# LPD-EPFL/ByzantineMomentum

Measured on AMD Instinct MI355X. Metric: aggregations/sec (Byzantine-robust GAR over n workers x d dims; achieved HBM GB/s per GAR in roofline/per_gar), higher is better.
Workload: dtype f32

## Files before the change

### byzantinemomentum_amd/_lib.py

```python

import ctypes
import pathlib

import torch

import os

_PKG_DIR = pathlib.Path(__file__).resolve().parent
LIB_PATH = pathlib.Path(os.environ["BM_GAR_LIB"]).resolve() if os.environ.get("BM_GAR_LIB") else _PKG_DIR / "libbm_gar.so"

ABI_VERSION = 23
MAX_ROWS = 64
EINVAL = -100000
ENOCOMM, ECOMM = -100001, -100002

OP_MEDIAN, OP_TRMEAN, OP_PHOCAS, OP_MEAMED = 0, 1, 2, 3
WS_PAIRWISE, WS_AKSEL, WS_STATS, WS_DOT, WS_STEP, WS_STUDY = 0, 1, 2, 3, 4, 5
STUDY_SLOTS = 32
STUDY_GRAM, STUDY_EX, STUDY_ATTACK = slice(0, 16), slice(16, 18), slice(18, 20)
STUDY_SUMS = slice(0, 20)
STUDY_MAXES = slice(20, 22)
STUDY_L2 = slice(22, 23)
OUT3_SUMS, OUT3_MAX = slice(0, 2), slice(2, 3)
STEP_S2, STEP_SD, STEP_H2, STEP_HD, STEP_D2, STEP_A2, STEP_AD, STEP_L2 = range(8)
STEP_GRAM, STEP_EX = slice(8, 24), slice(24, 26)
STEP_SMAX, STEP_HMAX, STEP_DMAX, STEP_AMAX = range(26, 30)
RANK_KRUM, RANK_BULYAN = 0, 1
ATTACK_EMPIRE, ATTACK_LITTLE, ATTACK_DIRECTION = 0, 1, 16

_c_float_pp = ctypes.POINTER(ctypes.c_void_p)

SIGNATURES = {
  "bm_abi_version": (ctypes.c_int, []),
  "bm_tuning_set": (ctypes.c_int, [ctypes.c_char_p, ctypes.c_int]),
  "bm_error_string": (ctypes.c_char_p, [ctypes.c_int]),
  "bm_colwise": (ctypes.c_int, [ctypes.c_int, _c_float_pp, ctypes.c_int, ctypes.c_int64, ctypes.c_int,
                                ctypes.c_void_p, ctypes.c_void_p]),
  "bm_workspace_bytes": (ctypes.c_int64, [ctypes.c_int, ctypes.c_int, ctypes.c_int64]),
  "bm_pairwise_sqdist": (ctypes.c_int, [_c_float_pp, ctypes.c_int, ctypes.c_int64, ctypes.c_void_p,
                                        ctypes.c_void_p, ctypes.c_void_p]),
  "bm_pairwise_sqdist_shard": (ctypes.c_int, [_c_float_pp, ctypes.c_int, ctypes.c_int64, ctypes.c_int64,
                                              ctypes.c_void_p, ctypes.c_void_p, ctypes.c_void_p]),
  "bm_krum_rank": (ctypes.c_int, [ctypes.c_void_p, ctypes.c_int, ctypes.c_int, ctypes.c_int, ctypes.c_int,
                                  ctypes.c_void_p, ctypes.c_void_p, ctypes.c_void_p]),
  "bm_selected_mean": (ctypes.c_int, [_c_float_pp, ctypes.c_int, ctypes.c_void_p, ctypes.c_int,
                                      ctypes.c_int64, ctypes.c_void_p, ctypes.c_void_p]),
  "bm_bulyan_pass2": (ctypes.c_int, [_c_float_pp, ctypes.c_int, ctypes.c_void_p, ctypes.c_int, ctypes.c_int,
                                     ctypes.c_int64, ctypes.c_void_p, ctypes.c_void_p]),
  "bm_aksel_pass1": (ctypes.c_int, [_c_float_pp, ctypes.c_int, ctypes.c_int64, ctypes.c_void_p,
                                    ctypes.c_void_p, ctypes.c_void_p, ctypes.c_void_p]),
  "bm_stack_stats": (ctypes.c_int, [_c_float_pp, ctypes.c_int, ctypes.c_int64, ctypes.c_void_p, ctypes.c_void_p,
                                    ctypes.c_float, ctypes.c_int, ctypes.c_void_p, ctypes.c_void_p,
                                    ctypes.c_void_p]),
  "bm_multi_dot": (ctypes.c_int, [_c_float_pp, ctypes.c_int, _c_float_pp, ctypes.c_int, ctypes.c_int64,
                                  ctypes.c_void_p, ctypes.c_void_p, ctypes.c_void_p]),
  "bm_momentum_stats_colwise": (ctypes.c_int, [_c_float_pp, ctypes.c_int, _c_float_pp, ctypes.c_int, ctypes.c_int64,
                                               ctypes.c_float, ctypes.c_float, ctypes.c_void_p, ctypes.c_void_p,
                                               ctypes.c_void_p, ctypes.c_void_p, ctypes.c_float, ctypes.c_int,
                                               ctypes.c_int, ctypes.c_int, ctypes.c_int, ctypes.c_void_p,
                                               ctypes.c_void_p, ctypes.c_void_p, ctypes.c_void_p]),
  "bm_momentum_stats_sqdist": (ctypes.c_int, [_c_float_pp, ctypes.c_int, _c_float_pp, ctypes.c_int, ctypes.c_int64,
                                              ctypes.c_int64, ctypes.c_float, ctypes.c_float, ctypes.c_void_p,
                                              ctypes.c_void_p, ctypes.c_void_p, ctypes.c_void_p, ctypes.c_float,
                                              ctypes.c_int, ctypes.c_int, ctypes.c_void_p, ctypes.c_void_p,
                                              ctypes.c_void_p, ctypes.c_void_p, ctypes.c_void_p]),
  "bm_sharded_sq_slot": (ctypes.c_void_p, [ctypes.c_void_p]),
  "bm_sharded_pair_workspace": (ctypes.c_void_p, [ctypes.c_void_p]),
  "bm_sharded_rule_from_sq": (ctypes.c_int, [ctypes.c_void_p, ctypes.c_int, _c_float_pp, ctypes.c_int, ctypes.c_int64,
                                             ctypes.c_int, ctypes.c_int, ctypes.c_void_p, ctypes.c_void_p,
                                             ctypes.c_void_p, ctypes.c_void_p]),
  "bm_stack_stats_colwise": (ctypes.c_int, [_c_float_pp, ctypes.c_int, ctypes.c_int64, ctypes.c_void_p, ctypes.c_void_p,
                                            ctypes.c_float, ctypes.c_int, ctypes.c_int, ctypes.c_int, ctypes.c_int,
                                            ctypes.c_void_p, ctypes.c_void_p, ctypes.c_void_p, ctypes.c_void_p]),
  "bm_stack_stats_sqdist": (ctypes.c_int, [_c_float_pp, ctypes.c_int, ctypes.c_int64, ctypes.c_int64, ctypes.c_void_p,
                                           ctypes.c_void_p, ctypes.c_float, ctypes.c_int, ctypes.c_int, ctypes.c_void_p,
                                           ctypes.c_void_p, ctypes.c_void_p, ctypes.c_void_p, ctypes.c_void_p]),
  "bm_study_stats": (ctypes.c_int, [ctypes.c_void_p, ctypes.c_void_p, ctypes.c_void_p, ctypes.c_void_p, ctypes.c_int,
                                    ctypes.c_void_p, ctypes.c_void_p, ctypes.c_void_p, ctypes.c_void_p, ctypes.c_int,
                                    ctypes.c_float, ctypes.c_float, ctypes.c_void_p, ctypes.c_void_p, ctypes.c_int64,
                                    ctypes.c_void_p, ctypes.c_void_p, ctypes.c_void_p]),
  "bm_study_stats_update": (ctypes.c_int, [ctypes.c_void_p, ctypes.c_void_p, ctypes.c_void_p, ctypes.c_void_p, ctypes.c_int,
                                           ctypes.c_void_p, ctypes.c_void_p, ctypes.c_void_p, ctypes.c_void_p, ctypes.c_int,
                                           ctypes.c_float, ctypes.c_float, ctypes.c_void_p, ctypes.c_void_p,
                                           ctypes.c_void_p, ctypes.c_float, ctypes.c_float, ctypes.c_int64,
                                           ctypes.c_void_p, ctypes.c_void_p, ctypes.c_void_p]),
  "bm_row_sqnorms": (ctypes.c_int, [_c_float_pp, ctypes.c_int, ctypes.c_int64, ctypes.c_void_p, ctypes.c_void_p,
                                    ctypes.c_void_p]),
  "bm_stable_argsort": (ctypes.c_int, [ctypes.c_void_p, ctypes.c_int, ctypes.c_void_p, ctypes.c_void_p]),
  "bm_anticge_workspace_bytes": (ctypes.c_int64, [ctypes.c_int64]),
  "bm_anticge_sum": (ctypes.c_int, [_c_float_pp, ctypes.c_int, ctypes.c_int64, ctypes.c_int, ctypes.c_void_p,
                                    ctypes.c_void_p, ctypes.c_void_p, ctypes.c_void_p, ctypes.c_void_p, ctypes.c_void_p]),
  "bm_anticge_scale": (ctypes.c_int, [ctypes.c_void_p, ctypes.c_int64, ctypes.c_void_p, ctypes.c_void_p]),
  "bm_multi_axpby": (ctypes.c_int, [_c_float_pp, _c_float_pp, ctypes.c_int, ctypes.c_int64,
                                    ctypes.c_float, ctypes.c_float, ctypes.c_void_p]),
  "bm_brute_select": (ctypes.c_int, [ctypes.c_void_p, ctypes.c_int, ctypes.c_int, ctypes.c_void_p]),
  "bm_momentum_stats": (ctypes.c_int, [_c_float_pp, ctypes.c_int, _c_float_pp, ctypes.c_int, ctypes.c_int64,
                                       ctypes.c_float, ctypes.c_float, ctypes.c_void_p, ctypes.c_void_p,
                                       ctypes.c_void_p, ctypes.c_void_p, ctypes.c_float, ctypes.c_int,
                                       ctypes.c_void_p, ctypes.c_void_p, ctypes.c_void_p]),
  "bm_multi_fma3": (ctypes.c_int, [_c_float_pp, _c_float_pp, _c_float_pp, ctypes.c_int, ctypes.c_int64,
                                   ctypes.c_float, ctypes.c_float, ctypes.c_void_p, ctypes.c_void_p]),
  "bm_multi_fma3_bdev": (ctypes.c_int, [_c_float_pp, _c_float_pp, _c_float_pp, ctypes.c_int, ctypes.c_int64,
                                        ctypes.c_float, ctypes.c_void_p, ctypes.c_void_p, ctypes.c_void_p]),
  "bm_clip_factors": (ctypes.c_int, [ctypes.c_void_p, ctypes.c_int, ctypes.c_float, ctypes.c_void_p,
                                     ctypes.c_void_p]),
  "bm_multi_scale": (ctypes.c_int, [_c_float_pp, ctypes.c_int, ctypes.c_int64, ctypes.c_void_p, ctypes.c_void_p]),
  "bm_comm_available": (ctypes.c_int, []),
  "bm_comm_unique_id": (ctypes.c_int, [ctypes.c_void_p]),
  "bm_comm_init": (ctypes.c_int, [ctypes.POINTER(ctypes.c_void_p), ctypes.c_int, ctypes.c_int, ctypes.c_void_p]),
  "bm_comm_destroy": (ctypes.c_int, [ctypes.c_void_p]),
  "bm_comm_size": (ctypes.c_int, [ctypes.c_void_p]),
  "bm_allreduce_sum_f64": (ctypes.c_int, [ctypes.c_void_p, ctypes.c_void_p, ctypes.c_int64, ctypes.c_void_p]),
  "bm_allgather_f32": (ctypes.c_int, [ctypes.c_void_p, ctypes.c_void_p, ctypes.c_void_p, ctypes.c_int64,
                                      ctypes.c_void_p]),
  "bm_brute_select_device": (ctypes.c_int, [ctypes.c_void_p, ctypes.c_int, ctypes.c_int, ctypes.c_void_p, ctypes.c_void_p,
                                            ctypes.c_void_p]),
  "bm_colwise_eval_supported": (ctypes.c_int, [ctypes.c_int, ctypes.c_int]),
  "bm_colwise_eval_workspace_bytes": (ctypes.c_int64, []),
  "bm_colwise_eval": (ctypes.c_int, [ctypes.c_int, _c_float_pp, ctypes.c_int, ctypes.c_int, ctypes.c_int64, ctypes.c_int,
                                     ctypes.c_void_p, ctypes.c_void_p, ctypes.c_float, ctypes.c_void_p, ctypes.c_void_p,
                                     ctypes.c_void_p]),
  "bm_colwise_eval_tdev": (ctypes.c_int, [ctypes.c_int, _c_float_pp, ctypes.c_int, ctypes.c_int, ctypes.c_int64,
                                          ctypes.c_int, ctypes.c_void_p, ctypes.c_void_p, ctypes.c_void_p, ctypes.c_void_p,
                                          ctypes.c_void_p, ctypes.c_void_p]),
  "bm_sqdist2": (ctypes.c_int, [ctypes.c_void_p, ctypes.c_void_p, ctypes.c_int64, ctypes.c_void_p, ctypes.c_void_p,
                                ctypes.c_void_p]),
  "bm_attack_ranking_device": (ctypes.c_int, [ctypes.c_void_p, ctypes.c_int, ctypes.c_int, ctypes.c_int, ctypes.c_int, ctypes.c_int,
                                              ctypes.c_void_p, ctypes.c_void_p, ctypes.c_void_p]),
  "bm_bulyan_pass2_eval_supported": (ctypes.c_int, [ctypes.c_int, ctypes.c_int, ctypes.c_int]),
  "bm_bulyan_pass2_eval": (ctypes.c_int, [_c_float_pp, ctypes.c_int, ctypes.c_int, ctypes.c_void_p, ctypes.c_int, ctypes.c_int,
                                          ctypes.c_int64, ctypes.c_void_p, ctypes.c_void_p, ctypes.c_float, ctypes.c_void_p,
                                          ctypes.c_void_p, ctypes.c_void_p, ctypes.c_void_p]),
  "bm_order_pair_supported": (ctypes.c_int, [ctypes.c_int]),
  "bm_order_pair": (ctypes.c_int, [_c_float_pp, ctypes.c_int, ctypes.c_int64, ctypes.c_int, ctypes.c_int, ctypes.c_void_p,
                                   ctypes.c_void_p, ctypes.c_void_p]),
  "bm_search_device_next": (ctypes.c_int, [ctypes.c_void_p, ctypes.c_void_p, ctypes.c_int, ctypes.c_int, ctypes.c_double,
                                           ctypes.c_double, ctypes.c_double, ctypes.c_void_p, ctypes.c_void_p,
                                           ctypes.c_void_p]),
  "bm_pairwise_rank": (ctypes.c_int, [_c_float_pp, ctypes.c_int, ctypes.c_int64, ctypes.c_int64, ctypes.c_int, ctypes.c_int,
                                      ctypes.c_int, ctypes.c_void_p, ctypes.c_void_p, ctypes.c_void_p, ctypes.c_void_p,
                                      ctypes.c_void_p]),
  "bm_sharded_workspace_bytes": (ctypes.c_int64, [ctypes.c_int, ctypes.c_int64]),
  "bm_sharded_krum": (ctypes.c_int, [ctypes.c_void_p, _c_float_pp, ctypes.c_int, ctypes.c_int64, ctypes.c_int64,
                                     ctypes.c_int, ctypes.c_int, ctypes.c_void_p, ctypes.c_void_p, ctypes.c_void_p, ctypes.c_void_p]),
  "bm_sharded_bulyan": (ctypes.c_int, [ctypes.c_void_p, _c_float_pp, ctypes.c_int, ctypes.c_int64, ctypes.c_int64,
                                       ctypes.c_int, ctypes.c_int, ctypes.c_void_p, ctypes.c_void_p, ctypes.c_void_p,
                                       ctypes.c_void_p]),
  "bm_step_stats_count": (ctypes.c_int, []),
  "bm_step_workspace_bytes": (ctypes.c_int64, [ctypes.c_int, ctypes.c_int64]),
  "bm_step_worker": (ctypes.c_int, [ctypes.c_void_p, ctypes.c_void_p, _c_float_pp, _c_float_pp, ctypes.c_int64,
                                    ctypes.c_int64] + [ctypes.c_void_p] * 13),
  "bm_search_begin": (ctypes.c_int, [ctypes.c_void_p, ctypes.c_double, ctypes.c_double, ctypes.c_double]),
  "bm_search_propose": (ctypes.c_int, [ctypes.c_void_p, ctypes.c_void_p]),
  "bm_search_report": (ctypes.c_int, [ctypes.c_void_p, ctypes.c_double]),
  "bm_attack_objective": (ctypes.c_int, [ctypes.c_void_p, ctypes.c_int, ctypes.c_int, ctypes.c_int, ctypes.c_int,
                                         ctypes.c_int, ctypes.c_double, ctypes.c_void_p, ctypes.c_void_p,
# ... 72 lines not shown
```

### byzantinemomentum_amd/csrc/api.cpp

```cpp
#include <stdlib.h>
#include <string.h>
#include <math.h>
#include <algorithm>
#include <vector>
#include "bm_common.h"

namespace bm {
static int env_int(const char* name, int dflt) {
  const char* v = getenv(name);
  if (v == nullptr || *v == '\0') return dflt;
  return atoi(v);
}
static double env_double(const char* name, double dflt) {
  const char* v = getenv(name);
  if (v == nullptr || *v == '\0') return dflt;
  return atof(v);
}
Tuning& tuning_mutable() {
  static Tuning t = {env_int("BM_COL_BURST", 8),  env_int("BM_MEAN_BURST", 8),
                           env_int("BM_STEP_BURST", 8), env_int("BM_STEP_STREAM", 0), env_int("BM_PAIR_MODE", 0),
                           env_int("BM_PAIR_PLANES", 0), env_int("BM_PAIR_DITHER", 0), env_double("BM_PAIR_TAU", 2e-3),
                           env_int("BM_STUDY_BURST", 8), env_int("BM_STEP_STAGGER_US", 0),
                           env_int("BM_GRAM_STEADY", 1), env_int("BM_BULYAN_SHORT", 1),
                           env_int("BM_PAIR_LOAD_NT", 1), env_int("BM_RANK_ALGO", 0), env_int("BM_COL_WIDE", 1), env_int("BM_BRUTE_BUDGET", 0)};
  return t;
}
const Tuning& tuning() { return tuning_mutable(); }
}

extern "C" int bm_abi_version(void) { return 23; }

extern "C" int bm_tuning_set(const char* name, int value) {
  using namespace bm;
  if (name == nullptr) return BM_EINVAL;
  Tuning& t = tuning_mutable();
  const struct { const char* key; int* slot; } knobs[] = {
      {"BM_COL_BURST", &t.col_burst}, {"BM_MEAN_BURST", &t.mean_burst}, {"BM_STEP_BURST", &t.step_burst},
      {"BM_STEP_STREAM", &t.step_stream}, {"BM_PAIR_MODE", &t.pair_mode}, {"BM_PAIR_PLANES", &t.pair_planes},
      {"BM_PAIR_DITHER", &t.pair_dither}, {"BM_STUDY_BURST", &t.study_burst},
      {"BM_STEP_STAGGER_US", &t.step_stagger_us}, {"BM_GRAM_STEADY", &t.gram_steady},
      {"BM_BULYAN_SHORT", &t.bulyan_short}, {"BM_PAIR_LOAD_NT", &t.pair_load_nt},
      {"BM_RANK_ALGO", &t.rank_algo}, {"BM_COL_WIDE", &t.col_wide}, {"BM_BRUTE_BUDGET", &t.brute_budget}};
  for (const auto& k : knobs)
    if (strcmp(name, k.key) == 0) {
      *k.slot = value;
      return 0;
    }
  return BM_EINVAL;
}

extern "C" const char* bm_error_string(int code) {
  if (code == 0) return "success";
  if (code == BM_EINVAL) return "invalid argument for libbm_gar";
  if (code == BM_ENOCOMM) return "RCCL is not available in this process (librccl.so.1 could not be bound)";
  if (code == BM_ECOMM) return "an RCCL call failed";
  if (code < 0) return hipGetErrorString(static_cast<hipError_t>(-code));
  return "unknown libbm_gar status";
}

namespace {
struct BruteGraph {
  int n;
  uint64_t adj[BM_MAX_ROWS];

  void build(const double* dist, double t) {
    for (int i = 0; i < n; ++i) adj[i] = 0;
    for (int i = 0; i < n; ++i)
      for (int j = i + 1; j < n; ++j) {
        const double v = dist[i * n + j];
        if (isfinite(v) && v <= t) {
          adj[i] |= (uint64_t)1 << j;
          adj[j] |= (uint64_t)1 << i;
        }
      }
  }

  bool has_clique(uint64_t cand, int need) const {
    const int count = __builtin_popcountll(cand);
    if (count < need) return false;
    if (need <= 1) return true;
    int worst = -1, worst_missing = 0;
    for (uint64_t rest = cand; rest != 0; rest &= rest - 1) {
      const int u = __builtin_ctzll(rest);
      const int missing = __builtin_popcountll(cand & ~adj[u] & ~((uint64_t)1 << u));
      if (missing > worst_missing) {
        worst = u;
        worst_missing = missing;
      }
    }
    if (worst < 0) return true;
    const int budget = count - need;
    if (budget == 0) return false;
    const uint64_t bit = (uint64_t)1 << worst;
    if (worst_missing <= budget && has_clique(cand & (adj[worst] | bit), need)) return true;
    return has_clique(cand & ~bit, need);
  }
};
}

extern "C" int bm_brute_select(const double* dist_nxn, int n, int f, int32_t* sel_out) {
  if (dist_nxn == nullptr || sel_out == nullptr || n < 1 || n > BM_MAX_ROWS || f < 0 || n - f < 1)
    return BM_EINVAL;
  const int k = n - f;
  const uint64_t everyone = n == 64 ? ~(uint64_t)0 : (((uint64_t)1 << n) - 1);
  std::vector<double> values;
  values.reserve((size_t)n * (n - 1) / 2 + 1);
  values.push_back(0.0);
  for (int i = 0; i < n; ++i)
    for (int j = i + 1; j < n; ++j) {
      const double v = dist_nxn[i * n + j];
      if (isfinite(v) && v > 0.0) values.push_back(v);
    }
  std::sort(values.begin(), values.end());
  values.erase(std::unique(values.begin(), values.end()), values.end());
  BruteGraph g;
  g.n = n;
  g.build(dist_nxn, values.back());
  if (!g.has_clique(everyone, k)) return BM_EINVAL;
  size_t lo = 0, hi = values.size() - 1;
  while (lo < hi) {
    const size_t mid = (lo + hi) / 2;
    g.build(dist_nxn, values[mid]);
    if (g.has_clique(everyone, k))
      hi = mid;
    else
// ... 18 lines not shown
```

### byzantinemomentum_amd/csrc/bm_common.h

```cpp
#pragma once
#include <hip/hip_runtime.h>
#include <stdint.h>
#include <utility>
#include "../../include/bm_gar.h"
#include "launch_plan.h"

namespace bm {

struct RowTable {
  const float* p[BM_MAX_ROWS];
  RowTable advanced(int64_t by) const {
    RowTable t = *this;
    advance(t.p, by);
    return t;
  }
};

static inline int hip_code(hipError_t e) { return e == hipSuccess ? 0 : -(int)e; }

#define BM_LAUNCH_CHECK()                      \
  do {                                         \
    hipError_t e__ = hipGetLastError();        \
    if (e__ != hipSuccess) return hip_code(e__); \
  } while (0)
// ... 135 lines not shown
    store_result<VEC>(p, src);
}

constexpr int kColMaxBlocks = 256 * 64;

static inline int lds_opt_in(const void* kernel, size_t dynamic_bytes, size_t static_bytes) {
  if (dynamic_bytes + static_bytes <= 48u * 1024u) return 0;
  return hip_code(hipFuncSetAttribute(kernel, hipFuncAttributeMaxDynamicSharedMemorySize, (int)dynamic_bytes));
}

static inline int compute_units() {
  static int cached[16] = {0};
  int dev = 0;
  if (hipGetDevice(&dev) != hipSuccess || dev < 0 || dev >= 16) dev = 0;
  if (cached[dev] == 0) {
    int cus = 0;
    if (hipDeviceGetAttribute(&cus, hipDeviceAttributeMultiprocessorCount, dev) != hipSuccess || cus <= 0) cus = 256;
    cached[dev] = cus;
  }
  return cached[dev];
}

__device__ __forceinline__ bool arrive_last(int* counter, int total, int* lds_flag) {
  asm volatile("s_waitcnt vmcnt(0)" ::: "memory");
  __syncthreads();
  if (threadIdx.x == 0) {
    __builtin_amdgcn_fence(__ATOMIC_RELEASE, "agent");
    asm volatile("s_waitcnt vmcnt(0)" ::: "memory");
    const int ticket = atomicAdd(counter, 1);
    const int last = (ticket == total - 1) ? 1 : 0;
    if (last) __builtin_amdgcn_fence(__ATOMIC_ACQUIRE, "agent");
    *lds_flag = last;
  }
  __syncthreads();
  return *lds_flag != 0;
}

__device__ __forceinline__ int32_t load_index_coherent(const int32_t* p) {
  return __hip_atomic_load(p, __ATOMIC_RELAXED, __HIP_MEMORY_SCOPE_AGENT);
}

template <int BLOCK>
__device__ __forceinline__ double block_reduce_sum(double v, double* lds ) {
#pragma unroll
  for (int off = 32; off > 0; off >>= 1) v += __shfl_down(v, off, 64);
  const int wave = threadIdx.x >> 6, lane = threadIdx.x & 63;
  if (lane == 0) lds[wave] = v;
  __syncthreads();
  double r = 0.0;
  if (threadIdx.x == 0) {
#pragma unroll
    for (int w = 0; w < BLOCK / 64; ++w) r += lds[w];
  }
  __syncthreads();
  return r;
}

__device__ __forceinline__ float byzantine_coordinate(float avg, float q, float fk, float scale, int attack_kind) {
  const float dir = ((attack_kind & 15) == BM_ATTACK_LITTLE) ? __builtin_sqrtf(q / (fk - 1.0f)) : -avg;
  const float att = dir * scale;
  return (attack_kind & BM_ATTACK_DIRECTION) ? att : avg + att;
}

}

namespace bm {
struct Tuning {
  int col_burst;
  int mean_burst;
  int step_burst;
  int step_stream;
  int pair_mode;
  int pair_planes;
  int pair_dither;
  double pair_tau;
  int study_burst;
  int step_stagger_us;
  int gram_steady;
  int bulyan_short;
  int pair_load_nt;
  int rank_algo;
  int col_wide;
  int brute_budget;
};
const Tuning& tuning();
Tuning& tuning_mutable();
}
```

### byzantinemomentum_amd/csrc/step.hip

```cpp
#include "colwise_kernels.h"
#include "gram_split.h"

namespace bm {

constexpr int kStepBlock = 256;
constexpr int kStepMaxBlocks = 16384;
constexpr int kStepPieceCap = 2047;
static_assert(caps_of(kStepPieceCap).sets() <= kStepMaxBlocks + 1, "first pass: partials exceed BM_WS_STEP");

struct StepTable {
  const float* g[BM_MAX_ROWS];
  float* b[BM_MAX_ROWS];
  StepTable advanced(int64_t by) const {
    StepTable t = *this;
    advance(t.g, by);
    advance(t.b, by);
    return t;
  }
};

template <int BLOCK>
__device__ __forceinline__ float block_reduce_absmax(float m, float* lds) {
#pragma unroll
  for (int off = 32; off > 0; off >>= 1) {
    const float o = __shfl_down(m, off, 64);
    m = (m != m || o != o) ? __builtin_nanf("") : fmaxf(m, o);
  }
  if ((threadIdx.x & 63) == 0) lds[threadIdx.x >> 6] = m;
  __syncthreads();
  float r = 0.0f;
  if (threadIdx.x == 0) {
    r = lds[0];
    for (int w = 1; w < BLOCK / 64; ++w) {
      const float o = lds[w];
      r = (r != r || o != o) ? __builtin_nanf("") : fmaxf(r, o);
    }
  }
  __syncthreads();
  return r;
}

template <int BLOCK>
__device__ __forceinline__ void store_step_partials(float n2s, float dvs, float mxs, float n2h, float dvh, float mxh, bool nan_s,
                                                    bool nan_h, double* red, float* mred, double* __restrict__ partial) {
  if (nan_s) mxs = __builtin_nanf("");
  if (nan_h) mxh = __builtin_nanf("");
  const double r0 = block_reduce_sum<BLOCK>((double)n2s, red);
  const double r1 = block_reduce_sum<BLOCK>((double)dvs, red);
  const double r3 = block_reduce_sum<BLOCK>((double)n2h, red);
  const double r4 = block_reduce_sum<BLOCK>((double)dvh, red);
  const float r2 = block_reduce_absmax<BLOCK>(mxs, mred);
  const float r5 = block_reduce_absmax<BLOCK>(mxh, mred);
  if (threadIdx.x == 0) {
    double* p = partial + (int64_t)blockIdx.x * 6;
    p[0] = r0;
    p[1] = r1;
    p[2] = (double)r2;
    p[3] = r3;
    p[4] = r4;
    p[5] = (double)r5;
  }
}

typedef const float* __attribute__((address_space(4))) const* KargRowPtrs;
constexpr int kStepBurstBlock = 512;

template <int T, int VEC, bool EXACT, bool CLIP, bool BURST, int RULE = -1, int NB = 0, bool NOMOM = false>
__global__ __launch_bounds__(BURST ? kStepBurstBlock : kStepBlock) void momentum_stats_kernel(
    StepTable tab, int ks_rt, int h_rt, uint32_t nvec, float mu, float omd, const float* __restrict__ clipf,
    float* __restrict__ s_avg_out, float* __restrict__ h_avg_out, float* __restrict__ byz_out, float scale,
    int attack_kind, double* __restrict__ partial, int rule_f, float rule_inv_keep, float* __restrict__ defense_out) {
  static_assert(RULE < 0 || (EXACT && NB >= 1), "the fused rule needs the row count at compile time");
  static_assert(!NOMOM || (EXACT && !CLIP), "without buffers: same stack, clipped in place beforehand");
  constexpr int BLOCK = BURST ? kStepBurstBlock : kStepBlock;
  __shared__ double red[BLOCK / 64];
  __shared__ float mred[BLOCK / 64];
  const float fks = (float)(EXACT ? T : ks_rt), fh = (float)(EXACT ? T : h_rt);
  float n2s = 0.0f, dvs = 0.0f, mxs = 0.0f, n2h = 0.0f, dvh = 0.0f, mxh = 0.0f;
  bool nan_s = false, nan_h = false;
  uint64_t kbase = (uint64_t)__builtin_amdgcn_kernarg_segment_ptr();
  (void)tab;
  const uint32_t span = gridDim.x * BLOCK;
  const uint32_t iters = (nvec + span - 1) / span;
  const uint32_t first = blockIdx.x * BLOCK + threadIdx.x;
  for (uint32_t it = 0; it < iters; ++it) {
    const uint32_t v = it * span + first;
    const bool live = v < nvec;
    const uint32_t off = v * (uint32_t)(VEC * sizeof(float));
    float g[T][VEC], b[T][VEC];
    float sa[VEC], ha[VEC], bz[VEC], df[VEC];
    asm volatile("" : "+s"(kbase));
    int ks = T, h = T;
    if constexpr (!EXACT) {
      ks = ks_rt;
      h = h_rt;
      asm volatile("" : "+s"(ks), "+s"(h));
    }
    if (live) {
      KargRowPtrs karg = (KargRowPtrs)kbase;
#pragma unroll
      for (int i = 0; i < T; ++i) {
        if (i < ks) load_stream_off<VEC>(karg[i], off, g[i]);
        if constexpr (!NOMOM) {
          if (i < h) load_stream_off<VEC>(karg[BM_MAX_ROWS + i], off, b[i]);
        }
      }
#pragma unroll
      for (int i = 0; i < T; ++i) {
        if constexpr (CLIP) {
          if (i < ks) {
            const float cf = clipf[i];
#pragma unroll
            for (int c = 0; c < VEC; ++c) g[i][c] *= cf;
          }
        }
        if (i < h) {
#pragma unroll
          for (int c = 0; c < VEC; ++c) b[i][c] = NOMOM ? g[i][c] : __builtin_fmaf(omd, g[i][c], mu * b[i][c]);
        }
      }
#pragma unroll
      for (int c = 0; c < VEC; ++c) {
        float s = g[0][c];
#pragma unroll
        for (int i = 1; i < T; ++i)
          if (i < ks) s += g[i][c];
        s = s / fks;
        sa[c] = s;
        n2s = __builtin_fmaf(s, s, n2s);
        mxs = fmaxf(mxs, __builtin_fabsf(s));
        nan_s |= (s != s);
        float q = 0.0f;
#pragma unroll
        for (int i = 0; i < T; ++i)
          if (i < ks) {
            const float df = g[i][c] - s;
            q = __builtin_fmaf(df, df, q);
          }
        dvs += q;
        float t = b[0][c];
#pragma unroll
        for (int i = 1; i < T; ++i)
          if (i < h) t += b[i][c];
        t = t / fh;
        ha[c] = t;
        n2h = __builtin_fmaf(t, t, n2h);
        mxh = fmaxf(mxh, __builtin_fabsf(t));
        nan_h |= (t != t);
        float qh = 0.0f;
#pragma unroll
        for (int i = 0; i < T; ++i)
          if (i < h) {
            const float df = b[i][c] - t;
            qh = __builtin_fmaf(df, df, qh);
          }
        dvh += qh;
        bz[c] = byzantine_coordinate(t, qh, fh, scale, attack_kind);
        if constexpr (RULE >= 0) {
          float x[T + NB];
#pragma unroll
          for (int i = 0; i < T; ++i) x[i] = b[i][c];
#pragma unroll
          for (int i = 0; i < NB; ++i) x[T + i] = bz[c];
          df[c] = column_rule<T + NB, RULE, BLOCK>(x, rule_f, rule_inv_keep, nullptr);
        }
      }
    }
    if constexpr (BURST) __syncthreads();
    asm volatile("" : "+s"(kbase));
    if (live) {
      KargRowPtrs karg = (KargRowPtrs)kbase;
      if constexpr (!NOMOM) {
#pragma unroll
        for (int i = 0; i < T; ++i)
          if (i < h) store_stream_off<VEC>(const_cast<float*>(karg[BM_MAX_ROWS + i]), off, b[i]);
      }
      if (s_avg_out != nullptr) store_stream_off<VEC>(s_avg_out, off, sa);
      if (h_avg_out != nullptr) store_stream_off<VEC>(h_avg_out, off, ha);
      if (byz_out != nullptr) store_stream_off<VEC>(byz_out, off, bz);
      if constexpr (RULE >= 0) store_stream_off<VEC>(defense_out, off, df);
    }
  }
  store_step_partials<BLOCK>(n2s, dvs, mxs, n2h, dvh, mxh, nan_s, nan_h, red, mred, partial);
}

constexpr int kSgRowBytes = 272;
constexpr int kSgWaves = kStepBurstBlock / 64;
template <int TT>
struct SgShape {
  static constexpr int N = TT + 1;
  static constexpr int RB = (N + 15) / 16;
  static constexpr int NP = RB * (RB + 1) / 2;
  static constexpr int kRows = N + 1;
  static constexpr int kPlaneBytes = kRows * kSgRowBytes;
  static constexpr int kWaveBytes = 2 * kPlaneBytes;
  static constexpr int kAccBytes = NP * 4 * kStepBurstBlock * 4;
  static constexpr int kRedBytes = kSgWaves * 256 * 8;
  static constexpr int kPlanes = kSgWaves * kWaveBytes > kRedBytes ? kSgWaves * kWaveBytes : kRedBytes;
  static constexpr int kLds = kPlanes + kAccBytes;
};

template <int TT, bool CLIP, bool NOMOM = false>
__global__ __launch_bounds__(kStepBurstBlock) void momentum_gram_kernel(
    StepTable tab, uint32_t nvec, float mu, float omd, const float* __restrict__ clipf, float* __restrict__ s_avg_out,
    float* __restrict__ h_avg_out, float* __restrict__ byz_out, float scale, int attack_kind, unsigned dither_seed,
    double* __restrict__ partial, double* __restrict__ gram_partial, int* __restrict__ arrival, int stagger_ticks) {
  using SG = SgShape<TT>;
  constexpr int T = TT, VEC = 4, BLOCK = kStepBurstBlock;
  constexpr int kSgPlaneBytes = SG::kPlaneBytes, kSgWaveBytes = SG::kWaveBytes, kSgN = SG::N, RB = SG::RB, NP = SG::NP;
  extern __shared__ __attribute__((aligned(16))) char sg_smem[];
  __shared__ double red[BLOCK / 64];
  __shared__ float mred[BLOCK / 64];
  const int tid = threadIdx.x, wave = tid >> 6, lane = tid & 63;
  char* wbase = sg_smem + wave * kSgWaveBytes;
  for (int o = lane * 16; o < kSgWaveBytes; o += 64 * 16) *reinterpret_cast<f32x4*>(wbase + o) = f32x4{0.0f, 0.0f, 0.0f, 0.0f};
  if (blockIdx.x == 0 && tid == 0 && arrival != nullptr) *arrival = 0;
  if (stagger_ticks > 0 && ((blockIdx.x >> 3) & 1)) {
    const uint64_t t0 = wall_clock64();
    while ((uint64_t)wall_clock64() - t0 < (uint64_t)stagger_ticks) __builtin_amdgcn_s_sleep(16);
  }
  const float fks = (float)T, fh = (float)T;
  float n2s = 0.0f, dvs = 0.0f, mxs = 0.0f, n2h = 0.0f, dvh = 0.0f, mxh = 0.0f;
  bool nan_s = false, nan_h = false;
  float* acc_lds = reinterpret_cast<float*>(sg_smem + SG::kPlanes) + tid;
#pragma unroll
  for (int p = 0; p < NP * 4; ++p) acc_lds[p * BLOCK] = 0.0f;
  uint64_t kbase = (uint64_t)__builtin_amdgcn_kernarg_segment_ptr();
  (void)tab;
  const uint32_t span = gridDim.x * BLOCK;
  const uint32_t iters = (nvec + span - 1) / span;
  const uint32_t first = blockIdx.x * BLOCK + threadIdx.x;
  const int li = lane & 15, lg = lane >> 4;
  const int rd0 = li * kSgRowBytes + lg * 16;
  const int rd_last = ((16 * (RB - 1) + li < kSgN) ? (16 * (RB - 1) + li) : kSgN) * kSgRowBytes + lg * 16;
  const int wr0 = (lane & 31) * 8;
  for (uint32_t it = 0; it < iters; ++it) {
    const uint32_t v = it * span + first;
    const bool live = v < nvec;
    const uint32_t off = v * (uint32_t)(VEC * sizeof(float));
    float b[T][VEC];
    float sa[VEC], ha[VEC], bz[VEC];
#pragma unroll
    for (int c = 0; c < VEC; ++c) sa[c] = ha[c] = bz[c] = 0.0f;
    asm volatile("" : "+s"(kbase));
    if (live) {
      float g[T][VEC];
      KargRowPtrs karg = (KargRowPtrs)kbase;
#pragma unroll
      for (int i = 0; i < T; ++i) {
        load_stream_off<VEC>(karg[i], off, g[i]);
        if constexpr (!NOMOM) load_stream_off<VEC>(karg[BM_MAX_ROWS + i], off, b[i]);
      }
#pragma unroll
      for (int i = 0; i < T; ++i) {
        if constexpr (CLIP) {
          const float cf = clipf[i];
#pragma unroll
          for (int c = 0; c < VEC; ++c) g[i][c] *= cf;
        }
#pragma unroll
        for (int c = 0; c < VEC; ++c) b[i][c] = NOMOM ? g[i][c] : __builtin_fmaf(omd, g[i][c], mu * b[i][c]);
      }
#pragma unroll
      for (int c = 0; c < VEC; ++c) {
        float s = g[0][c];
#pragma unroll
// ... 170 lines not shown
          for (int c = 0; c < VEC; ++c) {
            const float gv = CLIP ? g[j][c] * cfi : g[j][c];
            if (i == 0) {
              ps[c] = gv;
              ss[c] = gv;
              qs[c] = 0.0f;
              ts[c] = 0.0f;
            } else {
              const float dd = on_s ? gv - ps[c] : 0.0f;
              ss[c] += on_s ? gv : 0.0f;
              qs[c] = __builtin_fmaf(dd, dd, qs[c]);
              ts[c] += dd;
            }
            g[j][c] = gv;
          }
          if (base < hl) {
#pragma unroll
            for (int c = 0; c < VEC; ++c) b[j][c] = __builtin_fmaf(omd, g[j][c], mu * b[j][c]);
            if (on_h) store_stream_off<VEC>(const_cast<float*>(karg[BM_MAX_ROWS + i]), off, b[j]);
#pragma unroll
            for (int c = 0; c < VEC; ++c) {
              const float bv = b[j][c];
              if (i == 0) {
                ph[c] = bv;
                sh[c] = bv;
                qh[c] = 0.0f;
                th[c] = 0.0f;
              } else {
                const float dd = on_h ? bv - ph[c] : 0.0f;
                sh[c] += on_h ? bv : 0.0f;
                qh[c] = __builtin_fmaf(dd, dd, qh[c]);
                th[c] += dd;
              }
            }
          }
        }
      }
    }
    float r_sa[VEC], r_ha[VEC], r_bz[VEC];
#pragma unroll
    for (int c = 0; c < VEC; ++c) {
      const float s = ss[c] / fks;
      r_sa[c] = s;
      n2s = __builtin_fmaf(s, s, n2s);
      mxs = fmaxf(mxs, __builtin_fabsf(s));
      nan_s |= (s != s);
      const float es = s - ps[c];
      dvs += __builtin_fmaf(es, __builtin_fmaf(fks, es, -2.0f * ts[c]), qs[c]);
      const float t = sh[c] / fh;
      r_ha[c] = t;
      n2h = __builtin_fmaf(t, t, n2h);
      mxh = fmaxf(mxh, __builtin_fabsf(t));
      nan_h |= (t != t);
      const float eh = t - ph[c];
      float colq = __builtin_fmaf(eh, __builtin_fmaf(fh, eh, -2.0f * th[c]), qh[c]);
      colq = colq < 0.0f ? 0.0f : colq;
      dvh += colq;
      r_bz[c] = byzantine_coordinate(t, colq, fh, scale, attack_kind);
    }
    if (s_avg_out != nullptr) store_stream_off<VEC>(s_avg_out, off, r_sa);
    if (h_avg_out != nullptr) store_stream_off<VEC>(h_avg_out, off, r_ha);
    if (byz_out != nullptr) store_stream_off<VEC>(byz_out, off, r_bz);
  }
  if (nan_s) mxs = __builtin_nanf("");
  if (nan_h) mxh = __builtin_nanf("");
  const double r0 = block_reduce_sum<kStepBlock>((double)n2s, red);
  const double r1 = block_reduce_sum<kStepBlock>((double)dvs, red);
  const double r3 = block_reduce_sum<kStepBlock>((double)n2h, red);
  const double r4 = block_reduce_sum<kStepBlock>((double)dvh, red);
  const float r2 = block_reduce_absmax<kStepBlock>(mxs, mred);
  const float r5 = block_reduce_absmax<kStepBlock>(mxh, mred);
  if (threadIdx.x == 0) {
    double* p = partial + (int64_t)blockIdx.x * 6;
    p[0] = r0;
    p[1] = r1 < 0.0 ? 0.0 : r1;
    p[2] = (double)r2;
    p[3] = r3;
    p[4] = r4;
    p[5] = (double)r5;
  }
}

constexpr int kFinishThreads = 256;
__global__ __launch_bounds__(kFinishThreads) void step_finish_kernel(const double* __restrict__ partial, int nparts,
                                                                     double* __restrict__ out6) {
  __shared__ double red[kFinishThreads / 64][8];
  const int lane = threadIdx.x & 63, wave = threadIdx.x >> 6;
  double s[6] = {0.0, 0.0, 0.0, 0.0, 0.0, 0.0};
  bool nan2 = false, nan5 = false;
  for (int b = threadIdx.x; b < nparts; b += kFinishThreads) {
    const double* p = partial + (int64_t)b * 6;
    s[0] += p[0];
    s[1] += p[1];
    s[3] += p[3];
    s[4] += p[4];
    nan2 |= (p[2] != p[2]);
    nan5 |= (p[5] != p[5]);
    s[2] = p[2] > s[2] ? p[2] : s[2];
    s[5] = p[5] > s[5] ? p[5] : s[5];
  }
#pragma unroll
  for (int off = 32; off > 0; off >>= 1) {
    s[0] += __shfl_down(s[0], off, 64);
    s[1] += __shfl_down(s[1], off, 64);
    s[3] += __shfl_down(s[3], off, 64);
    s[4] += __shfl_down(s[4], off, 64);
    const double o2 = __shfl_down(s[2], off, 64), o5 = __shfl_down(s[5], off, 64);
    s[2] = o2 > s[2] ? o2 : s[2];
    s[5] = o5 > s[5] ? o5 : s[5];
    nan2 |= (bool)__shfl_down((int)nan2, off, 64);
    nan5 |= (bool)__shfl_down((int)nan5, off, 64);
  }
  if (lane == 0) {
#pragma unroll
    for (int k = 0; k < 6; ++k) red[wave][k] = s[k];
    red[wave][6] = nan2 ? 1.0 : 0.0;
    red[wave][7] = nan5 ? 1.0 : 0.0;
  }
  __syncthreads();
  if (threadIdx.x == 0) {
    for (int w = 1; w < kFinishThreads / 64; ++w) {
      s[0] += red[w][0];
      s[1] += red[w][1];
      s[3] += red[w][3];
      s[4] += red[w][4];
      s[2] = red[w][2] > s[2] ? red[w][2] : s[2];
      s[5] = red[w][5] > s[5] ? red[w][5] : s[5];
      nan2 |= red[w][6] != 0.0;
      nan5 |= red[w][7] != 0.0;
    }
  }
  if (threadIdx.x == 0) {
    out6[0] = s[0];
    out6[1] = s[1];
    out6[2] = nan2 ? __builtin_nan("") : s[2];
    out6[3] = s[3];
    out6[4] = s[4];
    out6[5] = nan5 ? __builtin_nan("") : s[5];
  }
}

struct StepArgs {
  StepTable tab;
  int ks, h;
  int64_t nvec;
  float mu, omd;
  const float* clipf;
  float *s_avg, *h_avg, *byz;
  float scale;
  int kind;
  double* partial;
  int* grid_io;
  hipStream_t s;
  bool nomom = false;
  int rule_f = 0;
  float rule_inv_keep = 0.0f;
  float* defense = nullptr;
  StepArgs moved(int64_t by) const {
    StepArgs a = *this;
    a.tab = tab.advanced(by);
    a.s_avg = advanced(s_avg, by);
    a.h_avg = advanced(h_avg, by);
    a.byz = advanced(byz, by);
    return a;
  }
  StepArgs at(Span& sp) const {
    StepArgs a = moved(sp.first);
    a.nvec = sp.count;
    a.partial = partial + (int64_t)sp.part * 6;
    a.grid_io = &sp.grid;
    return a;
  }
};

static StepTable make_step_table(const float* const* sampled, int ks, float* const* buffers, int h) {
  StepTable tab{};
  for (int i = 0; i < BM_MAX_ROWS; ++i) {
    tab.g[i] = sampled[i < ks ? i : ks - 1];
    if (buffers != nullptr) tab.b[i] = buffers[i < h ? i : h - 1];
  }
  return tab;
}

static bool burst_ready(int64_t nvec, int cus) {
  return tuning().step_burst > 0 && nvec / ((int64_t)cus * kStepBurstBlock) >= tuning().step_burst;
}

static bool is_column_rule(int op) {
  return op == BM_OP_MEDIAN || op == BM_OP_TRMEAN || op == BM_OP_PHOCAS || op == BM_OP_MEAMED;
}
static bool is_identical_attack(int kind) {
  return (kind & ~BM_ATTACK_DIRECTION) == BM_ATTACK_EMPIRE || (kind & ~BM_ATTACK_DIRECTION) == BM_ATTACK_LITTLE;
}

template <class Kernel>
static int launch_momentum_stats_kernel(Kernel kernel, int grid, int block, const StepArgs& a) {
  hipLaunchKernelGGL(kernel, dim3(grid), dim3(block), 0, a.s, a.tab, a.ks, a.h, (uint32_t)a.nvec, a.mu, a.omd, a.clipf,
                     a.s_avg, a.h_avg, a.byz, a.scale, a.kind, a.partial, a.rule_f, a.rule_inv_keep, a.defense);
  BM_LAUNCH_CHECK();
  return 0;
}

template <int T, int VEC, bool EXACT, bool CLIP, int RULE = -1, int NB = 0, bool NOMOM = false>
static int launch_momentum_stats_form(const StepArgs& a) {
  const int cus = compute_units();
  if (burst_ready(a.nvec, cus) && cus < *a.grid_io) {
    *a.grid_io = cus;
    return launch_momentum_stats_kernel(momentum_stats_kernel<T, VEC, EXACT, CLIP, true, RULE, NB, NOMOM>, cus, kStepBurstBlock, a);
  }
  return launch_momentum_stats_kernel(momentum_stats_kernel<T, VEC, EXACT, CLIP, false, RULE, NB, NOMOM>, *a.grid_io, kStepBlock, a);
}

template <int T, int VEC>
static int launch_momentum_stats(const StepArgs& a) {
  const bool exact = (a.ks == T && a.h == T);
  if constexpr (T > 12) {
    if (!exact) return BM_EINVAL;
    return a.clipf != nullptr ? launch_momentum_stats_form<T, VEC, true, true>(a) : launch_momentum_stats_form<T, VEC, true, false>(a);
  } else {
    if (a.clipf != nullptr) return exact ? launch_momentum_stats_form<T, VEC, true, true>(a) : launch_momentum_stats_form<T, VEC, false, true>(a);
    return exact ? launch_momentum_stats_form<T, VEC, true, false>(a) : launch_momentum_stats_form<T, VEC, false, false>(a);
  }
}

template <int T, int VEC>
static int launch_momentum_stats_stream(const StepArgs& a) {
  auto kernel = a.clipf != nullptr ? momentum_stats_stream_kernel<T, VEC, true> : momentum_stats_stream_kernel<T, VEC, false>;
  hipLaunchKernelGGL(kernel, dim3(*a.grid_io), dim3(kStepBlock), 0, a.s, a.tab, a.ks, a.h, (uint32_t)a.nvec, a.mu, a.omd,
                     a.clipf, a.s_avg, a.h_avg, a.byz, a.scale, a.kind, a.partial);
  BM_LAUNCH_CHECK();
  return 0;
}

template <int VEC>
static int dispatch_momentum_stats(const StepArgs& a) {
  const int ks = a.ks, h = a.h, t = ks > h ? ks : h;
  if (tuning().step_stream != 1) {
    if (t <= 8) return launch_momentum_stats<8, VEC>(a);
    if (t <= 12) return launch_momentum_stats<12, VEC>(a);
    if (ks == 14 && h == 14) return launch_momentum_stats<14, VEC>(a);
    if (ks == 20 && h == 20) return launch_momentum_stats<20, VEC>(a);
  }
  if (t <= 20) return launch_momentum_stats_stream<20, VEC>(a);
  if (t <= 40) return launch_momentum_stats_stream<40, VEC>(a);
  return launch_momentum_stats_stream<64, VEC>(a);
}

struct Fma3Table {
  float* out[BM_MAX_ROWS];
  const float* p[BM_MAX_ROWS];
  const float* q[BM_MAX_ROWS];
  Fma3Table advanced(int64_t by) const {
    Fma3Table t = *this;
    advance(t.out, by);
    advance(t.p, by);
    advance(t.q, by);
    return t;
  }
};

template <int VEC>
__global__ __launch_bounds__(kStepBlock) void multi_fma3_kernel(Fma3Table tab, int64_t nvec, float a, float b_host,
                                                                const float* __restrict__ pscale,
                                                                const double* __restrict__ b_dev) {
  const float b = b_dev != nullptr ? (float)b_dev[0] : b_host;
  float* out = tab.out[blockIdx.y];
  const float* p = tab.p[blockIdx.y];
  const float* q = tab.q[blockIdx.y];
  const float c = pscale != nullptr ? pscale[blockIdx.y] : 1.0f;
  const int64_t stride = (int64_t)gridDim.x * kStepBlock;
  for (int64_t v = (int64_t)blockIdx.x * kStepBlock + threadIdx.x; v < nvec; v += stride) {
    float pp[VEC], qq[VEC];
    load_stream<VEC>(p + v * VEC, pp);
    load_stream<VEC>(q + v * VEC, qq);
#pragma unroll
    for (int e = 0; e < VEC; ++e) {
      const float x = pscale != nullptr ? pp[e] * c : pp[e];
      pp[e] = __builtin_fmaf(b, qq[e], a * x);
    }
    store_stream<VEC>(out + v * VEC, pp);
  }
}

struct ScaleTable {
  float* y[BM_MAX_ROWS];
  ScaleTable advanced(int64_t by) const {
    ScaleTable t = *this;
    advance(t.y, by);
    return t;
  }
};
template <int VEC>
__global__ __launch_bounds__(kStepBlock) void multi_scale_kernel(ScaleTable tab, int64_t nvec,
                                                                 const float* __restrict__ factors) {
  const float c = factors[blockIdx.y];
  if (c == 1.0f) return;
  float* y = tab.y[blockIdx.y];
  const int64_t stride = (int64_t)gridDim.x * kStepBlock;
  for (int64_t v = (int64_t)blockIdx.x * kStepBlock + threadIdx.x; v < nvec; v += stride) {
    float yy[VEC];
    load_stream<VEC>(y + v * VEC, yy);
#pragma unroll
    for (int e = 0; e < VEC; ++e) yy[e] *= c;
    store_stream<VEC>(y + v * VEC, yy);
  }
}

__global__ __launch_bounds__(64) void clip_factors_kernel(const double* __restrict__ row_sq, int k, float clip,
                                                          float* __restrict__ factors) {
  const int i = threadIdx.x;
  if (i >= k) return;
  const double norm = sqrt(row_sq[i]);
  factors[i] = (norm > (double)clip) ? (float)((double)clip / norm) : 1.0f;
}

template <int T, int RULE, int NB, bool CLIP, bool NOMOM = false>
static int launch_fused_rule(StepArgs a) {
  constexpr int N = T + NB;
  const int keep = (RULE == BM_OP_TRMEAN) ? (N - 2 * a.rule_f) : ((RULE == BM_OP_PHOCAS || RULE == BM_OP_MEAMED) ? (N - a.rule_f) : N);
  a.rule_inv_keep = 1.0f / (float)(keep > 0 ? keep : 1);
  return launch_momentum_stats_form<T, 4, true, CLIP, RULE, NB, NOMOM>(a);
}

template <int T, int RULE, int NB>
static int launch_fused_rule_clip(const StepArgs& a) {
  if (a.nomom) return launch_fused_rule<T, RULE, NB, false, true>(a);
  return a.clipf != nullptr ? launch_fused_rule<T, RULE, NB, true>(a) : launch_fused_rule<T, RULE, NB, false>(a);
}

static bool fused_rule_shape(int h, int nb) { return (h == 20 && nb == 5) || (h == 14 && nb == 11); }
static bool fused_rule_instance(int ks, int h, int nb, int op) {
  return is_column_rule(op) && tuning().step_stream != 1 && ks == h && fused_rule_shape(h, nb);
}

static int launch_fused_rule_any(int op, int nb, int rule_f, float* defense, StepArgs a) {
  a.rule_f = rule_f;
  a.defense = defense;
#define BM_FUSED_CASE(TV, NBV)                                                                 \
  if (a.h == TV && nb == NBV) {                                                                \
    if (op == BM_OP_MEDIAN) return launch_fused_rule_clip<TV, BM_OP_MEDIAN, NBV>(a);           \
    if (op == BM_OP_TRMEAN) return launch_fused_rule_clip<TV, BM_OP_TRMEAN, NBV>(a);           \
    if (op == BM_OP_PHOCAS) return launch_fused_rule_clip<TV, BM_OP_PHOCAS, NBV>(a);           \
    return launch_fused_rule_clip<TV, BM_OP_MEAMED, NBV>(a);                                   \
  }
  BM_FUSED_CASE(20, 5) BM_FUSED_CASE(14, 11)
#undef BM_FUSED_CASE
  return BM_EINVAL;
}

double* pairwise_gram_area(void* ws);
int* pairwise_arrival_counter(void* ws);
int pairwise_from_gram_partials(const float* const* rows, int n_full, int nc, int blocks, int64_t d, double* sq_nxn,
                                void* ws, hipStream_t s);

template <int TT>
static int launch_momentum_gram_rows(const StepArgs& a, int cus, void* ws_pair) {
  auto kernel = a.nomom ? momentum_gram_kernel<TT, false, true>
                        : (a.clipf != nullptr ? momentum_gram_kernel<TT, true> : momentum_gram_kernel<TT, false>);
  constexpr int lds = SgShape<TT>::kLds;
  if (const int rc = lds_opt_in(reinterpret_cast<const void*>(kernel), lds, kSgWaves * (sizeof(double) + sizeof(float)))) return rc;
  *a.grid_io = cus;
  hipLaunchKernelGGL(kernel, dim3(cus), dim3(kStepBurstBlock), lds, a.s, a.tab, (uint32_t)a.nvec, a.mu, a.omd, a.clipf,
                     a.s_avg, a.h_avg, a.byz, a.scale, a.kind, (unsigned)tuning().pair_dither, a.partial,
                     pairwise_gram_area(ws_pair), pairwise_arrival_counter(ws_pair), tuning().step_stagger_us * 100);
  BM_LAUNCH_CHECK();
  return 0;
}
static int launch_momentum_gram(const StepArgs& a, int cus, void* ws_pair) {
  return a.h == 20 ? launch_momentum_gram_rows<20>(a, cus, ws_pair) : launch_momentum_gram_rows<14>(a, cus, ws_pair);
}

__global__ __launch_bounds__(256) void tail_gram_kernel(RowTable rows , int nrows,
                                                        const float* __restrict__ h_avg_tail, int cols,
                                                        double* __restrict__ block) {
  const int t = threadIdx.x;
  if (t >= nrows * (nrows + 1) / 2) return;
  int i = 0, rem = t, len = nrows;
  while (rem >= len) {
    rem -= len;
    --len;
    ++i;
  }
  const int j = i + rem;
  double acc = 0.0;
  for (int c = 0; c < cols; ++c) {
    const float ctr = (__builtin_fabsf(h_avg_tail[c]) < __builtin_inff()) ? h_avg_tail[c] : 0.0f;
    acc += (double)(rows.p[i][c] - ctr) * (double)(rows.p[j][c] - ctr);
  }
  block[b3_tri_index(i, j, nrows)] = acc;
}

int64_t step_workspace_bytes() { return (int64_t)(kStepMaxBlocks + 1) * 6 * (int64_t)sizeof(double); }

static int momentum_stats_impl(const float* const* sampled, int ks, float* const* buffers, int h, int64_t d, float mu,
                               float one_minus_damp, const float* clip_factors, float* sampled_avg, float* honest_avg,
                               float* byz_out, float scale, int attack_kind, double* out6, void* ws, void* stream,
                               int rule_op, int rule_f, int nb, float* defense_out) {
  if (sampled == nullptr || buffers == nullptr || out6 == nullptr || ws == nullptr || h < 1 || ks < h ||
      ks > BM_MAX_ROWS || d < 0 || !is_identical_attack(attack_kind))
    return BM_EINVAL;
  if (rule_op >= 0 && (!is_column_rule(rule_op) || nb < 1 || h + nb > BM_MAX_ROWS || (attack_kind & BM_ATTACK_DIRECTION) != 0 ||
                       (d > 0 && (byz_out == nullptr || defense_out == nullptr)) ||
                       (rule_op != BM_OP_MEDIAN && (rule_f < 0 || h + nb < 2 * rule_f + 1))))
    return BM_EINVAL;
  hipStream_t s = static_cast<hipStream_t>(stream);
  const int vec = Alignment().of(sampled_avg).of(honest_avg).of(byz_out).of(rule_op >= 0 ? defense_out : nullptr)
                      .of(sampled, ks).of(buffers, h).vec();
  double* partial = static_cast<double*>(ws);
  const StepArgs pass{make_step_table(sampled, ks, buffers, h), ks, h, 0, mu, one_minus_damp, clip_factors, sampled_avg,
                      honest_avg, byz_out, scale, attack_kind, partial, nullptr, s};
  const int64_t pieces = piece_count(d);
  int cap = pieces > 1 ? (int)((kStepMaxBlocks - 1) / pieces) - 1 : kStepPieceCap;
  if (cap > kStepPieceCap) cap = kStepPieceCap;
  if (cap < 1) return BM_EINVAL;
  const bool fusable = rule_op >= 0 && fused_rule_instance(ks, h, nb, rule_op);
  int nparts = 0;
  const int rc = for_pieces(d, [&](int64_t lo, int64_t dp) {
    const StepArgs piece = pass.moved(lo);
    int64_t ruled = 0;
    const int rc = for_body_and_tail<4>(Tail::kOwnLaunch, vec, dp, kStepBlock, caps_of(cap), [&](auto width, Span& sp) {
      constexpr int VEC = decltype(width)::value;
      if constexpr (VEC == 4) {
        if (fusable) {
          ruled = sp.end;
          return launch_fused_rule_any(rule_op, nb, rule_f, defense_out + lo, piece.at(sp));
        }
      }
      return dispatch_momentum_stats<VEC>(piece.at(sp));
    }, &nparts);
    if (rc != 0 || rule_op < 0 || ruled == dp) return rc;
    const float* rows[BM_MAX_ROWS];
    for (int i = 0; i < h; ++i) rows[i] = buffers[i] + lo + ruled;
    for (int i = 0; i < nb; ++i) rows[h + i] = byz_out + lo + ruled;
    return bm_colwise(rule_op, rows, h + nb, dp - ruled, rule_f, defense_out + lo + ruled, stream);
  });
  if (rc != 0) return rc;
  hipLaunchKernelGGL(step_finish_kernel, dim3(1), dim3(kFinishThreads), 0, s, partial, nparts, out6);
  BM_LAUNCH_CHECK();
  return 0;
}
}

extern "C" int bm_momentum_stats(const float* const* sampled, int ks, float* const* buffers, int h, int64_t d,
                                 float mu, float one_minus_damp, const float* clip_factors, float* sampled_avg,
                                 float* honest_avg, float* byz_out, float scale, int attack_kind, double* out6,
                                 void* ws, void* stream) {
  return bm::momentum_stats_impl(sampled, ks, buffers, h, d, mu, one_minus_damp, clip_factors, sampled_avg, honest_avg,
                                 byz_out, scale, attack_kind, out6, ws, stream, -1, 0, 0, nullptr);
}

extern "C" int bm_momentum_stats_colwise(const float* const* sampled, int ks, float* const* buffers, int h, int64_t d,
                                         float mu, float one_minus_damp, const float* clip_factors, float* sampled_avg,
                                         float* honest_avg, float* byz_out, float scale, int attack_kind, int rule_op,
                                         int rule_f, int n_byz, float* defense_out, double* out6, void* ws,
                                         void* stream) {
  if (rule_op < 0) return BM_EINVAL;
  return bm::momentum_stats_impl(sampled, ks, buffers, h, d, mu, one_minus_damp, clip_factors, sampled_avg, honest_avg,
                                 byz_out, scale, attack_kind, out6, ws, stream, rule_op, rule_f, n_byz, defense_out);
}

extern "C" int bm_momentum_stats_sqdist(const float* const* sampled, int ks, float* const* buffers, int h, int64_t d,
                                        int64_t d_total, float mu, float one_minus_damp, const float* clip_factors,
                                        float* sampled_avg, float* honest_avg, float* byz_out, float scale,
                                        int attack_kind, int n_byz, double* sq_nxn, double* out6, void* ws,
                                        void* ws_pair, void* stream) {
  using namespace bm;
  const int n = h + n_byz;
  if (sampled == nullptr || buffers == nullptr || out6 == nullptr || ws == nullptr || ws_pair == nullptr ||
      sq_nxn == nullptr || h < 1 || ks < h || ks > BM_MAX_ROWS || n_byz < 1 || n > BM_MAX_ROWS || d < 0 || d_total < d ||
      !is_identical_attack(attack_kind) || (attack_kind & BM_ATTACK_DIRECTION) != 0 || (d > 0 && byz_out == nullptr))
    return BM_EINVAL;
  hipStream_t s = static_cast<hipStream_t>(stream);
  const float* rows[BM_MAX_ROWS];
  for (int i = 0; i < h; ++i) rows[i] = buffers[i];
  for (int i = h; i < n; ++i) rows[i] = byz_out;
// ... 10 lines not shown
    return bm_pairwise_sqdist_shard(rows, n, d, d_total, sq_nxn, ws_pair, stream);
  }
  double* partial = static_cast<double*>(ws);
  const StepArgs pass{make_step_table(sampled, ks, buffers, h), ks, h, 0, mu, one_minus_damp, clip_factors, sampled_avg,
                      honest_avg, byz_out, scale, attack_kind, partial, nullptr, s};
  const int nc = h + 1;
  const int per_block = nc * (nc + 1) / 2;
  int nparts = 0, blocks = 0;
  const int rc = for_body_and_tail<4>(Tail::kOwnLaunch, vec, d, kStepBlock, caps_of(kStepPieceCap), [&](auto width, Span& sp) {
    constexpr int VEC = decltype(width)::value;
    if constexpr (VEC == 4) {
      blocks = cus;
      return launch_momentum_gram(pass.at(sp), cus, ws_pair);
    } else if constexpr (VEC == 1) {
      if (const int rc = dispatch_momentum_stats<1>(pass.at(sp))) return rc;
      RowTable trows{};
      for (int i = 0; i < h; ++i) trows.p[i] = buffers[i] + sp.first;
      trows.p[h] = byz_out + sp.first;
      hipLaunchKernelGGL(tail_gram_kernel, dim3(1), dim3(256), 0, s, trows, nc, honest_avg + sp.first, (int)sp.count,
                         pairwise_gram_area(ws_pair) + (int64_t)blocks * per_block);
      BM_LAUNCH_CHECK();
      blocks += 1;
      return 0;
    } else {
      return BM_EINVAL;
    }
  }, &nparts);
  if (rc != 0) return rc;
  hipLaunchKernelGGL(step_finish_kernel, dim3(1), dim3(kFinishThreads), 0, s, partial, nparts, out6);
  BM_LAUNCH_CHECK();
  return pairwise_from_gram_partials(rows, n, nc, blocks, d, sq_nxn, ws_pair, s);
}

namespace bm {
static int stack_stats_plain(const float* const* rows, int k, int64_t d, float* avg_out, float* byz_out, float scale,
                             int attack_kind, double* out6, void* ws, void* stream) {
  int rc = bm_stack_stats(rows, k, d, avg_out, byz_out, scale, attack_kind, out6 + 3, ws, stream);
  if (rc != 0) return rc;
  return hip_code(hipMemcpyAsync(out6, out6 + 3, 3 * sizeof(double), hipMemcpyDeviceToDevice,
                                 static_cast<hipStream_t>(stream)));
}
static bool nomom_shape(int k, int nb) { return (k == 20 && nb >= 1 && nb <= 6) || (k == 14 && nb == 11); }
}

extern "C" int bm_stack_stats_colwise(const float* const* rows, int k, int64_t d, float* avg_out, float* byz_out,
                                      float scale, int attack_kind, int rule_op, int rule_f, int n_byz,
                                      float* defense_out, double* out6, void* ws, void* stream) {
  using namespace bm;
  const int n = k + n_byz;
  if (rows == nullptr || out6 == nullptr || ws == nullptr || k < 1 || n_byz < 1 || n > BM_MAX_ROWS || d < 0 ||
      !is_identical_attack(attack_kind) || (attack_kind & BM_ATTACK_DIRECTION) != 0 || !is_column_rule(rule_op) ||
      (rule_op != BM_OP_MEDIAN && (rule_f < 0 || n < 2 * rule_f + 1)) ||
      (d > 0 && (avg_out == nullptr || byz_out == nullptr || defense_out == nullptr)))
    return BM_EINVAL;
  hipStream_t s = static_cast<hipStream_t>(stream);
  const int vec = Alignment().of(avg_out).of(byz_out).of(defense_out).of(rows, k).vec();
  const bool fused = fused_rule_shape(k, n_byz) && vec == 4 && d % 4 == 0 && d > 0 && d <= kMaxColsPerLaunch &&
                     tuning().step_stream != 1;
  if (fused) {
    double* partial = static_cast<double*>(ws);
    StepArgs pass{make_step_table(rows, k, nullptr, k), k, k, 0, 0.0f, 1.0f, nullptr, nullptr, avg_out, byz_out, scale,
                  attack_kind, partial, nullptr, s};
    pass.nomom = true;
    int nparts = 0;
    const int rc = for_body_and_tail<4>(Tail::kOwnLaunch, vec, d, kStepBlock, caps_of(kStepPieceCap), [&](auto width, Span& sp) {
      if constexpr (decltype(width)::value == 4)
        return launch_fused_rule_any(rule_op, n_byz, rule_f, defense_out, pass.at(sp));
      else
        return BM_EINVAL;
    }, &nparts);
    if (rc != 0) return rc;
    hipLaunchKernelGGL(step_finish_kernel, dim3(1), dim3(kFinishThreads), 0, s, partial, nparts, out6);
    BM_LAUNCH_CHECK();
    return 0;
  }
  int rc = stack_stats_plain(rows, k, d, avg_out, byz_out, scale, attack_kind, out6, ws, stream);
  if (rc != 0 || d == 0) return rc;
  const float* all[BM_MAX_ROWS];
  for (int i = 0; i < k; ++i) all[i] = rows[i];
  for (int i = k; i < n; ++i) all[i] = byz_out;
  return bm_colwise(rule_op, all, n, d, rule_f, defense_out, stream);
}

extern "C" int bm_stack_stats_sqdist(const float* const* rows, int k, int64_t d, int64_t d_total, float* avg_out,
                                     float* byz_out, float scale, int attack_kind, int n_byz, double* sq_nxn,
                                     double* out6, void* ws, void* ws_pair, void* stream) {
  using namespace bm;
  const int n = k + n_byz;
  if (rows == nullptr || out6 == nullptr || ws == nullptr || ws_pair == nullptr || sq_nxn == nullptr || k < 1 ||
      n_byz < 1 || n > BM_MAX_ROWS || d < 0 || d_total < d ||
      !is_identical_attack(attack_kind) || (attack_kind & BM_ATTACK_DIRECTION) != 0 ||
      (d > 0 && (avg_out == nullptr || byz_out == nullptr)))
    return BM_EINVAL;
  hipStream_t s = static_cast<hipStream_t>(stream);
  const float* all[BM_MAX_ROWS];
  for (int i = 0; i < k; ++i) all[i] = rows[i];
  for (int i = k; i < n; ++i) all[i] = byz_out;
  const int vec = Alignment().of(avg_out).of(byz_out).of(rows, k).vec();
  const int cus = compute_units();
  const bool fused = nomom_shape(k, n_byz) && vec == 4 && d % 4 == 0 && d <= kMaxColsPerLaunch &&
                     tuning().step_stream != 1 && tuning().pair_mode == 0 && tuning().pair_planes != 3 &&
                     burst_ready(d / 4, cus);
  if (!fused) {
    int rc = stack_stats_plain(rows, k, d, avg_out, byz_out, scale, attack_kind, out6, ws, stream);
    if (rc != 0) return rc;
    return bm_pairwise_sqdist_shard(all, n, d, d_total, sq_nxn, ws_pair, stream);
  }
  double* partial = static_cast<double*>(ws);
  StepArgs pass{make_step_table(rows, k, nullptr, k), k, k, 0, 0.0f, 1.0f, nullptr, nullptr, avg_out, byz_out, scale,
                attack_kind, partial, nullptr, s};
  pass.nomom = true;
  int nparts = 0;
  const int rc = for_body_and_tail<4>(Tail::kOwnLaunch, vec, d, kStepBlock, caps_of(kStepPieceCap), [&](auto width, Span& sp) {
    if constexpr (decltype(width)::value == 4)
      return launch_momentum_gram(pass.at(sp), cus, ws_pair);
    else
      return BM_EINVAL;
  }, &nparts);
  if (rc != 0) return rc;
  hipLaunchKernelGGL(step_finish_kernel, dim3(1), dim3(kFinishThreads), 0, s, partial, nparts, out6);
  BM_LAUNCH_CHECK();
  return pairwise_from_gram_partials(all, n, k + 1, cus, d, sq_nxn, ws_pair, s);
}

static int multi_fma3_launch(float* const* out, const float* const* p, const float* const* q, int k, int64_t d, float a,
                             float b, const float* p_scale, const double* b_dev, void* stream) {
  using namespace bm;
  if (out == nullptr || p == nullptr || q == nullptr || k < 1 || k > BM_MAX_ROWS || d < 0) return BM_EINVAL;
  if (d == 0) return 0;
  hipStream_t s = static_cast<hipStream_t>(stream);
  Fma3Table tab{};
  for (int i = 0; i < k; ++i) {
    tab.out[i] = out[i];
    tab.p[i] = p[i];
    tab.q[i] = q[i];
  }
  const int vec = Alignment().of(out, k).of(p, k).of(q, k).vec();
  return for_body_and_tail<4>(Tail::kOwnLaunch, vec, d, kStepBlock, caps_of(2048), [&](auto width, const Span& sp) {
    hipLaunchKernelGGL(multi_fma3_kernel<decltype(width)::value>, dim3(sp.grid, k), dim3(kStepBlock), 0, s,
                       tab.advanced(sp.first), sp.count, a, b, p_scale, b_dev);
    BM_LAUNCH_CHECK();
    return 0;
  });
}

extern "C" int bm_multi_fma3(float* const* out, const float* const* p, const float* const* q, int k, int64_t d,
                             float a, float b, const float* p_scale, void* stream) {
  return multi_fma3_launch(out, p, q, k, d, a, b, p_scale, nullptr, stream);
}

extern "C" int bm_multi_fma3_bdev(float* const* out, const float* const* p, const float* const* q, int k, int64_t d,
                                  float a, const double* b_dev, const float* p_scale, void* stream) {
  if (b_dev == nullptr) return BM_EINVAL;
  return multi_fma3_launch(out, p, q, k, d, a, 0.0f, p_scale, b_dev, stream);
}

extern "C" int bm_multi_scale(float* const* y, int k, int64_t d, const float* factors, void* stream) {
  using namespace bm;
  if (y == nullptr || factors == nullptr || k < 1 || k > BM_MAX_ROWS || d < 0) return BM_EINVAL;
  if (d == 0) return 0;
  hipStream_t s = static_cast<hipStream_t>(stream);
  ScaleTable tab{};
  for (int i = 0; i < k; ++i) tab.y[i] = y[i];
  const int vec = Alignment().of(y, k).vec();
  return for_body_and_tail<4>(Tail::kOwnLaunch, vec, d, kStepBlock, caps_of(2048), [&](auto width, const Span& sp) {
    hipLaunchKernelGGL(multi_scale_kernel<decltype(width)::value>, dim3(sp.grid, k), dim3(kStepBlock), 0, s,
// ... 15 lines not shown
```

### byzantinemomentum_amd/csrc/step_call.hip

```cpp
#include "bm_common.h"

namespace bm {

constexpr int kStatSums = 26;
constexpr int kStatMaxes = 4;
constexpr int kStatSlots = 32;
static_assert(kStatSums + kStatMaxes <= kStatSlots, "statistics vector layout");

struct StepScalars {
  double out6[6];
  double study[BM_STUDY_SLOTS];
  double rowsq[BM_MAX_ROWS];
  double mine[kStatSlots];
  double all[kStatSlots * BM_MAX_ROWS];
  float clipf[BM_MAX_ROWS];
};

__global__ void step_pack_kernel(StepScalars* sc, int has_attack, int has_past, int has_l2, double* __restrict__ direct_out) {
  if (threadIdx.x != 0) return;
  double* m = sc->mine;
  const double* st = sc->study;
  for (int i = 0; i < kStatSlots; ++i) m[i] = 0.0;
  m[0] = sc->out6[0];
  m[1] = sc->out6[1];
// ... 21 lines not shown
  const int slot = threadIdx.x;
  if (slot >= kStatSlots) return;
  double acc = all[slot];
  bool nan = acc != acc;
  for (int r = 1; r < nranks; ++r) {
    const double v = all[r * kStatSlots + slot];
    if (slot < kStatSums) {
      acc += v;
    } else {
      nan |= (v != v);
      acc = v > acc ? v : acc;
    }
  }
  out[slot] = (slot >= kStatSums && nan) ? __builtin_nan("") : acc;
}

struct StepLayout {
  int64_t scalars, ws_step, ws_study, ws_dot, ws_rule, total;
};

static StepLayout step_layout(int n, int64_t d) {
  StepLayout l;
  auto up = [](int64_t v) { return (v + 255) / 256 * 256; };
  int64_t off = 0;
  l.scalars = off;
  off += up((int64_t)sizeof(StepScalars));
  l.ws_step = off;
  off += up(bm_workspace_bytes(BM_WS_STEP, 1, d));
  l.ws_study = off;
  off += up(bm_workspace_bytes(BM_WS_STUDY, 1, d));
  l.ws_dot = off;
  off += up(bm_workspace_bytes(BM_WS_DOT, 1, d));
  l.ws_rule = off;
  off += up(bm_sharded_workspace_bytes(n, d));
  l.total = off;
  return l;
}

}

extern "C" int bm_step_stats_count(void) { return bm::kStatSlots; }

extern "C" int64_t bm_step_workspace_bytes(int n, int64_t d_local) {
  if (n < 1 || n > BM_MAX_ROWS || d_local < 0) return BM_EINVAL;
  return bm::step_layout(n, d_local).total;
}

extern "C" int bm_step_worker(bm_comm* comm, const bm_step_params* p, const float* const* sampled,
                              float* const* buffers, int64_t d, int64_t d_total, float* defense_out,
                              float* sampled_avg_out,
                              float* honest_avg_out, float* byz_out, float* attack_avg_out,
                              const float* past_newest, float* curv, const float* past_oldest, const float* params,
                              const float* origin, double* stats_out, void* ws, void* stream) {
  using namespace bm;
  if (p == nullptr || sampled == nullptr || buffers == nullptr || stats_out == nullptr || ws == nullptr || d < 0 ||
      d_total < d)
    return BM_EINVAL;
  const int n = p->n, h = p->n - p->f_real, ks = p->ks, fr = p->f_real;
  if (n < 1 || n > BM_MAX_ROWS || h < 1 || ks < h || ks > BM_MAX_ROWS || fr < 0 ||
      (d > 0 && (defense_out == nullptr || sampled_avg_out == nullptr || honest_avg_out == nullptr)) ||
      (fr > 0 && d > 0 && byz_out == nullptr))
    return BM_EINVAL;
  const bool distance_rule = p->rule == BM_RULE_KRUM || p->rule == BM_RULE_BULYAN;
  if (!distance_rule && p->rule != BM_RULE_MEDIAN && p->rule != BM_RULE_TRMEAN && p->rule != BM_RULE_PHOCAS &&
      p->rule != BM_RULE_MEAMED)
    return BM_EINVAL;
  hipStream_t s = static_cast<hipStream_t>(stream);
  char* base = static_cast<char*>(ws);
  const StepLayout lay = step_layout(n, d);
  StepScalars* sc = reinterpret_cast<StepScalars*>(base + lay.scalars);
  int rc;

  const float* clipf = nullptr;
  if (p->clip > 0.0f) {
    rc = bm_row_sqnorms(sampled, ks, d, sc->rowsq, base + lay.ws_dot, stream);
    if (rc != 0) return rc;
    rc = bm_allreduce_sum_f64(comm, sc->rowsq, ks, stream);
    if (rc != 0) return rc;
    rc = bm_clip_factors(sc->rowsq, ks, p->clip, sc->clipf, stream);
    if (rc != 0) return rc;
    clipf = sc->clipf;
  }

  const bool rides_along = fr >= 1;
  const float* rows[BM_MAX_ROWS];
  for (int i = 0; i < h; ++i) rows[i] = buffers[i];
  for (int i = h; i < n; ++i) rows[i] = byz_out;
  const int m = p->m > 0 ? p->m : n - p->f_decl - 2;
  if (rides_along && !distance_rule) {
    const int op = p->rule == BM_RULE_MEDIAN ? BM_OP_MEDIAN
                   : p->rule == BM_RULE_TRMEAN ? BM_OP_TRMEAN : p->rule == BM_RULE_PHOCAS ? BM_OP_PHOCAS : BM_OP_MEAMED;
    rc = bm_momentum_stats_colwise(sampled, ks, buffers, h, d, p->mu, p->one_minus_damp, clipf, sampled_avg_out,
                                   honest_avg_out, byz_out, p->attack_scale, p->attack_kind, op, p->f_decl, fr,
                                   defense_out, sc->out6, base + lay.ws_step, stream);
    if (rc != 0) return rc;
  } else if (rides_along) {
    char* rule_ws = base + lay.ws_rule;
    rc = bm_momentum_stats_sqdist(sampled, ks, buffers, h, d, d_total, p->mu, p->one_minus_damp,
                                  clipf, sampled_avg_out, honest_avg_out, byz_out, p->attack_scale, p->attack_kind, fr,
                                  bm_sharded_sq_slot(rule_ws), sc->out6, base + lay.ws_step,
                                  bm_sharded_pair_workspace(rule_ws), stream);
    if (rc != 0) return rc;
    rc = bm_sharded_rule_from_sq(comm, p->rule, rows, n, d, p->f_decl, m, defense_out, nullptr, rule_ws, stream);
    if (rc != 0) return rc;
  } else {
    rc = bm_momentum_stats(sampled, ks, buffers, h, d, p->mu, p->one_minus_damp, clipf, sampled_avg_out, honest_avg_out,
                           nullptr, p->attack_scale, p->attack_kind, sc->out6, base + lay.ws_step, stream);
    if (rc != 0) return rc;
    switch (p->rule) {
      case BM_RULE_KRUM:
        rc = bm_sharded_krum(comm, rows, n, d, d_total, p->f_decl, m, defense_out, nullptr, base + lay.ws_rule, stream);
        break;
      case BM_RULE_BULYAN:
        rc = bm_sharded_bulyan(comm, rows, n, d, d_total, p->f_decl, m, defense_out, nullptr, base + lay.ws_rule, stream);
        break;
      case BM_RULE_MEDIAN: rc = bm_colwise(BM_OP_MEDIAN, rows, n, d, 0, defense_out, stream); break;
      case BM_RULE_TRMEAN: rc = bm_colwise(BM_OP_TRMEAN, rows, n, d, p->f_decl, defense_out, stream); break;
      case BM_RULE_PHOCAS: rc = bm_colwise(BM_OP_PHOCAS, rows, n, d, p->f_decl, defense_out, stream); break;
      default: rc = bm_colwise(BM_OP_MEAMED, rows, n, d, p->f_decl, defense_out, stream); break;
    }
    if (rc != 0) return rc;
  }

  int curv_mode = 0;
  if (p->nb_past > 0 && curv != nullptr) {
    if (p->past_count == 0 || past_newest == nullptr)
      curv_mode = 1;
    else
      curv_mode = past_oldest != nullptr ? 3 : 2;
  }
  const bool has_past = curv_mode >= 2;
  const bool has_l2 = params != nullptr && origin != nullptr;
  rc = bm_study_stats(sampled_avg_out, honest_avg_out, defense_out, byz_out, fr, attack_avg_out, past_newest, curv,
                      past_oldest, curv_mode, p->mu, p->oldest_weight, params, origin, d, sc->study,
                      base + lay.ws_study, stream);
  if (rc != 0) return rc;

  hipLaunchKernelGGL(step_pack_kernel, dim3(1), dim3(64), 0, s, sc, fr > 0 ? 1 : 0, has_past ? 1 : 0, has_l2 ? 1 : 0,
                     comm == nullptr ? stats_out : static_cast<double*>(nullptr));
  BM_LAUNCH_CHECK();
  if (comm == nullptr) return 0;
  const int nranks = bm_comm_size(comm);
  if (nranks > BM_MAX_ROWS) return BM_EINVAL;
  rc = bm_allgather_f32(comm, reinterpret_cast<const float*>(sc->mine), reinterpret_cast<float*>(sc->all),
                        2 * kStatSlots, stream);
  if (rc != 0) return rc;
  hipLaunchKernelGGL(step_reduce_kernel, dim3(1), dim3(64), 0, s, sc->all, nranks, stats_out);
  BM_LAUNCH_CHECK();
  return 0;
}
```

### byzantinemomentum_amd/csrc/study.hip

```cpp
#include "bm_common.h"

namespace bm {

constexpr int kStudyBlock = 256;
constexpr int kStudyMaxBlocks = 2048;
constexpr int kStudySums = 14;
constexpr int kStudyPartial = 16;

struct StudyArgs {
  const float* s;
  const float* h;
  const float* def;
  const float* byz;
  const float* past;
  const float* oldest;
  const float* params;
  const float* origin;
  float* curv;
  float* a_out;
  float* mom;
  float mom_a, mom_b;
  StudyArgs advanced(int64_t by) const {
    using bm::advanced;
    return StudyArgs{advanced(s, by), advanced(h, by), advanced(def, by), advanced(byz, by), advanced(past, by),
                     advanced(oldest, by), advanced(params, by), advanced(origin, by), advanced(curv, by),
                     advanced(a_out, by), advanced(mom, by), mom_a, mom_b};
  }
};
constexpr Caps kStudyCaps = caps_of(kStudyMaxBlocks);

template <bool ATT, int CM, bool L2, int VEC>
__global__ __launch_bounds__(kStudyBlock) void study_stats_kernel(StudyArgs a, int f_real, float mu, float w_oldest,
                                                                  int64_t nvec, double* __restrict__ partial) {
  __shared__ double red[kStudyBlock / 64];
  __shared__ float mred[kStudyBlock / 64];
  float acc[kStudySums];
  double acc64[kStudySums];
#pragma unroll
  for (int i = 0; i < kStudySums; ++i) {
    acc[i] = 0.0f;
    acc64[i] = 0.0;
  }
  int since = 0;
  float amax = 0.0f, dmax = 0.0f;
  bool a_nan = false, d_nan = false;
  const float ff = (float)f_real;
  const int64_t stride = (int64_t)gridDim.x * kStudyBlock;
  for (int64_t v = (int64_t)blockIdx.x * kStudyBlock + threadIdx.x; v < nvec; v += stride) {
    const int64_t j = v * VEC;
    float s[VEC], h[VEC], df[VEC], bz[VEC], pa[VEC], cv[VEC], ol[VEC], pp[VEC], oo[VEC], mm[VEC];
    load_stream<VEC>(a.s + j, s);
    load_stream<VEC>(a.h + j, h);
    load_stream<VEC>(a.def + j, df);
    if (a.mom != nullptr) load_stream<VEC>(a.mom + j, mm);
    if constexpr (ATT) load_stream<VEC>(a.byz + j, bz);
    if constexpr (CM >= 2) {
      load_stream<VEC>(a.past + j, pa);
      load_stream<VEC>(a.curv + j, cv);
    }
    if constexpr (CM == 3) load_stream<VEC>(a.oldest + j, ol);
    if constexpr (L2) {
      load_stream<VEC>(a.params + j, pp);
      load_stream<VEC>(a.origin + j, oo);
    }
    float av[VEC];
#pragma unroll
    for (int c = 0; c < VEC; ++c) {
      av[c] = 0.0f;
      if constexpr (ATT) {
        float t = bz[c];
        for (int i = 1; i < f_real; ++i) t += bz[c];
        t = t / ff;
        av[c] = t;
        amax = fmaxf(amax, __builtin_fabsf(t));
        a_nan |= (t != t);
        const float dd = bz[c] - t;
        float q = 0.0f;
        for (int i = 0; i < f_real; ++i) q = __builtin_fmaf(dd, dd, q);
        acc[12] += q;
      }
      dmax = fmaxf(dmax, __builtin_fabsf(df[c]));
      d_nan |= (df[c] != df[c]);
      acc[0] = __builtin_fmaf(s[c], s[c], acc[0]);
      acc[1] = __builtin_fmaf(s[c], h[c], acc[1]);
      acc[2] = __builtin_fmaf(s[c], df[c], acc[2]);
      acc[4] = __builtin_fmaf(h[c], h[c], acc[4]);
      acc[5] = __builtin_fmaf(h[c], df[c], acc[5]);
      acc[7] = __builtin_fmaf(df[c], df[c], acc[7]);
      if constexpr (ATT) {
        acc[3] = __builtin_fmaf(s[c], av[c], acc[3]);
        acc[6] = __builtin_fmaf(h[c], av[c], acc[6]);
        acc[8] = __builtin_fmaf(df[c], av[c], acc[8]);
        acc[9] = __builtin_fmaf(av[c], av[c], acc[9]);
      }
      if constexpr (CM >= 2) {
        acc[10] = __builtin_fmaf(s[c], pa[c], acc[10]);
        acc[11] = __builtin_fmaf(s[c], cv[c], acc[11]);
      }
      if constexpr (L2) {
        const float e = pp[c] - oo[c];
        acc[13] = __builtin_fmaf(e, e, acc[13]);
      }
      if constexpr (CM == 1) cv[c] = s[c];
      if constexpr (CM == 3) cv[c] = __builtin_fmaf(w_oldest, ol[c], 1.0f * cv[c]);
      if constexpr (CM >= 2) cv[c] = __builtin_fmaf(1.0f, s[c], mu * cv[c]);
    }
    if constexpr (CM >= 1) store_stream<VEC>(a.curv + j, cv);
    if (a.mom != nullptr) {
#pragma unroll
      for (int c = 0; c < VEC; ++c) mm[c] = __builtin_fmaf(a.mom_b, df[c], a.mom_a * mm[c]);
      store_stream<VEC>(a.mom + j, mm);
    }
    if constexpr (ATT) {
      if (a.a_out != nullptr) store_stream<VEC>(a.a_out + j, av);
    }
    if (++since == 16) {
#pragma unroll
      for (int i = 0; i < kStudySums; ++i) {
        acc64[i] += (double)acc[i];
        acc[i] = 0.0f;
      }
      since = 0;
    }
  }
  if (a_nan) amax = __builtin_nanf("");
  if (d_nan) dmax = __builtin_nanf("");
  constexpr int64_t kSlotStride = kStudyMaxBlocks + 1;
  double* p = partial + blockIdx.x;
#pragma unroll
  for (int i = 0; i < kStudySums; ++i) {
    const double r = block_reduce_sum<kStudyBlock>(acc64[i] + (double)acc[i], red);
    if (threadIdx.x == 0) p[i * kSlotStride] = r;
  }
  float m2[2] = {amax, dmax};
#pragma unroll
  for (int k = 0; k < 2; ++k) {
    float m = m2[k];
#pragma unroll
    for (int off = 32; off > 0; off >>= 1) {
      const float o = __shfl_down(m, off, 64);
      m = (m != m || o != o) ? __builtin_nanf("") : fmaxf(m, o);
    }
    if ((threadIdx.x & 63) == 0) mred[threadIdx.x >> 6] = m;
    __syncthreads();
    if (threadIdx.x == 0) {
      float mm = mred[0];
      for (int wv = 1; wv < kStudyBlock / 64; ++wv) {
        const float o = mred[wv];
        mm = (mm != mm || o != o) ? __builtin_nanf("") : fmaxf(mm, o);
      }
      p[(kStudySums + k) * kSlotStride] = (double)mm;
    }
    __syncthreads();
  }
}

constexpr int kStudyBurstThreads = 1024;
constexpr int kStudySlotBudget = 8;

template <bool ATT, int CM, bool L2, bool MOM = false>
__global__ __launch_bounds__(kStudyBurstThreads) void study_stats_burst_kernel(StudyArgs a, int f_real, float mu,
                                                                               float w_oldest, uint32_t nvec,
                                                                               double* __restrict__ partial) {
  static_assert(CM >= 1, "without a written stream there is nothing to burst");
  constexpr int VEC = 4;
  constexpr int kStudySlots = MOM ? kStudySlotBudget / 2 : kStudySlotBudget;
  constexpr int U = ((L2 && CM >= 2) || MOM) ? 1 : 2;
  using V = typename VecLoad<VEC>::T;
  __shared__ V stage[kStudySlots * kStudyBurstThreads];
  __shared__ V stage_mom[MOM ? kStudySlots * kStudyBurstThreads : 1];
  __shared__ double red[kStudyBurstThreads / 64];
  __shared__ float mred[kStudyBurstThreads / 64];
  float acc[kStudySums];
  double acc64[kStudySums];
#pragma unroll
  for (int i = 0; i < kStudySums; ++i) {
    acc[i] = 0.0f;
    acc64[i] = 0.0;
  }
  float amax = 0.0f, dmax = 0.0f;
  bool a_nan = false, d_nan = false;
  const float ff = (float)f_real;
  const uint32_t tid = threadIdx.x;
  const uint32_t span = gridDim.x * kStudyBurstThreads;
  const uint32_t iters = (nvec + span - 1) / span;
  const uint32_t first = blockIdx.x * kStudyBurstThreads + tid;
  for (uint32_t p0 = 0; p0 < iters; p0 += kStudySlots) {
    const uint32_t p1 = (p0 + kStudySlots < iters) ? p0 + kStudySlots : iters;
    for (uint32_t it = p0; it < p1; it += U) {
      float s[U][VEC], h[U][VEC], df[U][VEC], bz[U][VEC], pa[U][VEC], cv[U][VEC], ol[U][VEC], pp[U][VEC], oo[U][VEC];
      float mm[U][VEC];
      bool live[U];
#pragma unroll
      for (int u = 0; u < U; ++u) {
        const uint32_t v = (it + u) * span + first;
        live[u] = (it + u) < p1 && v < nvec;
        if (live[u]) {
          const int64_t j = (int64_t)v * VEC;
          load_stream<VEC>(a.s + j, s[u]);
          load_stream<VEC>(a.h + j, h[u]);
          load_stream<VEC>(a.def + j, df[u]);
          if constexpr (MOM) load_stream<VEC>(a.mom + j, mm[u]);
          if constexpr (ATT) load_stream<VEC>(a.byz + j, bz[u]);
          if constexpr (CM >= 2) {
            load_stream<VEC>(a.past + j, pa[u]);
            load_stream<VEC>(a.curv + j, cv[u]);
          }
          if constexpr (CM == 3) load_stream<VEC>(a.oldest + j, ol[u]);
          if constexpr (L2) {
            load_stream<VEC>(a.params + j, pp[u]);
            load_stream<VEC>(a.origin + j, oo[u]);
          }
        }
      }
#pragma unroll
      for (int u = 0; u < U; ++u) {
        if (!live[u]) continue;
#pragma unroll
        for (int c = 0; c < VEC; ++c) {
          float av = 0.0f;
          if constexpr (ATT) {
            float t = bz[u][c];
            for (int i = 1; i < f_real; ++i) t += bz[u][c];
            t = t / ff;
            av = t;
            amax = fmaxf(amax, __builtin_fabsf(t));
            a_nan |= (t != t);
            const float dd = bz[u][c] - t;
            float q = 0.0f;
            for (int i = 0; i < f_real; ++i) q = __builtin_fmaf(dd, dd, q);
            acc[12] += q;
          }
          dmax = fmaxf(dmax, __builtin_fabsf(df[u][c]));
          d_nan |= (df[u][c] != df[u][c]);
          acc[0] = __builtin_fmaf(s[u][c], s[u][c], acc[0]);
          acc[1] = __builtin_fmaf(s[u][c], h[u][c], acc[1]);
          acc[2] = __builtin_fmaf(s[u][c], df[u][c], acc[2]);
          acc[4] = __builtin_fmaf(h[u][c], h[u][c], acc[4]);
          acc[5] = __builtin_fmaf(h[u][c], df[u][c], acc[5]);
          acc[7] = __builtin_fmaf(df[u][c], df[u][c], acc[7]);
          if constexpr (ATT) {
            acc[3] = __builtin_fmaf(s[u][c], av, acc[3]);
            acc[6] = __builtin_fmaf(h[u][c], av, acc[6]);
            acc[8] = __builtin_fmaf(df[u][c], av, acc[8]);
            acc[9] = __builtin_fmaf(av, av, acc[9]);
          }
          if constexpr (CM >= 2) {
            acc[10] = __builtin_fmaf(s[u][c], pa[u][c], acc[10]);
            acc[11] = __builtin_fmaf(s[u][c], cv[u][c], acc[11]);
          }
          if constexpr (L2) {
            const float e = pp[u][c] - oo[u][c];
            acc[13] = __builtin_fmaf(e, e, acc[13]);
          }
          if constexpr (CM == 1) cv[u][c] = s[u][c];
          if constexpr (CM == 3) cv[u][c] = __builtin_fmaf(w_oldest, ol[u][c], 1.0f * cv[u][c]);
          if constexpr (CM >= 2) cv[u][c] = __builtin_fmaf(1.0f, s[u][c], mu * cv[u][c]);
        }
        V packed;
#pragma unroll
        for (int c = 0; c < VEC; ++c) packed[c] = cv[u][c];
        stage[(it + u - p0) * kStudyBurstThreads + tid] = packed;
        if constexpr (MOM) {
#pragma unroll
          for (int c = 0; c < VEC; ++c) packed[c] = __builtin_fmaf(a.mom_b, df[u][c], a.mom_a * mm[u][c]);
          stage_mom[(it + u - p0) * kStudyBurstThreads + tid] = packed;
        }
      }
    }
#pragma unroll
    for (int i = 0; i < kStudySums; ++i) {
      acc64[i] += (double)acc[i];
      acc[i] = 0.0f;
    }
    __syncthreads();
    for (uint32_t it = p0; it < p1; ++it) {
      const uint32_t v = it * span + first;
      if (v < nvec) {
        __builtin_nontemporal_store(stage[(it - p0) * kStudyBurstThreads + tid], reinterpret_cast<V*>(a.curv + (int64_t)v * VEC));
        if constexpr (MOM)
          __builtin_nontemporal_store(stage_mom[(it - p0) * kStudyBurstThreads + tid], reinterpret_cast<V*>(a.mom + (int64_t)v * VEC));
      }
    }
  }
  if (a_nan) amax = __builtin_nanf("");
  if (d_nan) dmax = __builtin_nanf("");
  constexpr int64_t kSlotStride = kStudyMaxBlocks + 1;
  double* p = partial + blockIdx.x;
#pragma unroll
  for (int i = 0; i < kStudySums; ++i) {
    const double r = block_reduce_sum<kStudyBurstThreads>(acc64[i], red);
    if (threadIdx.x == 0) p[i * kSlotStride] = r;
  }
  float m2[2] = {amax, dmax};
#pragma unroll
  for (int k = 0; k < 2; ++k) {
    float m = m2[k];
#pragma unroll
    for (int off = 32; off > 0; off >>= 1) {
      const float o = __shfl_down(m, off, 64);
      m = (m != m || o != o) ? __builtin_nanf("") : fmaxf(m, o);
    }
    if ((threadIdx.x & 63) == 0) mred[threadIdx.x >> 6] = m;
    __syncthreads();
    if (threadIdx.x == 0) {
      float mm = mred[0];
      for (int wv = 1; wv < kStudyBurstThreads / 64; ++wv) {
        const float o = mred[wv];
        mm = (mm != mm || o != o) ? __builtin_nanf("") : fmaxf(mm, o);
      }
      p[(kStudySums + k) * kSlotStride] = (double)mm;
    }
    __syncthreads();
  }
}

__global__ __launch_bounds__(64) void study_finish_kernel(const double* __restrict__ partial, int nparts,
                                                          double* __restrict__ out) {
  const int slot = blockIdx.x, lane = threadIdx.x;
  if (slot == 0 && lane >= 23 && lane < BM_STUDY_SLOTS) out[lane] = 0.0;
  double tot = 0.0;
  bool nan = false;
  const bool is_max = slot >= kStudySums;
  for (int b = lane; b < nparts; b += 64) {
    const double v = partial[(int64_t)slot * (kStudyMaxBlocks + 1) + b];
    if (is_max) {
      nan |= (v != v);
      tot = v > tot ? v : tot;
    } else {
      tot += v;
    }
  }
#pragma unroll
  for (int off = 32; off > 0; off >>= 1) {
    const double o = __shfl_down(tot, off, 64);
    if (is_max) {
      tot = o > tot ? o : tot;
      nan |= (bool)__shfl_down((int)nan, off, 64);
    } else {
      tot += o;
    }
  }
  if (lane != 0) return;
  if (is_max) {
    out[20 + (slot - kStudySums)] = nan ? __builtin_nan("") : tot;
    return;
  }
  if (slot < 10) {
    int k = 0;
    for (int r = 0; r < 4; ++r)
      for (int c = r; c < 4; ++c) {
        if (k == slot) {
          out[r * 4 + c] = tot;
          out[c * 4 + r] = tot;
        }
        ++k;
      }
    if (slot == 9) out[18] = tot;
  } else if (slot == 10) {
    out[16] = tot;
  } else if (slot == 11) {
    out[17] = tot;
  } else if (slot == 12) {
    out[19] = tot;
  } else {
    out[22] = tot;
  }
}

template <bool ATT, int CM, bool L2>
static int launch_study_vec(const StudyArgs& a, int vec, int f_real, float mu, float w, int64_t n, int grid,
                            double* partial, hipStream_t s) {
  if (vec == 4)
    hipLaunchKernelGGL((study_stats_kernel<ATT, CM, L2, 4>), dim3(grid), dim3(kStudyBlock), 0, s, a, f_real, mu, w, n, partial);
  else if (vec == 2)
    hipLaunchKernelGGL((study_stats_kernel<ATT, CM, L2, 2>), dim3(grid), dim3(kStudyBlock), 0, s, a, f_real, mu, w, n, partial);
  else
    hipLaunchKernelGGL((study_stats_kernel<ATT, CM, L2, 1>), dim3(grid), dim3(kStudyBlock), 0, s, a, f_real, mu, w, n, partial);
  BM_LAUNCH_CHECK();
  return 0;
}

template <bool ATT, bool L2>
static int launch_study_cm(const StudyArgs& a, int cm, int vec, int f_real, float mu, float w, int64_t n, int grid,
                           double* partial, hipStream_t s) {
  switch (cm) {
    case 0: return launch_study_vec<ATT, 0, L2>(a, vec, f_real, mu, w, n, grid, partial, s);
    case 1: return launch_study_vec<ATT, 1, L2>(a, vec, f_real, mu, w, n, grid, partial, s);
    case 2: return launch_study_vec<ATT, 2, L2>(a, vec, f_real, mu, w, n, grid, partial, s);
    default: return launch_study_vec<ATT, 3, L2>(a, vec, f_real, mu, w, n, grid, partial, s);
  }
}

template <bool ATT, bool L2, bool MOM>
static int launch_study_burst_mom(const StudyArgs& a, int cm, int f_real, float mu, float w, int64_t n, int grid,
                                  double* partial, hipStream_t s) {
  const uint32_t nv = (uint32_t)n;
  if (cm == 1)
    hipLaunchKernelGGL((study_stats_burst_kernel<ATT, 1, L2, MOM>), dim3(grid), dim3(kStudyBurstThreads), 0, s, a, f_real, mu, w, nv, partial);
  else if (cm == 2)
    hipLaunchKernelGGL((study_stats_burst_kernel<ATT, 2, L2, MOM>), dim3(grid), dim3(kStudyBurstThreads), 0, s, a, f_real, mu, w, nv, partial);
  else
    hipLaunchKernelGGL((study_stats_burst_kernel<ATT, 3, L2, MOM>), dim3(grid), dim3(kStudyBurstThreads), 0, s, a, f_real, mu, w, nv, partial);
  BM_LAUNCH_CHECK();
  return 0;
}
template <bool ATT, bool L2>
static int launch_study_burst(const StudyArgs& a, int cm, int f_real, float mu, float w, int64_t n, int grid,
                              double* partial, hipStream_t s) {
  return a.mom != nullptr ? launch_study_burst_mom<ATT, L2, true>(a, cm, f_real, mu, w, n, grid, partial, s)
                          : launch_study_burst_mom<ATT, L2, false>(a, cm, f_real, mu, w, n, grid, partial, s);
}

static bool study_burst_eligible(const StudyArgs& a, int cm, int vec, int64_t nvec) {
  const int threshold = tuning().study_burst;
  if (threshold <= 0 || cm < 1 || vec != 4 || a.a_out != nullptr || nvec >= ((int64_t)1 << 30)) return false;
  return nvec >= (int64_t)threshold * compute_units() * kStudyBurstThreads;
}

static int launch_study(const StudyArgs& a, bool att, bool l2, int cm, int vec, int f_real, float mu, float w, int64_t n,
                        int grid, double* partial, hipStream_t s) {
  if (att) return l2 ? launch_study_cm<true, true>(a, cm, vec, f_real, mu, w, n, grid, partial, s)
                     : launch_study_cm<true, false>(a, cm, vec, f_real, mu, w, n, grid, partial, s);
  return l2 ? launch_study_cm<false, true>(a, cm, vec, f_real, mu, w, n, grid, partial, s)
            : launch_study_cm<false, false>(a, cm, vec, f_real, mu, w, n, grid, partial, s);
}

static_assert(kStudyCaps.sets() == kStudyMaxBlocks + 1, "bm_study_stats: partial sets and slot stride differ");
int64_t study_workspace_bytes() { return (int64_t)kStudyCaps.sets() * kStudyPartial * (int64_t)sizeof(double); }

}

extern "C" int bm_study_stats(const float* sampled_avg, const float* honest_avg, const float* defense, const float* byz,
                              int f_real, float* attack_avg_out, const float* past_newest, float* curv,
                              const float* past_oldest, int curv_mode, float mu, float oldest_weight,
                              const float* params, const float* origin, int64_t d, double* out, void* ws, void* stream) {
  return bm_study_stats_update(sampled_avg, honest_avg, defense, byz, f_real, attack_avg_out, past_newest, curv, past_oldest,
                               curv_mode, mu, oldest_weight, params, origin, nullptr, 0.0f, 0.0f, d, out, ws, stream);
}

extern "C" int bm_study_stats_update(const float* sampled_avg, const float* honest_avg, const float* defense,
                                     const float* byz, int f_real, float* attack_avg_out, const float* past_newest,
                                     float* curv, const float* past_oldest, int curv_mode, float mu, float oldest_weight,
                                     const float* params, const float* origin, float* update_momentum, float momentum_mu,
                                     float one_minus_damp, int64_t d, double* out, void* ws, void* stream) {
  using namespace bm;
  const bool att = f_real > 0, l2 = params != nullptr && origin != nullptr;
  if (out == nullptr || ws == nullptr || d < 0 || f_real < 0 || f_real > BM_MAX_ROWS || curv_mode < 0 || curv_mode > 3 ||
      (d > 0 && (sampled_avg == nullptr || honest_avg == nullptr || defense == nullptr || (att && byz == nullptr) ||
                 (curv_mode >= 1 && curv == nullptr) || (curv_mode >= 2 && past_newest == nullptr) ||
// ... 30 lines not shown
```

### byzantinemomentum_amd/sharded.py

```python

import ctypes
import math
import warnings

import torch
import torch.distributed as dist

from . import _lib

__all__ = ["shard_bounds", "owned_workers", "Shards", "ShardedAggregator", "HipBackend", "NativeComm"]


class Shards(list):

  def __init__(self, rows=(), d_total=None):
    super().__init__(rows)
    self.d_total = None if d_total is None else int(d_total)


def shard_bounds(d, world_size, rank, align=64):
  per = -(-d // world_size)
  per = -(-per // align) * align
  lo = min(rank * per, d)
  hi = min(lo + per, d)
  return lo, hi


def owned_workers(n, world_size, rank):
  return list(range(rank, n, world_size))


class NativeComm:

  def __init__(self, group=None, vote=None):
    lib = _lib.load()
    if not lib.bm_comm_available():
      raise RuntimeError("RCCL could not be bound by libbm_gar.so")
    world, rank = dist.get_world_size(group), dist.get_rank(group)
    ident, failure = [None], None
    if rank == 0:
      try:
        buf = ctypes.create_string_buffer(128)
        _lib.check(lib.bm_comm_unique_id(buf), "bm_comm_unique_id")
        ident[0] = buf.raw
      except Exception as err:
        failure = err
    if vote is not None:
      if not vote(failure is None):
        raise RuntimeError(f"bm_comm_unique_id failed on rank 0: {failure}" if failure is not None else
                           "bm_comm_unique_id failed on rank 0")
    elif failure is not None:
      raise failure
    dist.broadcast_object_list(ident, src=dist.get_global_rank(group, 0) if group is not None else 0, group=group)
    handle = ctypes.c_void_p()
    _lib.check(lib.bm_comm_init(ctypes.byref(handle), world, rank, ctypes.c_char_p(ident[0])), "bm_comm_init")
    self.handle = handle
    self.world_size = world

  def close(self):
    if self.handle is not None and self.handle.value:
      _lib.load().bm_comm_destroy(self.handle)
      self.handle = None

  def __del__(self):
    try:
      self.close()
    except Exception:
      pass


class HipBackend:

  capabilities = frozenset((
    "step_worker", "momentum_stats_colwise", "momentum_stats_sqdist", "stack_stats_colwise", "stack_stats_sqdist",
    "device_search", "attack_ranking_device", "bulyan_pass2_eval", "order_pair", "colwise_eval", "sqdist2", "anticge"))

  def __init__(self):
    from . import gars, stats
    self.gars = gars
    self.stats = stats


  def pairwise_sqdist(self, gradients, d_total=None):
    return self.gars.pairwise_sqdist(gradients, d_total)

  def rank(self, sq, n, f, m, mode):
    order, _ = self.gars.rank_from_sqdist(sq, n, f, m, mode)
    return order

  def selected_mean(self, gradients, order, m):
    return self.gars.selected_mean(gradients, order, m)

  def bulyan_pass2(self, gradients, order, f, m):
    return self.gars.bulyan_pass2(gradients, order, f, m)

  def colwise(self, rule, gradients, f):
    return getattr(self.gars, rule)(gradients, f=f) if rule != "median" else self.gars.median(gradients)

  def aksel_sqdist(self, gradients):
    return self.gars.aksel_sqdist(gradients)[:len(gradients)]

  def argsort(self, keys, n):
    return self.gars.stable_argsort(keys, n)

  def brute_select(self, dist_host, n, f):
    return self.gars.brute_select_host(dist_host, n, f)

  def brute_select_device(self, sq, n, f):
    return self.gars.brute_select_device(sq, n, f)

  def sharded_rule(self, name, comm, gradients, f, m, d_total=None):
    gars = self.gars
    n, d, device = gars._validate(gradients)
    lib = _lib.load()
    out = torch.empty(d, dtype=torch.float32, device=device)
    nbytes = lib.bm_sharded_workspace_bytes(n, d)
    ws = gars._Scratch.get(device, "ws_sharded", nbytes=int(nbytes))
    fn = lib.bm_sharded_krum if name == "krum" else lib.bm_sharded_bulyan
    with torch.cuda.device(device):
      _lib.check(fn(comm.handle if comm is not None else None, _lib.pointer_table(gradients), n, d,
                    int(d_total) if d_total is not None else d, f, m, gars._ptr(out), None, gars._ptr(ws), gars._stream(device)), "bm_sharded_" + name)
    return out

  def index_tensor(self, indices, like):
    return torch.tensor(indices, dtype=torch.int32, device=like.device)

  def sum_over_ranks(self, agg, value):
    t = torch.tensor([float(value)], dtype=torch.float64, device=torch.device("cuda", torch.cuda.current_device()))
    return int(agg.all_reduce_sum(t).item())


  def stack_stats(self, samples, scale=None, attack="empire", want_avg=True, direction=False):
    return self.stats.stack_stats_async(samples, scale=scale, attack=attack, want_avg=want_avg, direction=direction)

  def momentum_stats(self, sampled, buffers, mu, omd, factors, scale, attack, direction=False):
    return self.stats.momentum_stats(sampled, buffers, mu, omd, factors, scale, attack, direction)

  def momentum_stats_colwise(self, *args, **kwargs):
    return self.stats.momentum_stats_colwise(*args, **kwargs)

  def stack_stats_colwise(self, *args, **kwargs):
    return self.stats.stack_stats_colwise(*args, **kwargs)

  def stack_stats_sqdist(self, *args, **kwargs):
    return self.stats.stack_stats_sqdist(*args, **kwargs)

  def momentum_stats_sqdist(self, *args, **kwargs):
    return self.stats.momentum_stats_sqdist(*args, **kwargs)

  def multi_fma3(self, outs, ps, qs, a, b, p_scale=None):
    return self.stats.multi_fma3(outs, ps, qs, a, b, p_scale)

  @property
  def device_search_rules(self):
    return self.stats.DEVICE_SEARCH_RULES

  def attack_search_device(self, *args, **kwargs):
    return self.stats.attack_search_device(*args, **kwargs)

  def device_search(self, device, evals, negative=False):
    return self.stats.DeviceSearch(device, evals, negative)

  def multi_scale(self, ys, factors):
    return self.stats.multi_scale(ys, factors)

  def row_sqnorms(self, gradients):
    return self.stats.row_sqnorms(gradients).contiguous()

  def clip_factors_from_sq(self, sq, k, clip):
    return self.stats.clip_factors_from_sq(sq, k, clip)

  def study_stats(self, *args, **kwargs):
    return self.stats.study_stats(*args, **kwargs)

  def anticge(self, honests, f_decl, reduce):
    byz, _, scal = self.stats.anticge_sum(honests, f_decl, reduce(self.row_sqnorms(honests)))
    reduce(scal[:1])
    return self.stats.anticge_scale(byz, scal)

  def colwise_eval_supported(self, rule, n):
    return self.stats.colwise_eval_supported(rule, n)

  def colwise_eval(self, *args, **kwargs):
    return self.stats.colwise_eval(*args, **kwargs)

  def sqdist2(self, a, b):
    return self.stats.sqdist2(a, b)

  def attack_ranking_device(self, *args, **kwargs):
    return self.stats.attack_ranking_device(*args, **kwargs)

  def bulyan_pass2_eval_supported(self, n, f, m, d=0):
    return self.stats.bulyan_pass2_eval_supported(n, f, m, d)

  def bulyan_pass2_eval(self, *args, **kwargs):
    return self.stats.bulyan_pass2_eval(*args, **kwargs)

  def order_pair_supported(self, h):
    return self.stats.order_pair_supported(h)

  def order_pair(self, rows, il, ih):
    return self.stats.order_pair(rows, il, ih)

  def study_dots(self, core, extra):
    return self.stats.study_dots(core, extra)

  def step_worker(self, comm, *args, **kwargs):
    return self.stats.step_worker(comm, *args, **kwargs)


def _anticge_sum_torch(backend, local, f_decl, sq):
  h = len(local)
  maxpos = h - f_decl
  keys = torch.where(torch.isfinite(sq[:h]), sq[:h], torch.full_like(sq[:h], math.inf))
  order = backend.argsort(keys, h)
  ranked = order[:h].tolist()
  attack = local[ranked[0]].clone()
  for i in ranked[:maxpos]:
    attack.add_(local[i])
  return attack, order, torch.stack([attack.double().pow(2).sum(), keys[ranked[maxpos]]])


def _anticge_scale_torch(vec, scal):
  attnorm, byznorm = scal.sqrt().float().tolist()
  if attnorm > 0:
# ... 250 lines not shown
```

### byzantinemomentum_amd/stats.py

```python

import ctypes
import os
import math

import torch

from . import _lib
from . import gars

__all__ = ["compute_avg_dev_max", "stack_stats_async", "study_dots", "study_stats", "multi_axpby", "row_sqnorms", "momentum_stats", "momentum_stats_colwise", "momentum_stats_sqdist", "stack_stats_colwise", "stack_stats_sqdist",
           "multi_fma3", "clip_factors", "clip_factors_from_sq", "multi_scale", "clip_gradients", "l2_distance",
           "step_worker", "anticge_sum", "anticge_scale", "anticge_attack"]

_ptr = gars._ptr


def _opt(t):
  return _ptr(t) if t is not None else None


def _require_scalar_on(t, device, message):
  if not (isinstance(t, torch.Tensor) and t.is_cuda and t.device == device and t.dtype == torch.float64
          and t.numel() >= 1 and t.is_contiguous()):
    raise gars.GarInputError(message)


def _require_ext(ext, h):
  if not (isinstance(ext, torch.Tensor) and ext.is_cuda and ext.dtype == torch.float64 and ext.is_contiguous()
          and tuple(ext.shape) == (h + 2, h + 2)):
    raise gars.GarInputError(f"ext must be a contiguous float64 device tensor of shape ({h + 2}, {h + 2})")


def _attack_id(attack, direction):
  kind = _lib.ATTACK_LITTLE if attack == "little" else _lib.ATTACK_EMPIRE
  return kind | (_lib.ATTACK_DIRECTION if direction else 0)


def stack_stats_async(samples, scale=None, attack="empire", want_avg=True, direction=False):
  k, d, device = gars._validate(samples)
  lib = _lib.load()
  avg = torch.empty(d, dtype=torch.float32, device=device) if want_avg else None
  scaled = torch.empty(d, dtype=torch.float32, device=device) if scale is not None else None
  out3 = torch.empty(3, dtype=torch.float64, device=device)
  ws = gars._workspace(device, _lib.WS_STATS, k, d, "ws_stats")
  with torch.cuda.device(device):
    _lib.check(lib.bm_stack_stats(_lib.pointer_table(samples), k, d, _opt(avg), _opt(scaled),
                                  ctypes.c_float(scale if scale is not None else 0.0),
                                  _attack_id(attack, direction), _ptr(out3),
                                  _ptr(ws), gars._stream(device)), "bm_stack_stats")
  if scale is not None:
    return avg, out3, scaled
  return avg, out3


def compute_avg_dev_max(samples):
  if len(samples) == 0:
    return None, math.nan, math.nan, math.nan
  avg, out3 = stack_stats_async(samples)
  norm2, dev2, amax = out3.tolist()
  k = len(samples)
  norm_dev = math.sqrt(dev2 / (k - 1)) if k >= 2 else math.nan
  return avg, math.sqrt(norm2), norm_dev, amax


def study_dots(core, extra=()):
  core = list(core)
  extra = list(extra)
  nc, d, device = gars._validate(core)
  if extra:
    gars._validate(extra + [core[0]])
  lib = _lib.load()
  out = torch.empty(nc * nc + len(extra), dtype=torch.float64, device=device)
  ws = gars._workspace(device, _lib.WS_DOT, 1, d, "ws_dot")
  with torch.cuda.device(device):
    _lib.check(lib.bm_multi_dot(_lib.pointer_table(core), nc,
                                _lib.pointer_table(extra) if extra else None, len(extra), d, _ptr(out),
                                _ptr(ws), gars._stream(device)), "bm_multi_dot")
  return out[:nc * nc].view(nc, nc), out[nc * nc:]


_EVAL_OPS = {"trmean": _lib.OP_TRMEAN, "phocas": _lib.OP_PHOCAS, "meamed": _lib.OP_MEAMED, "median": _lib.OP_MEDIAN}


def colwise_eval_supported(rule, n):
  return rule in _EVAL_OPS and bool(_lib.load().bm_colwise_eval_supported(_EVAL_OPS[rule], n))


def colwise_eval(rule, honests, copies, f, h_avg, direction, t):
  honests = list(honests)
  h, d, device = gars._validate(honests)
  gars._validate([h_avg, direction] + honests[:1])
  lib = _lib.load()
  out = torch.empty(1, dtype=torch.float64, device=device)
# ... 147 lines not shown
                                  _ptr(scal), _ptr(ws), gars._stream(device)), "bm_anticge_sum")
  return out, order, scal


def anticge_scale(vec, scal):
  _, d, device = gars._validate([vec])
  _require_scalar_on(scal, device, "anticge_scale: scal must be a contiguous float64 tensor on the vector's device")
  if scal.numel() < 2:
    raise gars.GarInputError("anticge_scale: scal must hold the two scalars anticge_sum left")
  lib = _lib.load()
  gars.invalidate_rank_cache()
  with torch.cuda.device(device):
    _lib.check(lib.bm_anticge_scale(_ptr(vec), d, _ptr(scal), gars._stream(device)), "bm_anticge_scale")
  return vec


def anticge_attack(grad_honests, f_decl, f_real, **kwargs):
  grad_honests = list(grad_honests)
  h, d, device = gars._validate(grad_honests)
  if f_real <= 0:
    return []
  if f_real > f_decl:
    return [torch.full_like(grad_honests[0], math.nan)] * f_real
  byz, _, scal = anticge_sum(grad_honests, f_decl, row_sqnorms(grad_honests).contiguous())
  return [anticge_scale(byz, scal)] * f_real


def multi_axpby(ys, xs, a, b):
  k, d, device = gars._validate(list(ys))
  gars._validate(list(xs) + [ys[0]])
  if len(xs) != k:
    raise gars.GarInputError("multi_axpby needs as many x as y vectors")
  lib = _lib.load()
  gars.invalidate_rank_cache()
  with torch.cuda.device(device):
    _lib.check(lib.bm_multi_axpby(_lib.pointer_table(ys), _lib.pointer_table(xs), k, d,
                                  ctypes.c_float(a), ctypes.c_float(b), gars._stream(device)),
               "bm_multi_axpby")


def momentum_stats(sampled, buffers, mu, one_minus_damp, clip_factors_dev=None, attack_scale=None, attack="empire",
                   direction=False):
  ks, d, device = gars._validate(list(sampled))
  h = gars._validate(list(buffers) + [sampled[0]])[0] - 1
  if h < 1 or ks < h:
    raise gars.GarInputError("momentum_stats needs 1 <= len(buffers) <= len(sampled)")
  lib = _lib.load()
  s_avg = torch.empty(d, dtype=torch.float32, device=device)
  h_avg = torch.empty(d, dtype=torch.float32, device=device)
  byz = torch.empty(d, dtype=torch.float32, device=device) if attack_scale is not None else None
  out6 = torch.empty(6, dtype=torch.float64, device=device)
  ws = gars._workspace(device, _lib.WS_STEP, 1, d, "ws_step")
  gars.invalidate_rank_cache()
  with torch.cuda.device(device):
    _lib.check(lib.bm_momentum_stats(
      _lib.pointer_table(sampled), ks, _lib.pointer_table(buffers), h, d, ctypes.c_float(mu),
      ctypes.c_float(one_minus_damp), _opt(clip_factors_dev), _ptr(s_avg), _ptr(h_avg), _opt(byz),
      ctypes.c_float(attack_scale if attack_scale is not None else 0.0),
      _attack_id(attack, direction), _ptr(out6), _ptr(ws),
      gars._stream(device)), "bm_momentum_stats")
  return s_avg, h_avg, byz, out6


def momentum_stats_colwise(sampled, buffers, mu, one_minus_damp, clip_factors_dev, attack_scale, attack, rule, f, n_byz):
  ks, d, device = gars._validate(list(sampled))
  h = gars._validate(list(buffers) + [sampled[0]])[0] - 1
  if h < 1 or ks < h or n_byz < 1:
    raise gars.GarInputError("momentum_stats_colwise needs 1 <= len(buffers) <= len(sampled) and n_byz >= 1")
  lib = _lib.load()
  s_avg, h_avg, byz, defense = (torch.empty(d, dtype=torch.float32, device=device) for _ in range(4))
  out6 = torch.empty(6, dtype=torch.float64, device=device)
  ws = gars._workspace(device, _lib.WS_STEP, 1, d, "ws_step")
  gars.invalidate_rank_cache()
  with torch.cuda.device(device):
    _lib.check(lib.bm_momentum_stats_colwise(
      _lib.pointer_table(sampled), ks, _lib.pointer_table(buffers), h, d, ctypes.c_float(mu),
      ctypes.c_float(one_minus_damp), _opt(clip_factors_dev),
      _ptr(s_avg), _ptr(h_avg), _ptr(byz), ctypes.c_float(attack_scale), _attack_id(attack, False),
      _EVAL_OPS[rule], int(f), int(n_byz), _ptr(defense), _ptr(out6), _ptr(ws), gars._stream(device)),
      "bm_momentum_stats_colwise")
  return s_avg, h_avg, byz, defense, out6


def momentum_stats_sqdist(sampled, buffers, mu, one_minus_damp, clip_factors_dev, attack_scale, attack, n_byz,
                          d_total=None):
  ks, d, device = gars._validate(list(sampled))
  h = gars._validate(list(buffers) + [sampled[0]])[0] - 1
  if h < 1 or ks < h or n_byz < 1 or h + n_byz > _lib.MAX_ROWS:
    raise gars.GarInputError("momentum_stats_sqdist needs 1 <= len(buffers) <= len(sampled), n_byz >= 1, at most 64 rows")
  n = h + n_byz
  lib = _lib.load()
  s_avg, h_avg, byz = (torch.empty(d, dtype=torch.float32, device=device) for _ in range(3))
  sq = torch.empty((n, n), dtype=torch.float64, device=device)
  out6 = torch.empty(6, dtype=torch.float64, device=device)
  ws = gars._workspace(device, _lib.WS_STEP, 1, d, "ws_step")
  ws_pair = gars._workspace(device, _lib.WS_PAIRWISE, n, d, "ws_pair")
  gars.invalidate_rank_cache()
  with torch.cuda.device(device):
    _lib.check(lib.bm_momentum_stats_sqdist(
      _lib.pointer_table(sampled), ks, _lib.pointer_table(buffers), h, d, d if d_total is None else int(d_total),
      ctypes.c_float(mu), ctypes.c_float(one_minus_damp), _opt(clip_factors_dev), _ptr(s_avg), _ptr(h_avg), _ptr(byz),
      ctypes.c_float(attack_scale), _attack_id(attack, False), int(n_byz), _ptr(sq), _ptr(out6), _ptr(ws), _ptr(ws_pair),
      gars._stream(device)), "bm_momentum_stats_sqdist")
  return s_avg, h_avg, byz, sq, out6


def stack_stats_colwise(rows, attack_scale, attack, rule, f, n_byz):
  k, d, device = gars._validate(list(rows))
  if n_byz < 1:
    raise gars.GarInputError("stack_stats_colwise needs n_byz >= 1")
  lib = _lib.load()
  avg, byz, defense = (torch.empty(d, dtype=torch.float32, device=device) for _ in range(3))
  out6 = torch.empty(6, dtype=torch.float64, device=device)
  ws = gars._workspace(device, _lib.WS_STEP, 1, d, "ws_step")
  with torch.cuda.device(device):
    _lib.check(lib.bm_stack_stats_colwise(_lib.pointer_table(rows), k, d, _ptr(avg), _ptr(byz),
                                          ctypes.c_float(attack_scale), _attack_id(attack, False), _EVAL_OPS[rule],
                                          int(f), int(n_byz), _ptr(defense), _ptr(out6), _ptr(ws),
                                          gars._stream(device)), "bm_stack_stats_colwise")
  return avg, byz, defense, out6


def stack_stats_sqdist(rows, attack_scale, attack, n_byz, d_total=None):
  k, d, device = gars._validate(list(rows))
  if n_byz < 1 or k + n_byz > _lib.MAX_ROWS:
    raise gars.GarInputError("stack_stats_sqdist needs n_byz >= 1 and at most 64 rows")
  n = k + n_byz
  lib = _lib.load()
  avg, byz = (torch.empty(d, dtype=torch.float32, device=device) for _ in range(2))
  sq = torch.empty((n, n), dtype=torch.float64, device=device)
  out6 = torch.empty(6, dtype=torch.float64, device=device)
  ws = gars._workspace(device, _lib.WS_STEP, 1, d, "ws_step")
  ws_pair = gars._workspace(device, _lib.WS_PAIRWISE, n, d, "ws_pair")
  with torch.cuda.device(device):
    _lib.check(lib.bm_stack_stats_sqdist(_lib.pointer_table(rows), k, d, d if d_total is None else int(d_total),
                                         _ptr(avg), _ptr(byz), ctypes.c_float(attack_scale), _attack_id(attack, False),
                                         int(n_byz), _ptr(sq), _ptr(out6), _ptr(ws), _ptr(ws_pair),
                                         gars._stream(device)), "bm_stack_stats_sqdist")
  return avg, byz, sq, out6


def multi_fma3(outs, ps, qs, a, b, p_scale_dev=None):
  outs, ps, qs = list(outs), list(ps), list(qs)
  k, d, device = gars._validate(outs)
  gars._validate(ps + [outs[0]])
  gars._validate(qs + [outs[0]])
  if len(ps) != k or len(qs) != k:
    raise gars.GarInputError("multi_fma3 needs as many p and q as out vectors")
  lib = _lib.load()
  gars.invalidate_rank_cache()
  scale = _opt(p_scale_dev)
  with torch.cuda.device(device):
    if isinstance(b, torch.Tensor):
      _require_scalar_on(b, device, "multi_fma3: a tensor b must be a contiguous float64 tensor on the vectors' device")
      _lib.check(lib.bm_multi_fma3_bdev(_lib.pointer_table(outs), _lib.pointer_table(ps), _lib.pointer_table(qs), k, d,
                                        ctypes.c_float(a), _ptr(b), scale, gars._stream(device)), "bm_multi_fma3_bdev")
    else:
      _lib.check(lib.bm_multi_fma3(_lib.pointer_table(outs), _lib.pointer_table(ps), _lib.pointer_table(qs), k, d,
                                   ctypes.c_float(a), ctypes.c_float(b), scale, gars._stream(device)), "bm_multi_fma3")


DEVICE_SEARCH_RULES = ("krum", "average")


def attack_search_device(ext, h, k, f, rule, evals=16, negative=False, m=None):
  if rule not in DEVICE_SEARCH_RULES:
# ... 88 lines not shown
```

### byzantinemomentum_amd/step.py

```python

import collections
import math
from typing import NamedTuple, Optional

import torch

from . import _lib, linesearch

__all__ = ["AggregationStep"]

_RULES = ("krum", "bulyan", "median", "trmean", "phocas", "meamed", "aksel", "brute", "average", "cge")
_COLWISE = ("median", "trmean", "phocas", "meamed")
_DISTANCE = ("krum", "bulyan")
MAX_PAST = 4096


class StepPlan(NamedTuple):
  only_m: bool
  analytic: bool
  first_pass: str
  search: Optional[str]
  device_cursor: bool
  single_call: bool
  capabilities: frozenset
# ... 186 lines not shown
      return found
    ext = self._fetch(sq)
    factor, self.last_search = linesearch.attack_line_search(ext, self.h, self.f_real, self.f_decl, self.gar, **args)
    return factor

  def _written_objective(self, rule, h_avg, direction):
    ops = self.ops

    def evaluate(t):
      cand = torch.empty_like(h_avg)
      ops.multi_fma3([cand], [h_avg], [direction], 1.0, t)
      out = rule(cand, t)
      if "sqdist2" in self.plan.capabilities:
        return ops.sqdist2(out, h_avg)
      return ops.pairwise_sqdist([out, h_avg])[0, 1].reshape(1)
    return evaluate

  def _generic_objective(self, honests, h_avg, direction, on_device=False):
    return self._written_objective(lambda cand, t: self._aggregate(list(honests) + [cand] * self.f_real), h_avg, direction)

  def _colwise_objective(self, honests, h_avg, direction, on_device=False):
    ops, k = self.ops, self.f_real
    if not ops.colwise_eval_supported(self.gar, self.h + k):
      return self._generic_objective(honests, h_avg, direction)
    return lambda t: ops.colwise_eval(self.gar, honests, k, self.f_decl, h_avg, direction, t)

  def _median_objective(self, honests, h_avg, direction, on_device=False):
    ops, agg, h, k = self.ops, self.agg, self.h, self.f_real
    n, caps = h + k, self.plan.capabilities
    if "order_pair" in caps and ops.order_pair_supported(h):
      lo, hi = ops.order_pair(honests, (n - 1) // 2 - k, (n - 1) // 2)
    else:
      lo = agg.median(list(honests) + [torch.full_like(h_avg, -math.inf)] * k)
      hi = agg.median(list(honests) + [torch.full_like(h_avg, math.inf)] * k)
    if "colwise_eval" in caps:
      whole = not self.gar_args and ops.colwise_eval_supported("median", n)
      if ops.colwise_eval_supported("median", 3):
        return lambda t: ops.colwise_eval("median", [lo, hi], 1, 0, h_avg, direction, t)
      if whole:
        return lambda t: ops.colwise_eval("median", honests, k, self.f_decl, h_avg, direction, t)
    return self._written_objective(lambda cand, t: agg.median([cand, lo, hi]), h_avg, direction)

  def _bulyan_objective(self, honests, h_avg, direction, on_device):
    ops, h, k, f = self.ops, self.h, self.f_real, self.f_decl
    n = h + k
    m = self.gar_args.get("m") or n - f - 2
    sq_dev = self._unit_sqdist(honests, h_avg, direction)
    ext = None if on_device else self._fetch(sq_dev)

    def ranking(t):
      if on_device:
        return ops.attack_ranking_device(sq_dev, h, k, f, "bulyan", t, m)
      order = linesearch.attack_ranking(ext, h, k, f, "bulyan", t, m)
      return ops.index_tensor(order + [0] * (64 - n), h_avg)

    if "bulyan_pass2_eval" in self.plan.capabilities and ops.bulyan_pass2_eval_supported(n, f, m, h_avg.shape[0]):
      return lambda t: ops.bulyan_pass2_eval(honests, k, ranking(t), f, m, h_avg, direction, t)
    return self._written_objective(lambda cand, t: ops.bulyan_pass2(list(honests) + [cand] * k, ranking(t), f, m),
                                   h_avg, direction)

  def nesterov_lookahead(self, params, lr, worker=None):
    mom = (self.buffers[worker] if self.buffers is not None else None) if worker is not None else self.server_momentum
    if mom is not None:
      self.ops.multi_fma3([params], [params], [mom], 1.0, -(self.mu * lr))
    return params

  def run(self, grad_sampleds, params=None, origin=None):
    ops, agg, h = self.ops, self.agg, self.h
    sampled = list(grad_sampleds)
    if getattr(grad_sampleds, "d_total", None) is not None:
      from .sharded import Shards
      sampled = Shards(sampled, d_total=grad_sampleds.d_total)
    ks = len(sampled)
    if ks < h:
      raise ValueError(f"{ks} sampled gradients for {h} honest workers")
    omd = 1.0 - self.damp
    if self.single_call:
      return self._run_single_call(sampled, ks, omd, params, origin)
    factors = None
    if self.clip is not None:
      sq = ops.row_sqnorms(sampled)
      agg.all_reduce_sum(sq)
      factors = ops.clip_factors_from_sq(sq, ks, self.clip)
    fused_defense, fused_sq = None, None
    first_pass = self.plan.first_pass
    searched = first_pass == "direction"
    anticge = self.attack == "anticge"
    scale = None if anticge else (1.0 if searched else self.factor)
    if self.momentum_at == "worker":
      if self.buffers is None:
        self.buffers = self._new_rows(h, sampled[0], zero=True)
      if first_pass == "rule":
        s_avg, h_avg, byz, fused_defense, out6 = ops.momentum_stats_colwise(
          sampled, self.buffers, self.mu, omd, factors, self.factor, self.attack, self.gar, self.f_decl, self.f_real)
      elif first_pass == "sqdist":
        s_avg, h_avg, byz, fused_sq, out6 = ops.momentum_stats_sqdist(
          sampled, self.buffers, self.mu, omd, factors, self.factor, self.attack, self.f_real,
          d_total=agg._total_of(sampled))
      else:
        s_avg, h_avg, byz, out6 = ops.momentum_stats(sampled, self.buffers, self.mu, omd, factors, scale, self.attack,
                                                     direction=searched)
      honests = self.buffers
      s_out3, h_out3 = out6[:3], out6[3:]
    else:
      if factors is not None:
        ops.multi_scale(sampled, factors)
      if self.momentum_at == "server":
        mom = self.server_momentum if self.server_momentum is not None else torch.zeros_like(sampled[0])
        honests = self._new_rows(h, sampled[0])
        ops.multi_fma3(honests, sampled[:h], [mom] * h, omd, self.mu)
      else:
        honests = sampled[:h]
      if ks != h and first_pass in ("rule", "sqdist"):
        first_pass = "plain"
      if first_pass == "rule":
        h_avg, byz, fused_defense, o6 = ops.stack_stats_colwise(honests, self.factor, self.attack, self.gar, self.f_decl,
                                                                self.f_real)
        h_out3 = o6[3:]
      elif first_pass == "sqdist":
        h_avg, byz, fused_sq, o6 = ops.stack_stats_sqdist(honests, self.factor, self.attack, self.f_real,
                                                          d_total=agg._total_of(sampled))
        h_out3 = o6[3:]
      else:
        h_avg, h_out3, *byz = ops.stack_stats(honests, scale=scale, attack=self.attack, direction=searched)
        byz = byz[0] if byz else None
      if self.momentum_at == "update" and ks == h:
        s_avg, s_out3 = h_avg, h_out3
      else:
        s_avg, s_out3 = ops.stack_stats(sampled)
    if anticge and self.f_real > 0:
      byz = agg.anticge(honests, self.f_decl, self.f_real)[0]
    if searched and self.f_real > 0:
      direction = byz
      factor = self._search_factor(honests, h_avg, direction)
      self.last_factor = factor
      byz = torch.empty_like(h_avg)
      ops.multi_fma3([byz], [h_avg], [direction], 1.0, factor)
    attacks = [byz] * self.f_real
    self.last_byzantine = byz if self.f_real > 0 else None
    if fused_defense is not None:
      defense = fused_defense
    elif fused_sq is not None:
      defense = agg.rule_from_sq(self.gar, honests + attacks, fused_sq, self.f_decl, self.gar_args.get("m"))
    else:
      defense = self._aggregate(honests + attacks)
    if self.momentum_at == "server":
      self.server_momentum = defense
      self._update = defense
    elif self.momentum_at == "update":
      if self.server_momentum is None:
        self.server_momentum = torch.zeros_like(defense)
      self._update = self.server_momentum
    else:
      self._update = defense
    count = len(self.pasts) if self.nb_past > 0 else 0
    mode = 0
    if self.nb_past > 0:
      if self._curv is None:
        self._curv = torch.empty_like(s_avg)
      mode = 1 if count == 0 else (3 if count == self.nb_past else 2)
    has_l2 = params is not None and origin is not None
    study = ops.study_stats(s_avg, h_avg, defense, byz if self.f_real > 0 else None, self.f_real,
                            past_newest=self.pasts[0] if count > 0 else None, curv=self._curv,
                            past_oldest=self.pasts[-1] if mode == 3 else None, curv_mode=mode, mu=self.mu,
                            oldest_weight=-(self.mu ** (self.nb_past - 1)) if self.nb_past > 0 else 0.0,
                            params=params if has_l2 else None, origin=origin if has_l2 else None,
                            **(dict(update_momentum=self.server_momentum, update_mu=self.mu, update_omd=omd)
                               if self.momentum_at == "update" else {}))
    self._pending = dict(s=s_out3, h=h_out3, study=study, npast=2 if count > 0 else 0,
                         prev_s2=self._prev_s2 if count > 0 else None, has_l2=has_l2, ks=ks, floats=None)
    if self.nb_past > 0:
      self.pasts.appendleft(s_avg)
      self._prev_s2 = s_out3[:1]
    return defense

  def _run_single_call(self, sampled, ks, omd, params, origin):
    h = self.h
    if self.buffers is None:
      self.buffers = self._new_rows(h, sampled[0], zero=True)
    count = len(self.pasts) if self.nb_past > 0 else 0
    if self.nb_past > 0 and self._curv is None:
      self._curv = torch.empty_like(sampled[0])
    full = count == self.nb_past and count > 0
    defense, s_avg, h_avg, byz, stats = self.ops.step_worker(
      self.agg.native, sampled, self.buffers, self.n, self.f_decl, self.f_real, self.gar, self.gar_args.get("m"),
      self.mu, omd, self.clip, self.attack, self.factor, self.nb_past, count,
      self.pasts[0] if count > 0 else None, self._curv, self.pasts[-1] if full else None, params, origin,
      d_total=self.agg._total_of(sampled))
    self._update = defense
    self.last_byzantine = byz
    self._pending = dict(packed=stats, prev=self._prev_stats if count > 0 else None, npast=2 if count > 0 else 0,
                         has_l2=params is not None and origin is not None, ks=ks,
                         floats=None)
    if self.nb_past > 0:
      self.pasts.appendleft(s_avg)
      self._prev_stats = stats
    return defense

  def update_gradient(self):
    return self._update


  def _exchange(self, pend):
    s3, h3, st, prev = pend["s"], pend["h"], pend["study"], pend["prev_s2"]
    last = [prev] if prev is not None else []
    if not self.agg.collective:
      flat = torch.cat([s3, h3, st] + last).tolist()
      s3, h3, st, last = flat[0:3], flat[3:6], flat[6:6 + _lib.STUDY_SLOTS], flat[6 + _lib.STUDY_SLOTS:]
      sums = s3[_lib.OUT3_SUMS] + h3[_lib.OUT3_SUMS] + st[_lib.STUDY_SUMS] + st[_lib.STUDY_L2] + last
      maxes = s3[_lib.OUT3_MAX] + h3[_lib.OUT3_MAX] + st[_lib.STUDY_MAXES]
    else:
      sums, maxes = self.agg.exchange(
        torch.cat([s3[_lib.OUT3_SUMS], h3[_lib.OUT3_SUMS], st[_lib.STUDY_SUMS], st[_lib.STUDY_L2]] + last),
        torch.cat([s3[_lib.OUT3_MAX], h3[_lib.OUT3_MAX], st[_lib.STUDY_MAXES]]))
      ns = int(sums.numel())
      flat = torch.cat([sums, maxes]).tolist()
      sums, maxes = flat[:ns], flat[ns:]
    s2, sd, h2, hd = sums[0:4]
    st = sums[4:24]
    gram, (ex0, ex1), (a2, ad) = st[_lib.STUDY_GRAM], st[_lib.STUDY_EX], st[_lib.STUDY_ATTACK]
    smax, hmax, amax, dmax = maxes
    return _StudyRecord(s2, sd, smax, h2, hd, hmax, a2, ad, amax, gram[4 * 2 + 2], dmax, sums[24], gram, ex0, ex1,
                        sums[25] if prev is not None else math.nan)

  @staticmethod
  def _unpack(pend):
    vec = pend["packed"] if pend["prev"] is None else torch.cat([pend["packed"], pend["prev"][:1]])
    v = vec.tolist()
    L = _lib
    return _StudyRecord(v[L.STEP_S2], v[L.STEP_SD], v[L.STEP_SMAX], v[L.STEP_H2], v[L.STEP_HD], v[L.STEP_HMAX],
                        v[L.STEP_A2], v[L.STEP_AD], v[L.STEP_AMAX], v[L.STEP_D2], v[L.STEP_DMAX], v[L.STEP_L2],
                        v[L.STEP_GRAM], v[L.STEP_EX.start], v[L.STEP_EX.start + 1],
                        v[len(pend["packed"])] if pend["prev"] is not None else math.nan)

  def _study_floats(self, rec, pend):
    nan = math.nan
    att, k_s, k_h, k_a = self.f_real > 0, pend["ks"], self.h, self.f_real
    g = rec.gram

    def dev(x, k):
      return math.sqrt(x / (k - 1)) if k >= 2 else nan

    def cos(i, j):
      if not att and 3 in (i, j):
        return nan
      return g[4 * i + j] / math.sqrt(g[5 * i]) / math.sqrt(g[5 * j])

    past = pend["npast"] > 0
    return {
      "l2_origin": math.sqrt(rec.l2) if pend["has_l2"] else nan,
      "sampled_norm_avg": math.sqrt(rec.s2), "sampled_norm_dev": dev(rec.sd, k_s), "sampled_norm_max": rec.smax,
# ... 20 lines not shown
```

### include/bm_gar.h

```cpp
#ifndef BM_GAR_H
#define BM_GAR_H

#include <stdint.h>

#ifdef __cplusplus
extern "C" {
#endif

#define BM_MAX_ROWS 64
#define BM_EINVAL   (-100000)
#define BM_ENOCOMM  (-100001)
#define BM_ECOMM    (-100002)

enum bm_colwise_op {
  BM_OP_MEDIAN = 0,
  BM_OP_TRMEAN = 1,
  BM_OP_PHOCAS = 2,
  BM_OP_MEAMED = 3
};

int bm_abi_version(void);
int bm_tuning_set(const char* name, int value);

const char* bm_error_string(int code);
// ... 6 lines not shown
  BM_WS_AKSEL    = 1,
  BM_WS_STATS    = 2,
  BM_WS_DOT      = 3,
  BM_WS_STEP     = 4,
  BM_WS_STUDY    = 5
};
int64_t bm_workspace_bytes(int kind, int n, int64_t d);

int bm_pairwise_sqdist(const float* const* rows, int n, int64_t d,
                       double* sq_nxn, void* ws, void* stream);

int bm_pairwise_sqdist_shard(const float* const* rows, int n, int64_t d, int64_t d_total,
                             double* sq_nxn, void* ws, void* stream);

enum bm_rank_mode { BM_RANK_KRUM = 0, BM_RANK_BULYAN = 1 };
int bm_krum_rank(const double* sq_nxn, int n, int f, int m, int mode,
                 int32_t* order_out, double* scores_out, void* stream);

int bm_pairwise_rank(const float* const* rows, int n, int64_t d, int64_t d_total, int f, int m, int mode,
                     double* sq_nxn, int32_t* order_out, double* scores_out, void* ws, void* stream);

int bm_selected_mean(const float* const* rows, int n, const int32_t* idx, int m,
                     int64_t d, float* out, void* stream);

int bm_bulyan_pass2(const float* const* rows, int n, const int32_t* order, int f, int m,
                    int64_t d, float* out, void* stream);

int bm_aksel_pass1(const float* const* rows, int n, int64_t d, float* median_out,
                   double* sq_out, void* ws, void* stream);

enum bm_attack_kind { BM_ATTACK_EMPIRE = 0, BM_ATTACK_LITTLE = 1,
                      BM_ATTACK_DIRECTION = 16 };
int bm_stack_stats(const float* const* rows, int k, int64_t d, float* avg_out,
                   float* scaled_out, float scale, int attack_kind, double* out3, void* ws,
                   void* stream);

int bm_multi_dot(const float* const* core, int nc, const float* const* extra, int ne,
                 int64_t d, double* out, void* ws, void* stream);

#define BM_STUDY_SLOTS 32
int bm_study_stats(const float* sampled_avg, const float* honest_avg, const float* defense, const float* byz,
                   int f_real, float* attack_avg_out, const float* past_newest, float* curv,
                   const float* past_oldest, int curv_mode, float mu, float oldest_weight, const float* params,
                   const float* origin, int64_t d, double* out, void* ws, void* stream);
int bm_study_stats_update(const float* sampled_avg, const float* honest_avg, const float* defense, const float* byz,
                          int f_real, float* attack_avg_out, const float* past_newest, float* curv,
                          const float* past_oldest, int curv_mode, float mu, float oldest_weight, const float* params,
                          const float* origin, float* update_momentum, float momentum_mu, float one_minus_damp,
                          int64_t d, double* out, void* ws, void* stream);

int bm_row_sqnorms(const float* const* rows, int k, int64_t d, double* sq_out, void* ws, void* stream);

int bm_stable_argsort(const double* keys, int n, int32_t* order_out, void* stream);

int64_t bm_anticge_workspace_bytes(int64_t d);
int bm_anticge_sum(const float* const* rows, int h, int64_t d, int f_decl, const double* row_sq, float* sum_out,
                   int32_t* order_out, double* scal_out, void* ws, void* stream);
int bm_anticge_scale(float* vec, int64_t d, const double* scal, void* stream);

int bm_multi_axpby(float* const* y, const float* const* x, int k, int64_t d,
                   float a, float b, void* stream);

int bm_momentum_stats(const float* const* sampled, int ks, float* const* buffers, int h, int64_t d,
                      float mu, float one_minus_damp, const float* clip_factors, float* sampled_avg,
                      float* honest_avg, float* byz_out, float scale, int attack_kind, double* out6,
                      void* ws, void* stream);

int bm_momentum_stats_colwise(const float* const* sampled, int ks, float* const* buffers, int h, int64_t d,
                              float mu, float one_minus_damp, const float* clip_factors, float* sampled_avg,
                              float* honest_avg, float* byz_out, float scale, int attack_kind, int rule_op,
                              int rule_f, int n_byz, float* defense_out, double* out6, void* ws, void* stream);

int bm_momentum_stats_sqdist(const float* const* sampled, int ks, float* const* buffers, int h, int64_t d,
                             int64_t d_total, float mu, float one_minus_damp, const float* clip_factors,
                             float* sampled_avg, float* honest_avg, float* byz_out, float scale, int attack_kind,
                             int n_byz, double* sq_nxn, double* out6, void* ws, void* ws_pair, void* stream);

int bm_stack_stats_colwise(const float* const* rows, int k, int64_t d, float* avg_out, float* byz_out, float scale,
                           int attack_kind, int rule_op, int rule_f, int n_byz, float* defense_out, double* out6,
                           void* ws, void* stream);
int bm_stack_stats_sqdist(const float* const* rows, int k, int64_t d, int64_t d_total, float* avg_out, float* byz_out,
                          float scale, int attack_kind, int n_byz, double* sq_nxn, double* out6, void* ws,
                          void* ws_pair, void* stream);

int bm_multi_fma3(float* const* out, const float* const* p, const float* const* q, int k, int64_t d,
                  float a, float b, const float* p_scale, void* stream);
int bm_multi_fma3_bdev(float* const* out, const float* const* p, const float* const* q, int k, int64_t d,
                       float a, const double* b_dev, const float* p_scale, void* stream);

int bm_clip_factors(const double* row_sq, int k, float clip, float* factors_out, void* stream);
int bm_multi_scale(float* const* y, int k, int64_t d, const float* factors, void* stream);

int bm_brute_select(const double* dist_nxn, int n, int f, int32_t* sel_out);
int bm_brute_select_device(const double* sq_nxn, int n, int f, int32_t* sel_out, int32_t* status, void* stream);

typedef struct bm_comm bm_comm;

int bm_comm_available(void);
int bm_comm_unique_id(void* id128);
int bm_comm_init(bm_comm** out, int nranks, int rank, const void* id128);
int bm_comm_destroy(bm_comm* comm);
int bm_comm_size(const bm_comm* comm);

int bm_allreduce_sum_f64(bm_comm* comm, double* buf, int64_t count, void* stream);
int bm_allgather_f32(bm_comm* comm, const float* mine, float* all, int64_t count_per_rank, void* stream);

int64_t bm_sharded_workspace_bytes(int n, int64_t d_local);
int bm_sharded_krum(bm_comm* comm, const float* const* rows, int n, int64_t d_local, int64_t d_total, int f, int m,
                    float* out_local, int32_t* order_out, void* ws, void* stream);
int bm_sharded_bulyan(bm_comm* comm, const float* const* rows, int n, int64_t d_local, int64_t d_total, int f, int m,
                      float* out_local, int32_t* order_out, void* ws, void* stream);

double* bm_sharded_sq_slot(void* ws);
void* bm_sharded_pair_workspace(void* ws);
int bm_sharded_rule_from_sq(bm_comm* comm, int rule, const float* const* rows, int n, int64_t d_local, int f, int m,
                            float* out_local, int32_t* order_out, void* ws, void* stream);

enum bm_step_rule { BM_RULE_KRUM = 0, BM_RULE_BULYAN = 1, BM_RULE_MEDIAN = 2, BM_RULE_TRMEAN = 3,
                    BM_RULE_PHOCAS = 4, BM_RULE_MEAMED = 5,
                    BM_RULE_BRUTE = 6, BM_RULE_AVERAGE = 7  };
typedef struct bm_step_params {
  int32_t n, f_decl, f_real;
  int32_t ks;
  int32_t rule;
  int32_t m;
  int32_t attack_kind;
  int32_t nb_past;
  int32_t past_count;
  float attack_scale;
  float mu, one_minus_damp;
  float clip;
  float oldest_weight;
} bm_step_params;
int bm_step_stats_count(void);
int64_t bm_step_workspace_bytes(int n, int64_t d_local);
int bm_step_worker(bm_comm* comm, const bm_step_params* p, const float* const* sampled, float* const* buffers,
                   int64_t d, int64_t d_total , float* defense_out,
                   float* sampled_avg_out, float* honest_avg_out, float* byz_out,
                   float* attack_avg_out, const float* past_newest, float* curv, const float* past_oldest,
                   const float* params, const float* origin, double* stats_out, void* ws, void* stream);

int bm_colwise_eval_supported(int op, int n);
int64_t bm_colwise_eval_workspace_bytes(void);
int bm_colwise_eval(int op, const float* const* honests, int h, int copies, int64_t d, int f, const float* avg,
                    const float* dir, float t, double* out, void* ws, void* stream);
int bm_colwise_eval_tdev(int op, const float* const* honests, int h, int copies, int64_t d, int f, const float* avg,
                         const float* dir, const double* t_dev, double* out, void* ws, void* stream);

typedef struct bm_search {
  double best_x, best_y;
  double probe;
  double step, ratio;
  int32_t phase;
  int32_t evaluations;
  int32_t awaiting;
  int32_t reserved;
} bm_search;
int bm_search_begin(bm_search* c, double start, double delta, double ratio);
int bm_search_propose(bm_search* c, double* x_out);
int bm_search_report(bm_search* c, double y);
int bm_attack_objective(const double* ext, int h, int k, int f, int rule, int m, double t, double* y_out,
                        int32_t* sel_out, int32_t* count_out);
int bm_attack_line_search(const double* ext, int h, int k, int f, int rule, int m, int evals, int negative,
                          double* factor_out, double* trace_out);
int bm_attack_line_search_device(const double* ext, int h, int k, int f, int rule, int m, int evals, int negative,
                                 double* out, void* stream);
// ... 18 lines not shown
```

Before: 5505.

## Fuse study statistics pass into the momentum/colwise rule kernel

Adds a STUDY template variant of the fused momentum+stats+rule kernel that also computes the study statistics per element (past/curvature, L2 distance to origin, optional server momentum update). It accumulates per-block study partials, and a combined finish kernel reduces them. The training step calls this fused entry when the plan advertises the capability, so the separate study_stats pass, which re-read s_avg, h_avg, defense and byz from HBM, is skipped. In exchange the kernel carries more live registers and extra LDS, which may lower occupancy, and a new template instantiation is added.

```diff
diff --git a/byzantinemomentum_amd/_lib.py b/byzantinemomentum_amd/_lib.py
--- a/byzantinemomentum_amd/_lib.py
+++ b/byzantinemomentum_amd/_lib.py
@@ -72,6 +72,15 @@
   "bm_stack_stats_colwise": (ctypes.c_int, [_c_float_pp, ctypes.c_int, ctypes.c_int64, ctypes.c_void_p, ctypes.c_void_p,
                                             ctypes.c_float, ctypes.c_int, ctypes.c_int, ctypes.c_int, ctypes.c_int,
                                             ctypes.c_void_p, ctypes.c_void_p, ctypes.c_void_p, ctypes.c_void_p]),
+  "bm_momentum_stats_colwise_study": (ctypes.c_int, [_c_float_pp, ctypes.c_int, _c_float_pp, ctypes.c_int, ctypes.c_int64,
+                                                     ctypes.c_float, ctypes.c_float, ctypes.c_void_p, ctypes.c_void_p,
+                                                     ctypes.c_void_p, ctypes.c_void_p, ctypes.c_float, ctypes.c_int,
+                                                     ctypes.c_int, ctypes.c_int, ctypes.c_int, ctypes.c_void_p,
+                                                     ctypes.c_void_p, ctypes.c_void_p, ctypes.c_void_p, ctypes.c_void_p,
+                                                     ctypes.c_int, ctypes.c_float, ctypes.c_float, ctypes.c_void_p,
+                                                     ctypes.c_void_p, ctypes.c_void_p, ctypes.c_void_p, ctypes.c_float,
+                                                     ctypes.c_float, ctypes.c_void_p, ctypes.c_void_p, ctypes.c_void_p,
+                                                     ctypes.c_void_p]),
   "bm_stack_stats_sqdist": (ctypes.c_int, [_c_float_pp, ctypes.c_int, ctypes.c_int64, ctypes.c_int64, ctypes.c_void_p,
                                            ctypes.c_void_p, ctypes.c_float, ctypes.c_int, ctypes.c_int, ctypes.c_void_p,
                                            ctypes.c_void_p, ctypes.c_void_p, ctypes.c_void_p, ctypes.c_void_p]),
diff --git a/byzantinemomentum_amd/csrc/api.cpp b/byzantinemomentum_amd/csrc/api.cpp
--- a/byzantinemomentum_amd/csrc/api.cpp
+++ b/byzantinemomentum_amd/csrc/api.cpp
@@ -22,7 +22,8 @@
                            env_int("BM_PAIR_PLANES", 0), env_int("BM_PAIR_DITHER", 0), env_double("BM_PAIR_TAU", 2e-3),
                            env_int("BM_STUDY_BURST", 8), env_int("BM_STEP_STAGGER_US", 0),
                            env_int("BM_GRAM_STEADY", 1), env_int("BM_BULYAN_SHORT", 1),
-                           env_int("BM_PAIR_LOAD_NT", 1), env_int("BM_RANK_ALGO", 0), env_int("BM_COL_WIDE", 1), env_int("BM_BRUTE_BUDGET", 0)};
+                           env_int("BM_PAIR_LOAD_NT", 1), env_int("BM_RANK_ALGO", 0), env_int("BM_COL_WIDE", 1), env_int("BM_BRUTE_BUDGET", 0),
+                           env_int("BM_STEP_FUSE_STUDY", 1)};
   return t;
 }
 const Tuning& tuning() { return tuning_mutable(); }
@@ -40,7 +41,8 @@
       {"BM_PAIR_DITHER", &t.pair_dither}, {"BM_STUDY_BURST", &t.study_burst},
       {"BM_STEP_STAGGER_US", &t.step_stagger_us}, {"BM_GRAM_STEADY", &t.gram_steady},
       {"BM_BULYAN_SHORT", &t.bulyan_short}, {"BM_PAIR_LOAD_NT", &t.pair_load_nt},
-      {"BM_RANK_ALGO", &t.rank_algo}, {"BM_COL_WIDE", &t.col_wide}, {"BM_BRUTE_BUDGET", &t.brute_budget}};
+      {"BM_RANK_ALGO", &t.rank_algo}, {"BM_COL_WIDE", &t.col_wide}, {"BM_BRUTE_BUDGET", &t.brute_budget},
+      {"BM_STEP_FUSE_STUDY", &t.step_fuse_study}};
   for (const auto& k : knobs)
     if (strcmp(name, k.key) == 0) {
       *k.slot = value;
diff --git a/byzantinemomentum_amd/csrc/bm_common.h b/byzantinemomentum_amd/csrc/bm_common.h
--- a/byzantinemomentum_amd/csrc/bm_common.h
+++ b/byzantinemomentum_amd/csrc/bm_common.h
@@ -241,6 +241,7 @@
   int rank_algo;
   int col_wide;
   int brute_budget;
+  int step_fuse_study;
 };
 const Tuning& tuning();
 Tuning& tuning_mutable();
diff --git a/byzantinemomentum_amd/csrc/step.hip b/byzantinemomentum_amd/csrc/step.hip
--- a/byzantinemomentum_amd/csrc/step.hip
+++ b/byzantinemomentum_amd/csrc/step.hip
@@ -1,5 +1,7 @@
+#include <stddef.h>
 #include "colwise_kernels.h"
 #include "gram_split.h"
+#include "study_body.h"
 
 namespace bm {
 
@@ -65,16 +67,79 @@
 typedef const float* __attribute__((address_space(4))) const* KargRowPtrs;
 constexpr int kStepBurstBlock = 512;
 
-template <int T, int VEC, bool EXACT, bool CLIP, bool BURST, int RULE = -1, int NB = 0, bool NOMOM = false>
+struct StudyRide {
+  const float* past;
+  float* curv;
+  const float* oldest;
+  const float* params;
+  const float* origin;
+  float* mom;
+  double* partial;
+  float mu, w_oldest, mom_a, mom_b;
+  int cm, l2, has_mom;
+  StudyRide advanced(int64_t by) const {
+    using bm::advanced;
+    StudyRide r = *this;
+    r.past = advanced(past, by);
+    r.curv = advanced(curv, by);
+    r.oldest = advanced(oldest, by);
+    r.params = advanced(params, by);
+    r.origin = advanced(origin, by);
+    r.mom = advanced(mom, by);
+    return r;
+  }
+};
+struct StepKernargs {
+  StepTable tab;
+  int ks_rt, h_rt;
+  uint32_t nvec;
+  float mu, omd;
+  const float* clipf;
+  float *s_avg_out, *h_avg_out, *byz_out;
+  float scale;
+  int attack_kind;
+  double* partial;
+  int rule_f;
+  float rule_inv_keep;
+  float* defense_out;
+  StudyRide ride;
+};
+constexpr int kRideSlot = (int)(offsetof(StepKernargs, ride) / 8);
+static_assert(offsetof(StepKernargs, ride) % 8 == 0 && offsetof(StudyRide, past) == 0 && offsetof(StudyRide, mom) == 40 &&
+                  offsetof(StudyRide, partial) == 48,
+              "first pass: the pointers of the study block are fetched as karg[kRideSlot + 0..6]");
+
+typedef const int __attribute__((address_space(4)))* KargInts;
+typedef const float __attribute__((address_space(4)))* KargFloats;
+#define BM_RIDE_INT(kbase, field) (((KargInts)(kbase))[(offsetof(StepKernargs, ride) + offsetof(StudyRide, field)) / 4])
+#define BM_RIDE_FLOAT(kbase, field) (((KargFloats)(kbase))[(offsetof(StepKernargs, ride) + offsetof(StudyRide, field)) / 4])
+
+template <int BLOCK>
+__device__ __forceinline__ double* study_sums_lds() {
+  __shared__ double sums[kStudySums * BLOCK];
+  return sums;
+}
+
+template <int T, int VEC, bool EXACT, bool CLIP, bool BURST, int RULE = -1, int NB = 0, bool NOMOM = false, bool STUDY = false>
 __global__ __launch_bounds__(BURST ? kStepBurstBlock : kStepBlock) void momentum_stats_kernel(
     StepTable tab, int ks_rt, int h_rt, uint32_t nvec, float mu, float omd, const float* __restrict__ clipf,
     float* __restrict__ s_avg_out, float* __restrict__ h_avg_out, float* __restrict__ byz_out, float scale,
-    int attack_kind, double* __restrict__ partial, int rule_f, float rule_inv_keep, float* __restrict__ defense_out) {
+    int attack_kind, double* __restrict__ partial, int rule_f, float rule_inv_keep, float* __restrict__ defense_out,
+    StudyRide ride) {
   static_assert(RULE < 0 || (EXACT && NB >= 1), "the fused rule needs the row count at compile time");
   static_assert(!NOMOM || (EXACT && !CLIP), "without buffers: same stack, clipped in place beforehand");
+  static_assert(!STUDY || (RULE >= 0 && VEC == 4), "the study block needs the defense: it rides along with the rule");
   constexpr int BLOCK = BURST ? kStepBurstBlock : kStepBlock;
   __shared__ double red[BLOCK / 64];
   __shared__ float mred[BLOCK / 64];
+  (void)ride;
+  double* study_sums = nullptr;
+  StudyMax study_max;
+  if constexpr (STUDY) {
+    study_sums = study_sums_lds<BLOCK>() + threadIdx.x;
+#pragma unroll
+    for (int i = 0; i < kStudySums; ++i) study_sums[i * BLOCK] = 0.0;
+  }
   const float fks = (float)(EXACT ? T : ks_rt), fh = (float)(EXACT ? T : h_rt);
   float n2s = 0.0f, dvs = 0.0f, mxs = 0.0f, n2h = 0.0f, dvh = 0.0f, mxh = 0.0f;
   bool nan_s = false, nan_h = false;
@@ -89,6 +154,7 @@
     const uint32_t off = v * (uint32_t)(VEC * sizeof(float));
     float g[T][VEC], b[T][VEC];
     float sa[VEC], ha[VEC], bz[VEC], df[VEC];
+    float pa[VEC] = {}, cv[VEC] = {}, ol[VEC] = {}, pp[VEC] = {}, oo[VEC] = {}, mm[VEC] = {};
     asm volatile("" : "+s"(kbase));
     int ks = T, h = T;
     if constexpr (!EXACT) {
@@ -103,6 +169,25 @@
         if (i < ks) load_stream_off<VEC>(karg[i], off, g[i]);
         if constexpr (!NOMOM) {
           if (i < h) load_stream_off<VEC>(karg[BM_MAX_ROWS + i], off, b[i]);
+        }
+      }
+      float study_acc[kStudySums] = {};
+      int ride_cm = 0, ride_l2 = 0, ride_mom = 0;
+      if constexpr (STUDY) {
+        ride_cm = BM_RIDE_INT(kbase, cm);
+        ride_l2 = BM_RIDE_INT(kbase, l2);
+        if constexpr (NOMOM) ride_mom = BM_RIDE_INT(kbase, has_mom);
+        if (ride_cm >= 2) {
+          load_stream_off<VEC>(karg[kRideSlot + 0], off, pa);
+          load_stream_off<VEC>(karg[kRideSlot + 1], off, cv);
+        }
+        if (ride_cm == 3) load_stream_off<VEC>(karg[kRideSlot + 2], off, ol);
+        if (ride_l2) {
+          load_stream_off<VEC>(karg[kRideSlot + 3], off, pp);
+          load_stream_off<VEC>(karg[kRideSlot + 4], off, oo);
+        }
+        if constexpr (NOMOM) {
+          if (ride_mom) load_stream_off<VEC>(karg[kRideSlot + 5], off, mm);
         }
       }
 #pragma unroll
@@ -138,6 +223,9 @@
             q = __builtin_fmaf(df, df, q);
           }
         dvs += q;
+        if constexpr (STUDY)
+          study_past_element(ride_cm, ride_l2 != 0, s, pa[c], cv[c], ol[c], pp[c], oo[c], BM_RIDE_FLOAT(kbase, mu),
+                             BM_RIDE_FLOAT(kbase, w_oldest), study_acc);
         float t = b[0][c];
 #pragma unroll
         for (int i = 1; i < T; ++i)
@@ -164,6 +252,16 @@
           for (int i = 0; i < NB; ++i) x[T + i] = bz[c];
           df[c] = column_rule<T + NB, RULE, BLOCK>(x, rule_f, rule_inv_keep, nullptr);
         }
+        if constexpr (STUDY) {
+          study_core_element<true>(s, t, df[c], bz[c], NB, (float)NB, study_acc, study_max);
+          if constexpr (NOMOM) {
+            if (ride_mom) mm[c] = study_momentum_element(BM_RIDE_FLOAT(kbase, mom_a), BM_RIDE_FLOAT(kbase, mom_b), df[c], mm[c]);
+          }
+        }
+      }
+      if constexpr (STUDY) {
+#pragma unroll
+        for (int i = 0; i < kStudySums; ++i) study_sums[i * BLOCK] += (double)study_acc[i];
       }
     }
     if constexpr (BURST) __syncthreads();
@@ -179,9 +277,29 @@
       if (h_avg_out != nullptr) store_stream_off<VEC>(h_avg_out, off, ha);
       if (byz_out != nullptr) store_stream_off<VEC>(byz_out, off, bz);
       if constexpr (RULE >= 0) store_stream_off<VEC>(defense_out, off, df);
+      if constexpr (STUDY) {
+        if (BM_RIDE_INT(kbase, cm) >= 1) store_stream_off<VEC>(const_cast<float*>(karg[kRideSlot + 1]), off, cv);
+        if constexpr (NOMOM) {
+          if (BM_RIDE_INT(kbase, has_mom)) store_stream_off<VEC>(const_cast<float*>(karg[kRideSlot + 5]), off, mm);
+        }
+      }
     }
   }
   store_step_partials<BLOCK>(n2s, dvs, mxs, n2h, dvh, mxh, nan_s, nan_h, red, mred, partial);
+  if constexpr (STUDY) {
+    double* p = reinterpret_cast<double*>(const_cast<float*>(((KargRowPtrs)kbase)[kRideSlot + 6])) + (int64_t)blockIdx.x * kStudyPartial;
+#pragma unroll
+    for (int i = 0; i < kStudySums; ++i) {
+      const double r = block_reduce_sum<BLOCK>(study_sums[i * BLOCK], red);
+      if (threadIdx.x == 0) p[i] = r;
+    }
+    const float ra = block_reduce_absmax<BLOCK>(absmax_value(study_max.attack), mred);
+    const float rd = block_reduce_absmax<BLOCK>(absmax_value(study_max.defense), mred);
+    if (threadIdx.x == 0) {
+      p[kStudySums] = (double)ra;
+      p[kStudySums + 1] = (double)rd;
+    }
+  }
 }
 
 constexpr int kSgRowBytes = 272;
@@ -518,8 +636,7 @@
 }
 
 constexpr int kFinishThreads = 256;
-__global__ __launch_bounds__(kFinishThreads) void step_finish_kernel(const double* __restrict__ partial, int nparts,
-                                                                     double* __restrict__ out6) {
+__device__ __forceinline__ void step_finish_body(const double* __restrict__ partial, int nparts, double* __restrict__ out6) {
   __shared__ double red[kFinishThreads / 64][8];
   const int lane = threadIdx.x & 63, wave = threadIdx.x >> 6;
   double s[6] = {0.0, 0.0, 0.0, 0.0, 0.0, 0.0};
@@ -573,6 +690,20 @@
     out6[3] = s[3];
     out6[4] = s[4];
     out6[5] = nan5 ? __builtin_nan("") : s[5];
+  }
+}
+__global__ __launch_bounds__(kFinishThreads) void step_finish_kernel(const double* __restrict__ partial, int nparts,
+                                                                     double* __restrict__ out6) {
+  step_finish_body(partial, nparts, out6);
+}
+__global__ __launch_bounds__(kFinishThreads) void step_study_finish_kernel(const double* __restrict__ partial,
+                                                                           const double* __restrict__ study_partial,
+                                                                           int nparts, double* __restrict__ out6,
+                                                                           double* __restrict__ study_out) {
+  if (blockIdx.x == 0) {
+    step_finish_body(partial, nparts, out6);
+  } else if (threadIdx.x < 64) {
+    study_finish_slot(study_partial, 1, kStudyPartial, nparts, (int)blockIdx.x - 1, threadIdx.x, study_out);
   }
 }
 
@@ -592,18 +723,22 @@
   int rule_f = 0;
   float rule_inv_keep = 0.0f;
   float* defense = nullptr;
+  bool study = false;
+  StudyRide ride{};
   StepArgs moved(int64_t by) const {
     StepArgs a = *this;
     a.tab = tab.advanced(by);
     a.s_avg = advanced(s_avg, by);
     a.h_avg = advanced(h_avg, by);
     a.byz = advanced(byz, by);
+    a.ride = ride.advanced(by);
     return a;
   }
   StepArgs at(Span& sp) const {
     StepArgs a = moved(sp.first);
     a.nvec = sp.count;
     a.partial = partial + (int64_t)sp.part * 6;
+    a.ride.partial = advanced(ride.partial, (int64_t)sp.part * kStudyPartial);
     a.grid_io = &sp.grid;
     return a;
   }
@@ -632,19 +767,19 @@
 template <class Kernel>
 static int launch_momentum_stats_kernel(Kernel kernel, int grid, int block, const StepArgs& a) {
   hipLaunchKernelGGL(kernel, dim3(grid), dim3(block), 0, a.s, a.tab, a.ks, a.h, (uint32_t)a.nvec, a.mu, a.omd, a.clipf,
-                     a.s_avg, a.h_avg, a.byz, a.scale, a.kind, a.partial, a.rule_f, a.rule_inv_keep, a.defense);
+                     a.s_avg, a.h_avg, a.byz, a.scale, a.kind, a.partial, a.rule_f, a.rule_inv_keep, a.defense, a.ride);
   BM_LAUNCH_CHECK();
   return 0;
 }
 
-template <int T, int VEC, bool EXACT, bool CLIP, int RULE = -1, int NB = 0, bool NOMOM = false>
+template <int T, int VEC, bool EXACT, bool CLIP, int RULE = -1, int NB = 0, bool NOMOM = false, bool STUDY = false>
 static int launch_momentum_stats_form(const StepArgs& a) {
   const int cus = compute_units();
   if (burst_ready(a.nvec, cus) && cus < *a.grid_io) {
     *a.grid_io = cus;
-    return launch_momentum_stats_kernel(momentum_stats_kernel<T, VEC, EXACT, CLIP, true, RULE, NB, NOMOM>, cus, kStepBurstBlock, a);
-  }
-  return launch_momentum_stats_kernel(momentum_stats_kernel<T, VEC, EXACT, CLIP, false, RULE, NB, NOMOM>, *a.grid_io, kStepBlock, a);
+    return launch_momentum_stats_kernel(momentum_stats_kernel<T, VEC, EXACT, CLIP, true, RULE, NB, NOMOM, STUDY>, cus, kStepBurstBlock, a);
+  }
+  return launch_momentum_stats_kernel(momentum_stats_kernel<T, VEC, EXACT, CLIP, false, RULE, NB, NOMOM, STUDY>, *a.grid_io, kStepBlock, a);
 }
 
 template <int T, int VEC>
@@ -750,11 +885,21 @@
   factors[i] = (norm > (double)clip) ? (float)((double)clip / norm) : 1.0f;
 }
 
+constexpr bool study_instance(int t, int rule, bool nomom, bool clip) {
+  if (nomom) return true;
+  if (t == 20) return rule != BM_OP_PHOCAS && rule != BM_OP_MEAMED;
+  return !(rule == BM_OP_PHOCAS && clip);
+}
 template <int T, int RULE, int NB, bool CLIP, bool NOMOM = false>
 static int launch_fused_rule(StepArgs a) {
   constexpr int N = T + NB;
   const int keep = (RULE == BM_OP_TRMEAN) ? (N - 2 * a.rule_f) : ((RULE == BM_OP_PHOCAS || RULE == BM_OP_MEAMED) ? (N - a.rule_f) : N);
   a.rule_inv_keep = 1.0f / (float)(keep > 0 ? keep : 1);
+  if constexpr (study_instance(T, RULE, NOMOM, CLIP)) {
+    if (a.study) return launch_momentum_stats_form<T, 4, true, CLIP, RULE, NB, NOMOM, true>(a);
+  } else {
+    if (a.study) return BM_EINVAL;
+  }
   return launch_momentum_stats_form<T, 4, true, CLIP, RULE, NB, NOMOM>(a);
 }
 
@@ -826,7 +971,8 @@
   block[b3_tri_index(i, j, nrows)] = acc;
 }
 
-int64_t step_workspace_bytes() { return (int64_t)(kStepMaxBlocks + 1) * 6 * (int64_t)sizeof(double); }
+int64_t step_workspace_bytes() { return (int64_t)(kStepMaxBlocks + 1) * (6 + kStudyPartial) * (int64_t)sizeof(double); }
+static double* step_study_partials(void* ws) { return static_cast<double*>(ws) + (int64_t)(kStepMaxBlocks + 1) * 6; }
 
 static int momentum_stats_impl(const float* const* sampled, int ks, float* const* buffers, int h, int64_t d, float mu,
                                float one_minus_damp, const float* clip_factors, float* sampled_avg, float* honest_avg,
@@ -1003,6 +1149,114 @@
   return bm_colwise(rule_op, all, n, d, rule_f, defense_out, stream);
 }
 
+namespace bm {
+static bool study_rides_along(int ks, int h, int nb, int op, int vec, int64_t d, bool nomom, bool clip,
+                              const float* attack_avg_out, const float* update_momentum) {
+  return tuning().step_fuse_study != 0 && fused_rule_instance(ks, h, nb, op) && study_instance(h, op, nomom, clip) && vec == 4 &&
+         d > 0 && d % 4 == 0 &&
+         attack_avg_out == nullptr && (nomom || update_momentum == nullptr);
+}
+
+static int colwise_study_fused(const float* const* sampled, int ks, float* const* buffers, int h, int64_t d, float mu,
+                               float one_minus_damp, const float* clip_factors, float* sampled_avg, float* honest_avg,
+                               float* byz_out, float scale, int attack_kind, int rule_op, int rule_f, int nb,
+                               float* defense_out, double* out6, const StudyRide& ride, double* study_out, void* ws,
+                               hipStream_t s) {
+  double* partial = static_cast<double*>(ws);
+  const bool nomom = buffers == nullptr;
+  StepArgs pass{make_step_table(sampled, ks, buffers, h), ks, h, 0, nomom ? 0.0f : mu, nomom ? 1.0f : one_minus_damp,
+                nomom ? nullptr : clip_factors, sampled_avg, honest_avg, byz_out, scale, attack_kind, partial, nullptr, s};
+  pass.nomom = nomom;
+  pass.study = true;
+  pass.ride = ride;
+  pass.ride.partial = step_study_partials(ws);
+  const int64_t pieces = piece_count(d);
+  int cap = pieces > 1 ? (int)((kStepMaxBlocks - 1) / pieces) - 1 : kStepPieceCap;
+  if (cap > kStepPieceCap) cap = kStepPieceCap;
+  if (cap < 1) return BM_EINVAL;
+  int nparts = 0;
+  const int rc = for_pieces(d, [&](int64_t lo, int64_t dp) {
+    const StepArgs piece = pass.moved(lo);
+    return for_body_and_tail<4>(Tail::kOwnLaunch, 4, dp, kStepBlock, caps_of(cap), [&](auto width, Span& sp) {
+      if constexpr (decltype(width)::value == 4)
+        return launch_fused_rule_any(rule_op, nb, rule_f, defense_out + lo, piece.at(sp));
+      else
+        return BM_EINVAL;
+    }, &nparts);
+  });
+  if (rc != 0) return rc;
+  if (nparts > kStepMaxBlocks + 1) return BM_EINVAL;
+  hipLaunchKernelGGL(step_study_finish_kernel, dim3(1 + kStudyPartial), dim3(kFinishThreads), 0, s, partial,
+                     pass.ride.partial, nparts, out6, study_out);
+  BM_LAUNCH_CHECK();
+  return 0;
+}
+}
+
+extern "C" int bm_momentum_stats_colwise_study(const float* const* sampled, int ks, float* const* buffers, int h,
+                                               int64_t d, float mu, float one_minus_damp, const float* clip_factors,
+                                               float* sampled_avg, float* honest_avg, float* byz_out, float scale,
+                                               int attack_kind, int rule_op, int rule_f, int n_byz, float* defense_out,
+                                               double* out6, const float* past_newest, float* curv,
+                                               const float* past_oldest, int curv_mode, float curv_mu,
+                                               float oldest_weight, const float* params, const float* origin,
+                                               float* attack_avg_out, float* update_momentum, float momentum_mu,
+                                               float update_one_minus_damp, double* study_out, void* ws, void* ws_study,
+                                               void* stream) {
+  using namespace bm;
+  const bool nomom = buffers == nullptr;
+  const bool l2 = params != nullptr && origin != nullptr;
+  if (sampled == nullptr || out6 == nullptr || study_out == nullptr || ws == nullptr || ws_study == nullptr || h < 1 ||
+      ks < h || (nomom && ks != h) || ks > BM_MAX_ROWS || n_byz < 0 || h + n_byz > BM_MAX_ROWS || d < 0 ||
+      !is_column_rule(rule_op) || !is_identical_attack(attack_kind) || (attack_kind & BM_ATTACK_DIRECTION) != 0 ||
+      curv_mode < 0 || curv_mode > 3 ||
+      (d > 0 && (honest_avg == nullptr || (!nomom && sampled_avg == nullptr) || (n_byz > 0 && byz_out == nullptr) ||
+                 defense_out == nullptr ||
+                 (curv_mode >= 1 && curv == nullptr) || (curv_mode >= 2 && past_newest == nullptr) ||
+                 (curv_mode == 3 && past_oldest == nullptr))))
+    return BM_EINVAL;
+  if (nomom) sampled_avg = nullptr;
+  Alignment al;
+  al.of(sampled_avg).of(honest_avg).of(byz_out).of(defense_out).of(sampled, ks).of(curv_mode >= 2 ? past_newest : nullptr)
+      .of(curv_mode >= 1 ? curv : nullptr).of(curv_mode == 3 ? past_oldest : nullptr).of(l2 ? params : nullptr)
+      .of(l2 ? origin : nullptr).of(update_momentum);
+  if (!nomom) al.of(buffers, h);
+  const int vec = al.vec();
+  const float* study_s = nomom ? honest_avg : sampled_avg;
+  if (n_byz == 0) {
+    int rc = nomom ? stack_stats_plain(sampled, ks, d, honest_avg, nullptr, scale, attack_kind, out6, ws, stream)
+                   : bm_momentum_stats(sampled, ks, buffers, h, d, mu, one_minus_damp, clip_factors, sampled_avg, honest_avg,
+                                       nullptr, scale, attack_kind, out6, ws, stream);
+    if (rc != 0) return rc;
+    const float* rows[BM_MAX_ROWS];
+    for (int i = 0; i < h; ++i) rows[i] = nomom ? sampled[i] : buffers[i];
+    rc = bm_colwise(rule_op, rows, h, d, rule_op == BM_OP_MEDIAN ? 0 : rule_f, defense_out, stream);
+    if (rc != 0) return rc;
+    return bm_study_stats_update(study_s, honest_avg, defense_out, nullptr, 0, nullptr, past_newest, curv, past_oldest,
+                                 curv_mode, curv_mu, oldest_weight, params, origin, update_momentum, momentum_mu,
+                                 update_one_minus_damp, d, study_out, ws_study, stream);
+  }
+  if (study_rides_along(ks, h, n_byz, rule_op, vec, d, nomom, clip_factors != nullptr, attack_avg_out, update_momentum)) {
+    if (rule_op != BM_OP_MEDIAN && (rule_f < 0 || h + n_byz < 2 * rule_f + 1)) return BM_EINVAL;
+    StudyRide ride{curv_mode >= 2 ? past_newest : nullptr, curv_mode >= 1 ? curv : nullptr,
+                   curv_mode == 3 ? past_oldest : nullptr, l2 ? params : nullptr, l2 ? origin : nullptr, update_momentum,
+                   nullptr, curv_mu, oldest_weight, momentum_mu, update_one_minus_damp, curv_mode, l2 ? 1 : 0,
+                   update_momentum != nullptr ? 1 : 0};
+    return colwise_study_fused(sampled, ks, buffers, h, d, mu, one_minus_damp, clip_factors, sampled_avg, honest_avg,
+                               byz_out, scale, attack_kind, rule_op, rule_f, n_byz, defense_out, out6, ride, study_out, ws,
+                               static_cast<hipStream_t>(stream));
+  }
+  int rc = nomom ? bm_stack_stats_colwise(sampled, ks, d, honest_avg, byz_out, scale, attack_kind, rule_op, rule_f, n_byz,
+                                          defense_out, out6, ws, stream)
+                 : bm_momentum_stats_colwise(sampled, ks, buffers, h, d, mu, one_minus_damp, clip_factors, sampled_avg,
+                                             honest_avg, byz_out, scale, attack_kind, rule_op, rule_f, n_byz, defense_out,
+                                             out6, ws, stream);
+  if (rc != 0) return rc;
+  return bm_study_stats_update(study_s, honest_avg, defense_out, byz_out, n_byz, attack_avg_out,
+                               past_newest, curv, past_oldest, curv_mode, curv_mu, oldest_weight, params, origin,
+                               update_momentum, momentum_mu, update_one_minus_damp, d, study_out, ws_study, stream);
+}
+
 extern "C" int bm_stack_stats_sqdist(const float* const* rows, int k, int64_t d, int64_t d_total, float* avg_out,
                                      float* byz_out, float scale, int attack_kind, int n_byz, double* sq_nxn,
                                      double* out6, void* ws, void* ws_pair, void* stream) {
diff --git a/byzantinemomentum_amd/csrc/step_call.hip b/byzantinemomentum_amd/csrc/step_call.hip
--- a/byzantinemomentum_amd/csrc/step_call.hip
+++ b/byzantinemomentum_amd/csrc/step_call.hip
@@ -127,6 +127,16 @@
     clipf = sc->clipf;
   }
 
+  int curv_mode = 0;
+  if (p->nb_past > 0 && curv != nullptr) {
+    if (p->past_count == 0 || past_newest == nullptr)
+      curv_mode = 1;
+    else
+      curv_mode = past_oldest != nullptr ? 3 : 2;
+  }
+  const bool has_past = curv_mode >= 2;
+  const bool has_l2 = params != nullptr && origin != nullptr;
+
   const bool rides_along = fr >= 1;
   const float* rows[BM_MAX_ROWS];
   for (int i = 0; i < h; ++i) rows[i] = buffers[i];
@@ -135,9 +145,11 @@
   if (rides_along && !distance_rule) {
     const int op = p->rule == BM_RULE_MEDIAN ? BM_OP_MEDIAN
                    : p->rule == BM_RULE_TRMEAN ? BM_OP_TRMEAN : p->rule == BM_RULE_PHOCAS ? BM_OP_PHOCAS : BM_OP_MEAMED;
-    rc = bm_momentum_stats_colwise(sampled, ks, buffers, h, d, p->mu, p->one_minus_damp, clipf, sampled_avg_out,
-                                   honest_avg_out, byz_out, p->attack_scale, p->attack_kind, op, p->f_decl, fr,
-                                   defense_out, sc->out6, base + lay.ws_step, stream);
+    rc = bm_momentum_stats_colwise_study(sampled, ks, buffers, h, d, p->mu, p->one_minus_damp, clipf, sampled_avg_out,
+                                         honest_avg_out, byz_out, p->attack_scale, p->attack_kind, op, p->f_decl, fr,
+                                         defense_out, sc->out6, past_newest, curv, past_oldest, curv_mode, p->mu,
+                                         p->oldest_weight, params, origin, attack_avg_out, nullptr, 0.0f, 0.0f, sc->study,
+                                         base + lay.ws_step, base + lay.ws_study, stream);
     if (rc != 0) return rc;
   } else if (rides_along) {
     char* rule_ws = base + lay.ws_rule;
@@ -167,19 +179,12 @@
     if (rc != 0) return rc;
   }
 
-  int curv_mode = 0;
-  if (p->nb_past > 0 && curv != nullptr) {
-    if (p->past_count == 0 || past_newest == nullptr)
-      curv_mode = 1;
-    else
-      curv_mode = past_oldest != nullptr ? 3 : 2;
-  }
-  const bool has_past = curv_mode >= 2;
-  const bool has_l2 = params != nullptr && origin != nullptr;
-  rc = bm_study_stats(sampled_avg_out, honest_avg_out, defense_out, byz_out, fr, attack_avg_out, past_newest, curv,
-                      past_oldest, curv_mode, p->mu, p->oldest_weight, params, origin, d, sc->study,
-                      base + lay.ws_study, stream);
-  if (rc != 0) return rc;
+  if (!(rides_along && !distance_rule)) {
+    rc = bm_study_stats(sampled_avg_out, honest_avg_out, defense_out, byz_out, fr, attack_avg_out, past_newest, curv,
+                        past_oldest, curv_mode, p->mu, p->oldest_weight, params, origin, d, sc->study,
+                        base + lay.ws_study, stream);
+    if (rc != 0) return rc;
+  }
 
   hipLaunchKernelGGL(step_pack_kernel, dim3(1), dim3(64), 0, s, sc, fr > 0 ? 1 : 0, has_past ? 1 : 0, has_l2 ? 1 : 0,
                      comm == nullptr ? stats_out : static_cast<double*>(nullptr));
diff --git a/byzantinemomentum_amd/csrc/study.hip b/byzantinemomentum_amd/csrc/study.hip
--- a/byzantinemomentum_amd/csrc/study.hip
+++ b/byzantinemomentum_amd/csrc/study.hip
@@ -1,11 +1,9 @@
-#include "bm_common.h"
+#include "study_body.h"
 
 namespace bm {
 
 constexpr int kStudyBlock = 256;
 constexpr int kStudyMaxBlocks = 2048;
-constexpr int kStudySums = 14;
-constexpr int kStudyPartial = 16;
 
 struct StudyArgs {
   const float* s;
@@ -42,13 +40,12 @@
     acc64[i] = 0.0;
   }
   int since = 0;
-  float amax = 0.0f, dmax = 0.0f;
-  bool a_nan = false, d_nan = false;
+  StudyMax mx;
   const float ff = (float)f_real;
   const int64_t stride = (int64_t)gridDim.x * kStudyBlock;
   for (int64_t v = (int64_t)blockIdx.x * kStudyBlock + threadIdx.x; v < nvec; v += stride) {
     const int64_t j = v * VEC;
-    float s[VEC], h[VEC], df[VEC], bz[VEC], pa[VEC], cv[VEC], ol[VEC], pp[VEC], oo[VEC], mm[VEC];
+    float s[VEC], h[VEC], df[VEC], bz[VEC] = {}, pa[VEC] = {}, cv[VEC] = {}, ol[VEC] = {}, pp[VEC] = {}, oo[VEC] = {}, mm[VEC];
     load_stream<VEC>(a.s + j, s);
     load_stream<VEC>(a.h + j, h);
     load_stream<VEC>(a.def + j, df);
@@ -66,49 +63,13 @@
     float av[VEC];
 #pragma unroll
     for (int c = 0; c < VEC; ++c) {
-      av[c] = 0.0f;
-      if constexpr (ATT) {
-        float t = bz[c];
-        for (int i = 1; i < f_real; ++i) t += bz[c];
-        t = t / ff;
-        av[c] = t;
-        amax = fmaxf(amax, __builtin_fabsf(t));
-        a_nan |= (t != t);
-        const float dd = bz[c] - t;
-        float q = 0.0f;
-        for (int i = 0; i < f_real; ++i) q = __builtin_fmaf(dd, dd, q);
-        acc[12] += q;
-      }
-      dmax = fmaxf(dmax, __builtin_fabsf(df[c]));
-      d_nan |= (df[c] != df[c]);
-      acc[0] = __builtin_fmaf(s[c], s[c], acc[0]);
-      acc[1] = __builtin_fmaf(s[c], h[c], acc[1]);
-      acc[2] = __builtin_fmaf(s[c], df[c], acc[2]);
-      acc[4] = __builtin_fmaf(h[c], h[c], acc[4]);
-      acc[5] = __builtin_fmaf(h[c], df[c], acc[5]);
-      acc[7] = __builtin_fmaf(df[c], df[c], acc[7]);
-      if constexpr (ATT) {
-        acc[3] = __builtin_fmaf(s[c], av[c], acc[3]);
-        acc[6] = __builtin_fmaf(h[c], av[c], acc[6]);
-        acc[8] = __builtin_fmaf(df[c], av[c], acc[8]);
-        acc[9] = __builtin_fmaf(av[c], av[c], acc[9]);
-      }
-      if constexpr (CM >= 2) {
-        acc[10] = __builtin_fmaf(s[c], pa[c], acc[10]);
-        acc[11] = __builtin_fmaf(s[c], cv[c], acc[11]);
-      }
-      if constexpr (L2) {
-        const float e = pp[c] - oo[c];
-        acc[13] = __builtin_fmaf(e, e, acc[13]);
-      }
-      if constexpr (CM == 1) cv[c] = s[c];
-      if constexpr (CM == 3) cv[c] = __builtin_fmaf(w_oldest, ol[c], 1.0f * cv[c]);
-      if constexpr (CM >= 2) cv[c] = __builtin_fmaf(1.0f, s[c], mu * cv[c]);
+      study_past_element(CM, L2, s[c], pa[c], cv[c], ol[c], pp[c], oo[c], mu, w_oldest, acc);
+      av[c] = study_core_element<ATT>(s[c], h[c], df[c], bz[c], f_real, ff, acc, mx);
     }
     if constexpr (CM >= 1) store_stream<VEC>(a.curv + j, cv);
     if (a.mom != nullptr) {
 #pragma unroll
-      for (int c = 0; c < VEC; ++c) mm[c] = __builtin_fmaf(a.mom_b, df[c], a.mom_a * mm[c]);
+      for (int c = 0; c < VEC; ++c) mm[c] = study_momentum_element(a.mom_a, a.mom_b, df[c], mm[c]);
       store_stream<VEC>(a.mom + j, mm);
     }
     if constexpr (ATT) {
@@ -123,8 +84,7 @@
       since = 0;
     }
   }
-  if (a_nan) amax = __builtin_nanf("");
-  if (d_nan) dmax = __builtin_nanf("");
+  const float amax = absmax_value(mx.attack), dmax = absmax_value(mx.defense);
   constexpr int64_t kSlotStride = kStudyMaxBlocks + 1;
   double* p = partial + blockIdx.x;
 #pragma unroll
@@ -178,8 +138,7 @@
     acc[i] = 0.0f;
     acc64[i] = 0.0;
   }
-  float amax = 0.0f, dmax = 0.0f;
-  bool a_nan = false, d_nan = false;
+  StudyMax mx;
   const float ff = (float)f_real;
   const uint32_t tid = threadIdx.x;
   const uint32_t span = gridDim.x * kStudyBurstThreads;
@@ -188,7 +147,7 @@
   for (uint32_t p0 = 0; p0 < iters; p0 += kStudySlots) {
     const uint32_t p1 = (p0 + kStudySlots < iters) ? p0 + kStudySlots : iters;
     for (uint32_t it = p0; it < p1; it += U) {
-      float s[U][VEC], h[U][VEC], df[U][VEC], bz[U][VEC], pa[U][VEC], cv[U][VEC], ol[U][VEC], pp[U][VEC], oo[U][VEC];
+      float s[U][VEC], h[U][VEC], df[U][VEC], bz[U][VEC] = {}, pa[U][VEC] = {}, cv[U][VEC] = {}, ol[U][VEC] = {}, pp[U][VEC] = {}, oo[U][VEC] = {};
       float mm[U][VEC];
       bool live[U];
 #pragma unroll
@@ -218,44 +177,8 @@
         if (!live[u]) continue;
 #pragma unroll
         for (int c = 0; c < VEC; ++c) {
-          float av = 0.0f;
-          if constexpr (ATT) {
-            float t = bz[u][c];
-            for (int i = 1; i < f_real; ++i) t += bz[u][c];
-            t = t / ff;
-            av = t;
-            amax = fmaxf(amax, __builtin_fabsf(t));
-            a_nan |= (t != t);
-            const float dd = bz[u][c] - t;
-            float q = 0.0f;
-            for (int i = 0; i < f_real; ++i) q = __builtin_fmaf(dd, dd, q);
-            acc[12] += q;
-          }
-          dmax = fmaxf(dmax, __builtin_fabsf(df[u][c]));
-          d_nan |= (df[u][c] != df[u][c]);
-          acc[0] = __builtin_fmaf(s[u][c], s[u][c], acc[0]);
-          acc[1] = __builtin_fmaf(s[u][c], h[u][c], acc[1]);
-          acc[2] = __builtin_fmaf(s[u][c], df[u][c], acc[2]);
-          acc[4] = __builtin_fmaf(h[u][c], h[u][c], acc[4]);
-          acc[5] = __builtin_fmaf(h[u][c], df[u][c], acc[5]);
-          acc[7] = __builtin_fmaf(df[u][c], df[u][c], acc[7]);
-          if constexpr (ATT) {
-            acc[3] = __builtin_fmaf(s[u][c], av, acc[3]);
-            acc[6] = __builtin_fmaf(h[u][c], av, acc[6]);
-            acc[8] = __builtin_fmaf(df[u][c], av, acc[8]);
-            acc[9] = __builtin_fmaf(av, av, acc[9]);
-          }
-          if constexpr (CM >= 2) {
-            acc[10] = __builtin_fmaf(s[u][c], pa[u][c], acc[10]);
-            acc[11] = __builtin_fmaf(s[u][c], cv[u][c], acc[11]);
-          }
-          if constexpr (L2) {
-            const float e = pp[u][c] - oo[u][c];
-            acc[13] = __builtin_fmaf(e, e, acc[13]);
-          }
-          if constexpr (CM == 1) cv[u][c] = s[u][c];
-          if constexpr (CM == 3) cv[u][c] = __builtin_fmaf(w_oldest, ol[u][c], 1.0f * cv[u][c]);
-          if constexpr (CM >= 2) cv[u][c] = __builtin_fmaf(1.0f, s[u][c], mu * cv[u][c]);
+          study_past_element(CM, L2, s[u][c], pa[u][c], cv[u][c], ol[u][c], pp[u][c], oo[u][c], mu, w_oldest, acc);
+          study_core_element<ATT>(s[u][c], h[u][c], df[u][c], bz[u][c], f_real, ff, acc, mx);
         }
         V packed;
 #pragma unroll
@@ -263,7 +186,7 @@
         stage[(it + u - p0) * kStudyBurstThreads + tid] = packed;
         if constexpr (MOM) {
 #pragma unroll
-          for (int c = 0; c < VEC; ++c) packed[c] = __builtin_fmaf(a.mom_b, df[u][c], a.mom_a * mm[u][c]);
+          for (int c = 0; c < VEC; ++c) packed[c] = study_momentum_element(a.mom_a, a.mom_b, df[u][c], mm[u][c]);
           stage_mom[(it + u - p0) * kStudyBurstThreads + tid] = packed;
         }
       }
@@ -283,8 +206,7 @@
       }
     }
   }
-  if (a_nan) amax = __builtin_nanf("");
-  if (d_nan) dmax = __builtin_nanf("");
+  const float amax = absmax_value(mx.attack), dmax = absmax_value(mx.defense);
   constexpr int64_t kSlotStride = kStudyMaxBlocks + 1;
   double* p = partial + blockIdx.x;
 #pragma unroll
@@ -317,55 +239,7 @@
 
 __global__ __launch_bounds__(64) void study_finish_kernel(const double* __restrict__ partial, int nparts,
                                                           double* __restrict__ out) {
-  const int slot = blockIdx.x, lane = threadIdx.x;
-  if (slot == 0 && lane >= 23 && lane < BM_STUDY_SLOTS) out[lane] = 0.0;
-  double tot = 0.0;
-  bool nan = false;
-  const bool is_max = slot >= kStudySums;
-  for (int b = lane; b < nparts; b += 64) {
-    const double v = partial[(int64_t)slot * (kStudyMaxBlocks + 1) + b];
-    if (is_max) {
-      nan |= (v != v);
-      tot = v > tot ? v : tot;
-    } else {
-      tot += v;
-    }
-  }
-#pragma unroll
-  for (int off = 32; off > 0; off >>= 1) {
-    const double o = __shfl_down(tot, off, 64);
-    if (is_max) {
-      tot = o > tot ? o : tot;
-      nan |= (bool)__shfl_down((int)nan, off, 64);
-    } else {
-      tot += o;
-    }
-  }
-  if (lane != 0) return;
-  if (is_max) {
-    out[20 + (slot - kStudySums)] = nan ? __builtin_nan("") : tot;
-    return;
-  }
-  if (slot < 10) {
-    int k = 0;
-    for (int r = 0; r < 4; ++r)
-      for (int c = r; c < 4; ++c) {
-        if (k == slot) {
-          out[r * 4 + c] = tot;
-          out[c * 4 + r] = tot;
-        }
-        ++k;
-      }
-    if (slot == 9) out[18] = tot;
-  } else if (slot == 10) {
-    out[16] = tot;
-  } else if (slot == 11) {
-    out[17] = tot;
-  } else if (slot == 12) {
-    out[19] = tot;
-  } else {
-    out[22] = tot;
-  }
+  study_finish_slot(partial, kStudyMaxBlocks + 1, 1, nparts, blockIdx.x , threadIdx.x, out);
 }
 
 template <bool ATT, int CM, bool L2>
diff --git a/byzantinemomentum_amd/csrc/study_body.h b/byzantinemomentum_amd/csrc/study_body.h
--- /dev/null
+++ b/byzantinemomentum_amd/csrc/study_body.h
@@ -0,0 +1,124 @@
+#pragma once
+#include "bm_common.h"
+
+namespace bm {
+
+constexpr int kStudySums = 14;
+constexpr int kStudyPartial = 16;
+
+struct StudyMax {
+  uint32_t attack = 0u, defense = 0u;
+};
+__device__ __forceinline__ void absmax_bits(uint32_t& m, float x) {
+  const uint32_t b = __float_as_uint(__builtin_fabsf(x));
+  m = b > m ? b : m;
+}
+__device__ __forceinline__ float absmax_value(uint32_t m) {
+  const float v = __uint_as_float(m);
+  return v != v ? __builtin_nanf("") : v;
+}
+
+__device__ __forceinline__ void study_past_element(int cm, bool l2, float s, float pa, float& cv, float ol, float pp,
+                                                   float oo, float mu, float w_oldest, float (&acc)[kStudySums]) {
+  if (cm >= 2) {
+    acc[10] = __builtin_fmaf(s, pa, acc[10]);
+    acc[11] = __builtin_fmaf(s, cv, acc[11]);
+  }
+  if (l2) {
+    const float e = pp - oo;
+    acc[13] = __builtin_fmaf(e, e, acc[13]);
+  }
+  if (cm == 1) cv = s;
+  if (cm == 3) cv = __builtin_fmaf(w_oldest, ol, 1.0f * cv);
+  if (cm >= 2) cv = __builtin_fmaf(1.0f, s, mu * cv);
+}
+
+template <bool ATT>
+__device__ __forceinline__ float study_core_element(float s, float h, float df, float bz, int f_real, float ff,
+                                                    float (&acc)[kStudySums], StudyMax& mx) {
+  float av = 0.0f;
+  if constexpr (ATT) {
+    float t = bz;
+    for (int i = 1; i < f_real; ++i) t += bz;
+    t = t / ff;
+    av = t;
+    absmax_bits(mx.attack, t);
+    const float dd = bz - t;
+    float q = 0.0f;
+    for (int i = 0; i < f_real; ++i) q = __builtin_fmaf(dd, dd, q);
+    acc[12] += q;
+  }
+  absmax_bits(mx.defense, df);
+  acc[0] = __builtin_fmaf(s, s, acc[0]);
+  acc[1] = __builtin_fmaf(s, h, acc[1]);
+  acc[2] = __builtin_fmaf(s, df, acc[2]);
+  acc[4] = __builtin_fmaf(h, h, acc[4]);
+  acc[5] = __builtin_fmaf(h, df, acc[5]);
+  acc[7] = __builtin_fmaf(df, df, acc[7]);
+  if constexpr (ATT) {
+    acc[3] = __builtin_fmaf(s, av, acc[3]);
+    acc[6] = __builtin_fmaf(h, av, acc[6]);
+    acc[8] = __builtin_fmaf(df, av, acc[8]);
+    acc[9] = __builtin_fmaf(av, av, acc[9]);
+  }
+  return av;
+}
+
+__device__ __forceinline__ float study_momentum_element(float mom_a, float mom_b, float df, float m) {
+  return __builtin_fmaf(mom_b, df, mom_a * m);
+}
+
+__device__ __forceinline__ void study_finish_slot(const double* __restrict__ partial, int64_t slot_stride,
+                                                  int64_t part_stride, int nparts, int slot, int lane,
+                                                  double* __restrict__ out) {
+  if (slot == 0 && lane >= 23 && lane < BM_STUDY_SLOTS) out[lane] = 0.0;
+  double tot = 0.0;
+  bool nan = false;
+  const bool is_max = slot >= kStudySums;
+  for (int b = lane; b < nparts; b += 64) {
+    const double v = partial[(int64_t)slot * slot_stride + (int64_t)b * part_stride];
+    if (is_max) {
+      nan |= (v != v);
+      tot = v > tot ? v : tot;
+    } else {
+      tot += v;
+    }
+  }
+#pragma unroll
+  for (int off = 32; off > 0; off >>= 1) {
+    const double o = __shfl_down(tot, off, 64);
+    if (is_max) {
+      tot = o > tot ? o : tot;
+      nan |= (bool)__shfl_down((int)nan, off, 64);
+    } else {
+      tot += o;
+    }
+  }
+  if (lane != 0) return;
+  if (is_max) {
+    out[20 + (slot - kStudySums)] = nan ? __builtin_nan("") : tot;
+    return;
+  }
+  if (slot < 10) {
+    int k = 0;
+    for (int r = 0; r < 4; ++r)
+      for (int c = r; c < 4; ++c) {
+        if (k == slot) {
+          out[r * 4 + c] = tot;
+          out[c * 4 + r] = tot;
+        }
+        ++k;
+      }
+    if (slot == 9) out[18] = tot;
+  } else if (slot == 10) {
+    out[16] = tot;
+  } else if (slot == 11) {
+    out[17] = tot;
+  } else if (slot == 12) {
+    out[19] = tot;
+  } else {
+    out[22] = tot;
+  }
+}
+
+}
diff --git a/byzantinemomentum_amd/sharded.py b/byzantinemomentum_amd/sharded.py
--- a/byzantinemomentum_amd/sharded.py
+++ b/byzantinemomentum_amd/sharded.py
@@ -73,7 +73,8 @@
 
   capabilities = frozenset((
     "step_worker", "momentum_stats_colwise", "momentum_stats_sqdist", "stack_stats_colwise", "stack_stats_sqdist",
-    "device_search", "attack_ranking_device", "bulyan_pass2_eval", "order_pair", "colwise_eval", "sqdist2", "anticge"))
+    "device_search", "attack_ranking_device", "bulyan_pass2_eval", "order_pair", "colwise_eval", "sqdist2", "anticge",
+    "colwise_study"))
 
   def __init__(self):
     from . import gars, stats
@@ -141,6 +142,9 @@
 
   def stack_stats_colwise(self, *args, **kwargs):
     return self.stats.stack_stats_colwise(*args, **kwargs)
+
+  def colwise_study(self, *args, **kwargs):
+    return self.stats.colwise_study(*args, **kwargs)
 
   def stack_stats_sqdist(self, *args, **kwargs):
     return self.stats.stack_stats_sqdist(*args, **kwargs)
diff --git a/byzantinemomentum_amd/stats.py b/byzantinemomentum_amd/stats.py
--- a/byzantinemomentum_amd/stats.py
+++ b/byzantinemomentum_amd/stats.py
@@ -8,7 +8,7 @@
 from . import _lib
 from . import gars
 
-__all__ = ["compute_avg_dev_max", "stack_stats_async", "study_dots", "study_stats", "multi_axpby", "row_sqnorms", "momentum_stats", "momentum_stats_colwise", "momentum_stats_sqdist", "stack_stats_colwise", "stack_stats_sqdist",
+__all__ = ["compute_avg_dev_max", "stack_stats_async", "study_dots", "study_stats", "multi_axpby", "row_sqnorms", "momentum_stats", "momentum_stats_colwise", "colwise_study", "momentum_stats_sqdist", "stack_stats_colwise", "stack_stats_sqdist",
            "multi_fma3", "clip_factors", "clip_factors_from_sq", "multi_scale", "clip_gradients", "l2_distance",
            "step_worker", "anticge_sum", "anticge_scale", "anticge_attack"]
 
@@ -322,6 +322,40 @@
   return s_avg, h_avg, byz, defense, out6
 
 
+def colwise_study(sampled, buffers, mu, one_minus_damp, clip_factors_dev, attack_scale, attack, rule, f, n_byz,
+                  past_newest=None, curv=None, past_oldest=None, curv_mode=0, curv_mu=0.0, oldest_weight=0.0, params=None,
+                  origin=None, update_momentum=None, update_mu=0.0, update_omd=0.0):
+  ks, d, device = gars._validate(list(sampled))
+  h = ks if buffers is None else gars._validate(list(buffers) + [sampled[0]])[0] - 1
+  if h < 1 or ks < h or n_byz < 1:
+    raise gars.GarInputError("colwise_study needs 1 <= len(buffers) <= len(sampled) and n_byz >= 1")
+  if (params is None) != (origin is None):
+    raise gars.GarInputError("colwise_study needs both params and origin, or neither")
+  extra = [t for t in (past_newest if curv_mode >= 2 else None, curv if curv_mode >= 1 else None,
+                       past_oldest if curv_mode == 3 else None, params, origin, update_momentum) if t is not None]
+  if extra and gars._validate(extra + [sampled[0]])[1] != d:
+    raise gars.GarInputError("colwise_study: vectors of different lengths")
+  lib = _lib.load()
+  new = lambda: torch.empty(d, dtype=torch.float32, device=device)
+  h_avg, byz, defense = new(), new(), new()
+  s_avg = new() if buffers is not None else None
+  out6 = torch.empty(6, dtype=torch.float64, device=device)
+  study = torch.empty(_lib.STUDY_SLOTS, dtype=torch.float64, device=device)
+  ws = gars._workspace(device, _lib.WS_STEP, 1, d, "ws_step")
+  ws_study = gars._workspace(device, _lib.WS_STUDY, 1, d, "ws_study")
+  gars.invalidate_rank_cache()
+  with torch.cuda.device(device):
+    _lib.check(lib.bm_momentum_stats_colwise_study(
+      _lib.pointer_table(sampled), ks, _lib.pointer_table(buffers) if buffers is not None else None, h, d,
+      ctypes.c_float(mu), ctypes.c_float(one_minus_damp), _opt(clip_factors_dev), _opt(s_avg), _ptr(h_avg), _ptr(byz),
+      ctypes.c_float(attack_scale), _attack_id(attack, False), _EVAL_OPS[rule], int(f), int(n_byz), _ptr(defense),
+      _ptr(out6), _opt(past_newest), _opt(curv), _opt(past_oldest), int(curv_mode), ctypes.c_float(curv_mu),
+      ctypes.c_float(oldest_weight), _opt(params), _opt(origin), None, _opt(update_momentum), ctypes.c_float(update_mu),
+      ctypes.c_float(update_omd), _ptr(study), _ptr(ws), _ptr(ws_study), gars._stream(device)),
+      "bm_momentum_stats_colwise_study")
+  return (s_avg if s_avg is not None else h_avg), h_avg, byz, defense, out6, study
+
+
 def momentum_stats_sqdist(sampled, buffers, mu, one_minus_damp, clip_factors_dev, attack_scale, attack, n_byz,
                           d_total=None):
   ks, d, device = gars._validate(list(sampled))
diff --git a/byzantinemomentum_amd/step.py b/byzantinemomentum_amd/step.py
--- a/byzantinemomentum_amd/step.py
+++ b/byzantinemomentum_amd/step.py
@@ -292,6 +292,19 @@
       sq = ops.row_sqnorms(sampled)
       agg.all_reduce_sum(sq)
       factors = ops.clip_factors_from_sq(sq, ks, self.clip)
+    count = len(self.pasts) if self.nb_past > 0 else 0
+    mode = 0
+    if self.nb_past > 0:
+      if self._curv is None:
+        self._curv = torch.empty_like(sampled[0])
+      mode = 1 if count == 0 else (3 if count == self.nb_past else 2)
+    has_l2 = params is not None and origin is not None
+    past_args = dict(past_newest=self.pasts[0] if count > 0 else None, curv=self._curv,
+                     past_oldest=self.pasts[-1] if mode == 3 else None, curv_mode=mode,
+                     oldest_weight=-(self.mu ** (self.nb_past - 1)) if self.nb_past > 0 else 0.0,
+                     params=params if has_l2 else None, origin=origin if has_l2 else None)
+    rides = "colwise_study" in self.plan.capabilities
+    study = None
     fused_defense, fused_sq = None, None
     first_pass = self.plan.first_pass
     searched = first_pass == "direction"
@@ -300,7 +313,11 @@
     if self.momentum_at == "worker":
       if self.buffers is None:
         self.buffers = self._new_rows(h, sampled[0], zero=True)
-      if first_pass == "rule":
+      if first_pass == "rule" and rides:
+        s_avg, h_avg, byz, fused_defense, out6, study = ops.colwise_study(
+          sampled, self.buffers, self.mu, omd, factors, self.factor, self.attack, self.gar, self.f_decl, self.f_real,
+          curv_mu=self.mu, **past_args)
+      elif first_pass == "rule":
         s_avg, h_avg, byz, fused_defense, out6 = ops.momentum_stats_colwise(
           sampled, self.buffers, self.mu, omd, factors, self.factor, self.attack, self.gar, self.f_decl, self.f_real)
       elif first_pass == "sqdist":
@@ -323,7 +340,14 @@
         honests = sampled[:h]
       if ks != h and first_pass in ("rule", "sqdist"):
         first_pass = "plain"
-      if first_pass == "rule":
+      if first_pass == "rule" and rides and self.momentum_at == "update":
+        if self.server_momentum is None:
+          self.server_momentum = torch.zeros_like(sampled[0])
+        _, h_avg, byz, fused_defense, o6, study = ops.colwise_study(
+          honests, None, 0.0, 1.0, None, self.factor, self.attack, self.gar, self.f_decl, self.f_real, curv_mu=self.mu,
+          update_momentum=self.server_momentum, update_mu=self.mu, update_omd=omd, **past_args)
+        h_out3 = o6[3:]
+      elif first_pass == "rule":
         h_avg, byz, fused_defense, o6 = ops.stack_stats_colwise(honests, self.factor, self.attack, self.gar, self.f_decl,
                                                                 self.f_real)
         h_out3 = o6[3:]
@@ -363,20 +387,10 @@
       self._update = self.server_momentum
     else:
       self._update = defense
-    count = len(self.pasts) if self.nb_past > 0 else 0
-    mode = 0
-    if self.nb_past > 0:
-      if self._curv is None:
-        self._curv = torch.empty_like(s_avg)
-      mode = 1 if count == 0 else (3 if count == self.nb_past else 2)
-    has_l2 = params is not None and origin is not None
-    study = ops.study_stats(s_avg, h_avg, defense, byz if self.f_real > 0 else None, self.f_real,
-                            past_newest=self.pasts[0] if count > 0 else None, curv=self._curv,
-                            past_oldest=self.pasts[-1] if mode == 3 else None, curv_mode=mode, mu=self.mu,
-                            oldest_weight=-(self.mu ** (self.nb_past - 1)) if self.nb_past > 0 else 0.0,
-                            params=params if has_l2 else None, origin=origin if has_l2 else None,
-                            **(dict(update_momentum=self.server_momentum, update_mu=self.mu, update_omd=omd)
-                               if self.momentum_at == "update" else {}))
+    if study is None:
+      study = ops.study_stats(s_avg, h_avg, defense, byz if self.f_real > 0 else None, self.f_real, mu=self.mu, **past_args,
+                              **(dict(update_momentum=self.server_momentum, update_mu=self.mu, update_omd=omd)
+                                 if self.momentum_at == "update" else {}))
     self._pending = dict(s=s_out3, h=h_out3, study=study, npast=2 if count > 0 else 0,
                          prev_s2=self._prev_s2 if count > 0 else None, has_l2=has_l2, ks=ks, floats=None)
     if self.nb_past > 0:
diff --git a/include/bm_gar.h b/include/bm_gar.h
--- a/include/bm_gar.h
+++ b/include/bm_gar.h
@@ -112,6 +112,15 @@
 int bm_stack_stats_sqdist(const float* const* rows, int k, int64_t d, int64_t d_total, float* avg_out, float* byz_out,
                           float scale, int attack_kind, int n_byz, double* sq_nxn, double* out6, void* ws,
                           void* ws_pair, void* stream);
+
+int bm_momentum_stats_colwise_study(const float* const* sampled, int ks, float* const* buffers, int h, int64_t d,
+                                    float mu, float one_minus_damp, const float* clip_factors, float* sampled_avg,
+                                    float* honest_avg, float* byz_out, float scale, int attack_kind, int rule_op,
+                                    int rule_f, int n_byz, float* defense_out, double* out6, const float* past_newest,
+                                    float* curv, const float* past_oldest, int curv_mode, float curv_mu,
+                                    float oldest_weight, const float* params, const float* origin, float* attack_avg_out,
+                                    float* update_momentum, float momentum_mu, float update_one_minus_damp,
+                                    double* study_out, void* ws, void* ws_study, void* stream);
 
 int bm_multi_fma3(float* const* out, const float* const* p, const float* const* q, int k, int64_t d,
                   float a, float b, const float* p_scale, void* stream);
```

Result: slower. 5429 (-1.4%).
